# WilliamVenner/squad-mortar-helper

Measured on AMD Instinct MI355X. Metric: map frames/sec (1920x1080 full CV pipeline), whole job, higher is better.
Workload: dtype u8/f32

## Files before the change

squad-mortar-helper_amd/csrc/smh_kernels.h:

```cpp
#pragma once
#include <hip/hip_runtime.h>
#include <stdint.h>

#include "../../include/smh_vision_hip.h"
#include "../../include/smh_vision_hip_debug.h"

namespace smh {

struct Geom {
	uint32_t W, H;
	uint32_t rx, ry, rw, rh;
	uint32_t bx, by, bw, bh;
	uint32_t qx, qy, qw, qh;
	uint32_t m_ax, m_xoff, m_quads, m_block;
	uint32_t q_ax, q_xoff, q_quads, q_block;
	uint64_t frame_bytes;
	uint64_t ui_pitch, ui_stride;
	uint64_t mask_pitch, mask_stride;
	uint32_t bits_pitch_w; uint64_t bits_stride_w;
	uint64_t ocr_pitch, ocr_stride;
};

struct FrameAux {
	uint32_t open;
// ... 174 lines not shown
	uint8_t *img;
	uint8_t *cls;
	uint64_t img_stride, cls_stride;
	double mpx;
	double ring_m;
	float origin[2];
	uint32_t mm[4];
	uint32_t out_w, out_h;
	uint32_t origin_mode, line;
	uint32_t per_call, has_mpx, has_mm;
	uint32_t pal[10];
};
#define SMH_CLEAR_PROFILE (SMHV_CLEAR_MAX_SAMPLES + 1u)
struct ClearLinesRun {
	FiringRun fr;
	const smhv_frame_result *res;
	const smhv_line *lines;
	smhv_clearance_result *out;
	smhv_clearance *out_lines;
	float *profiles;
	double margin_m;
	uint32_t samples;
	uint32_t n_lines;
	uint32_t mm[4];
	uint32_t per_call, has_mm;
};
#define SMH_CLEAR_KC 32u
struct ClearMapRun {
	FiringRun fr;
	const FrameAux *aux;
	const smhv_frame_result *res;
	smhv_clearance_map_result *out;
	uint8_t *img;
	uint8_t *bytes;
	uint64_t img_stride, bytes_stride;
	double margin_m;
	float origin[2];
	uint32_t mm[4];
	uint32_t out_w, out_h;
	uint32_t samples;
	uint32_t origin_mode, line;
	uint32_t per_call, has_mm;
	uint32_t pal[4];
};
#define SMH_DBG_ITEMS (SMHV_TEXT_MAX_RUNS + 1u + 4u * SMHV_MAX_PROBES)
#define SMH_DBG_TEXT 200u
#define SMH_DBG_NONE 0u
#define SMH_DBG_TEXT_ITEM 1u
#define SMH_DBG_FILL 2u
#define SMH_DBG_FRAME 3u
struct DebugItem {
	const uint8_t *text;
	float ax, ay, bx, by;
	int32_t x0, y0, x1, y1;
	uint32_t color;
	uint32_t kind;
	uint32_t n_lines, pad;
	uint8_t off[8], len[8];
};
struct DebugRun {
	const uint8_t *ui;
	const FrameAux *aux;
	const smhv_frame_result *res;
	const smhv_text_run *runs;
	const smhv_probe_point *points;
	smhv_probe *probes;
	DebugItem *items;
	uint8_t *pool;
	uint8_t *img;
	uint64_t img_stride;
	uint32_t out_w, out_h;
	uint32_t n_runs, n_points;
	uint32_t flags;
	uint32_t scale;
	float sw, sh, tx, ty;
};
__host__ __device__ inline uint32_t tiled_rows(const Geom &g) { return (g.rh + 7u) >> 3; }
__host__ __device__ inline uint64_t tiled_stride_w(const Geom &g) { return (uint64_t)tiled_rows(g) * g.bits_pitch_w * 8u; }
__host__ __device__ inline uint32_t occ_pitch(const Geom &g) { return ((g.m_block >> 6) + 3u) & ~3u; }
__host__ __device__ inline uint64_t occ_stride(const Geom &g) { return (uint64_t)tiled_rows(g) * occ_pitch(g); }

#define SMH_RAY_OFF_BATCHES 168u

#define SMH_SECTOR_R 52
#define SMH_SECTOR_DIM (2 * SMH_SECTOR_R + 1)
#define SMH_SECTOR_ENTRIES (SMH_SECTOR_DIM * SMH_SECTOR_DIM)
#define SMH_CULL_CELLS (SMH_SECTOR_DIM * 4)
#define SMH_CULL_TAB_WORDS (SMH_CULL_CELLS + (SMH_SECTOR_ENTRIES + 3) / 4)

#define SVC_MAX_SLOTS 32u
struct SvcSlot {
	Buffers b;
	uint32_t n;
	uint32_t seq;
	uint32_t done;
	uint32_t pad;
	unsigned long long t_pub;
};
#define SVC_REMOTE_RING 12u
#define SVC_REMOTE_OPEN 0x80000000ull
struct SvcRemoteEntry {
	unsigned long long post;
	unsigned long long claim;
	uint32_t res_a[4];
	uint32_t res_b[4];
	unsigned long long pad[2];
};
struct SvcRemote {
	unsigned long long state;
	unsigned long long info;
	unsigned long long pad[6];
	SvcRemoteEntry ring[SVC_REMOTE_RING];
};
#define SVC_HELP_RING 256u
struct SvcCtl {
	int32_t avail;
	uint32_t closing;
	int32_t help_avail;
	uint32_t help_head, help_reserve;
	uint32_t stat_remote;
	uint32_t head;
	uint32_t reserve;
	uint32_t completed;
	uint32_t busy;
	uint32_t stat_items, stat_waves;
	unsigned long long stat_busy, stat_life;
	unsigned long long stat_phase[4];
	unsigned long long stat_help;
	uint32_t stat_requests, stat_attached;
	unsigned long long stat_t_wait, stat_t_sub, stat_t_last;
	uint32_t stat_h_polls, stat_h_empty, stat_h_lost, stat_h_idle_exit, stat_h_closed_exit, stat_h_pad;
	unsigned long long stat_h_cycles, stat_h_cast_cycles;
	unsigned long long help_ring[SVC_HELP_RING];
};
struct SvcHost {
	unsigned long long state;
	uint32_t launches;
	uint32_t pad0;
	uint32_t done_seq[SVC_MAX_SLOTS];
	uint32_t pad[12];
};
struct SvcParams {
	SvcCtl *ctl;
	unsigned long long *ring;
	SvcSlot *slots;
	SvcHost *host;
	const uint32_t *cull_tab;
	const float *ray_off;
	float max_gap;
	uint32_t tile_cap, list_cap;
	uint32_t part_words;
	uint32_t ring_log2;
	uint32_t epoch;
	uint32_t idle_short, idle_long;
	uint32_t flags;
	SvcRemote *remote;
	uint32_t *remote_store;
	uint32_t remote_store_words;
	uint32_t remote_after;
	uint32_t remote_tickets;
	uint32_t remote_last_div;
	uint32_t compact;
};
uint32_t svc_waves_for(const Geom &g, uint32_t tile_limit, uint32_t *part_words, uint32_t *tile_cap, uint32_t *list_cap, uint32_t *lds_bytes, uint32_t *compact = nullptr);
uint32_t svc_store_words_for(const Geom &g, uint32_t tile_cap, uint32_t compact);
hipError_t svc_probe_host_atomics(SvcHost *h, SvcHost *d_h, bool *ok);
hipError_t launch_svc_publish(SvcCtl *ctl, unsigned long long *ring, SvcSlot *slots, uint32_t slot, const Buffers &b, uint32_t n, uint32_t seq, uint32_t ring_log2, hipStream_t s);
hipError_t launch_lsd_service(const Geom &g, const SvcParams &p, uint32_t workgroups, uint32_t waves, uint32_t lds_bytes, hipStream_t s);

enum : uint32_t { MAP_UI = 1u, MAP_MASK = 2u, MAP_BYTES = 4u, MAP_PRIO = 0x100u, MAP_BAND_MAJOR = 0x200u };
enum : uint32_t { BRQ_OCR = 1u, BRQ_SCALES = 2u };
// ... 129 lines not shown
```

squad-mortar-helper_amd/csrc/smh_lsd.hip:

```cpp
#include <algorithm>
#include <atomic>
#include <cstdlib>
#include <cstring>

#include "smh_device.h"
#include "smh_proximity.h"
#include "smh_record.inc"

namespace smh {

struct RayDir { uint32_t dx, dy; };
__device__ RayDir g_ray_table[SMH_LSD_RAYS] = {
#include "ray_table.inc"
};

#ifndef LSD_BS
#define LSD_BS 1024
#endif
#define LSD_NW (LSD_BS / 64)
#ifndef LSD_C
#define LSD_C 8u
#endif
#ifndef LSD_C_RESET
#define LSD_C_RESET 2u
// ... 38 lines not shown
#define LSD_W2_PITCH 6u

enum { LSD_MODE_ROWS = 0, LSD_MODE_XWIN = 1, LSD_MODE_GLOBAL = 2, LSD_MODE_TILE = 3, LSD_MODE_WIN2 = 4, LSD_MODE_TILEC = 5 };

template <bool CACHED = false>
__device__ __forceinline__ uint32_t win_raw(const Win &m, int xi, int yi) {
	const uint32_t ry = min((uint32_t)(yi - m.y_lo), m.rows_hi);
	const int X = xi + m.xbias;
	const uint32_t rc = min((uint32_t)(X >> 5), m.cols_hi);
	uint32_t word;
	const uint32_t cr = ry - m.c_y0;
	if (CACHED && cr < m.c_rows) word = *(const LdsWord *)((const LdsByte *)m.c_p + __umul24(cr, m.c_pitch4) + (rc << 2));
	else word = *(const uint32_t *)((const char *)m.p + __umul24(ry, m.pitch4) + (rc << 2));
	return word >> ((uint32_t)X & 31u);
}
__device__ __forceinline__ uint32_t tile_word(const Win &m, int wq, int yi) {
	const uint32_t t = m.t_idx[__mul24(yi >> 3, (int)m.t_pitch) + wq];
	return m.t_tiles[(t << 3) + ((uint32_t)yi & 7u)];
}
typedef uint32_t lds_u32x4 __attribute__((ext_vector_type(4)));
__device__ __forceinline__ uint32_t tilec_number(const Win &m, int wq, int ty) {
	const uint32_t col = (uint32_t)(wq + 2);
	const lds_u32x4 e = *(const __attribute__((address_space(3))) lds_u32x4 *)(m.tc_rows + (__mul24(ty, (int)m.tc_groups) + (int)(col >> 6)) * 4);
	const uint32_t c = col & 63u;
	const uint32_t lo_m = c >= 32u ? 0xFFFFFFFFu : ((1u << c) - 1u), hi_m = c > 32u ? ((1u << (c - 32u)) - 1u) : 0u;
	const uint32_t bit = ((c >= 32u ? e.y >> (c - 32u) : e.x >> c) & 1u);
	const uint32_t before = (uint32_t)__builtin_popcount(e.x & lo_m) + (uint32_t)__builtin_popcount(e.y & hi_m);
	return bit ? e.z + before + 1u : 0u;
}
__device__ __forceinline__ uint32_t tilec_word(const Win &m, int wq, int yi) {
	return m.t_tiles[(tilec_number(m, wq, yi >> 3) << 3) + ((uint32_t)yi & 7u)];
}
__device__ __forceinline__ uint32_t tilec_raw(const Win &m, float x, float y) {
	const int yi = (int)__builtin_amdgcn_fmed3f(y, -1.0f, m.hf);
	const int xi = (int)x;
	return tilec_word(m, xi >> 5, yi) >> ((uint32_t)xi & 31u);
}
__device__ __forceinline__ void tilec_raw8(const Win &m, float xs, float ys, float dx, float dy, float &xo, float &yo, float &x, float &y, uint32_t &Wm) {
	int yi[8], xi[8];
	uint32_t t[8];
#pragma unroll
	for (int j = 0; j < 8; ++j) {
		x = xo + xs; y = yo + ys;
		yi[j] = (int)__builtin_amdgcn_fmed3f(y, -1.0f, m.hf);
		xi[j] = (int)x;
		xo += dx; yo += dy;
	}
#pragma unroll
	for (int j = 0; j < 8; ++j) t[j] = tilec_number(m, xi[j] >> 5, yi[j] >> 3);
#pragma unroll
	for (int j = 0; j < 8; ++j) t[j] = m.t_tiles[(t[j] << 3) + ((uint32_t)yi[j] & 7u)];
#pragma unroll
	for (int j = 0; j < 8; ++j) Wm = __builtin_amdgcn_alignbit(t[j] >> ((uint32_t)xi[j] & 31u), Wm, 1);
}
__device__ __forceinline__ uint32_t tile_raw(const Win &m, float x, float y) {
	const int yi = (int)__builtin_amdgcn_fmed3f(y, -1.0f, m.hf);
	const int xi = (int)x;
	return tile_word(m, xi >> 5, yi) >> ((uint32_t)xi & 31u);
}
__device__ __forceinline__ void tile_raw8(const Win &m, float xs, float ys, float dx, float dy, float &xo, float &yo, float &x, float &y, uint32_t &Wm) {
	int yi[8], xi[8];
	uint32_t t[8];
#pragma unroll
	for (int j = 0; j < 8; ++j) {
		x = xo + xs; y = yo + ys;
		yi[j] = (int)__builtin_amdgcn_fmed3f(y, -1.0f, m.hf);
		xi[j] = (int)x;
		xo += dx; yo += dy;
	}
#pragma unroll
	for (int j = 0; j < 8; ++j) t[j] = m.t_idx[__mul24(yi[j] >> 3, (int)m.t_pitch) + (xi[j] >> 5)];
#pragma unroll
	for (int j = 0; j < 8; ++j) t[j] = m.t_tiles[(t[j] << 3) + ((uint32_t)yi[j] & 7u)];
#pragma unroll
	for (int j = 0; j < 8; ++j) Wm = __builtin_amdgcn_alignbit(t[j] >> ((uint32_t)xi[j] & 31u), Wm, 1);
}
__device__ __forceinline__ uint32_t win2_raw(const Win &m, float x, float y) {
	const int yi = (int)y, xi = (int)x;
	const uint32_t word = *(const LdsWord *)(m.w2 + __mul24(yi, (int)(4u * LSD_W2_PITCH)) + ((xi >> 3) & ~3));
	return word >> ((uint32_t)xi & 31u);
}
__device__ __forceinline__ uint32_t win2_word(const Win &m, int wq, int yi) { return *(const LdsWord *)(m.w2 + __mul24(yi, (int)(4u * LSD_W2_PITCH)) + (wq << 2)); }
__device__ __forceinline__ uint32_t win2_bit(const Win &m, int xi, int yi) { return (win2_word(m, xi >> 5, yi) >> ((uint32_t)xi & 31u)) & 1u; }

__device__ __forceinline__ uint32_t win_bit(const Win &m, int xi, int yi) {
	if (m.tiled) return ((m.compact ? tilec_word(m, xi >> 5, yi) : tile_word(m, xi >> 5, yi)) >> ((uint32_t)xi & 31u)) & 1u;
	return (m.c_rows ? win_raw<true>(m, xi, yi) : win_raw<false>(m, xi, yi)) & 1u;
}

__device__ __forceinline__ uint32_t win_word(const Win &m, int wq, int yi) {
	if (m.tiled) return ((uint32_t)yi < m.h && (uint32_t)(wq + 2) < m.t_pitch) ? (m.compact ? tilec_word(m, wq, yi) : tile_word(m, wq, yi)) : 0u;
	const uint32_t ry = (uint32_t)(yi - m.y_lo), rc = (uint32_t)wq;
	uint32_t v = 0;
	if (ry <= m.rows_hi && rc <= m.cols_hi) {
		const uint32_t cr = ry - m.c_y0;
		if (cr < m.c_rows) v = *(const LdsWord *)((const LdsByte *)m.c_p + __umul24(cr, m.c_pitch4) + (rc << 2));
		else v = *(const uint32_t *)((const char *)m.p + __umul24(ry, m.pitch4) + (rc << 2));
	}
	return v;
}

__device__ __forceinline__ uint32_t win_raw_rows(const Win &m, float x, float y) {
	const int yi = (int)__builtin_amdgcn_fmed3f(y, m.ylo_f, m.yhi_f);
	const int xi = (int)x;
	const char *row = m.rows0 + __mul24(yi, (int)m.pitch4);
	const uint32_t word = *(const uint32_t *)(row + ((xi >> 5) << 2));
	return word >> ((uint32_t)xi & 31u);
}

__device__ __forceinline__ bool in_image(const Win &m, float x, float y) { return x >= 0.0f && y >= 0.0f && x < m.wf && y < m.hf; }

__device__ void cast_ray_literal(const Win &m, float xs, float ys, float max_gap, float dx, float dy, float &xe, float &ye, uint32_t &steps) {
	float x = xs, y = ys, xo = 0.0f, yo = 0.0f, g0 = 0.0f, g1 = 0.0f, g2 = 0.0f;
	while (in_image(m, x, y)) {
		++steps;
		if (win_bit(m, (int)x, (int)y)) {
			g0 = 0.0f; g1 = 0.0f; g2 = 0.0f;
		} else if (g0 >= max_gap) {
			x = g1; y = g2;
			break;
		} else if (g0 == 0.0f) {
			g0 = 1.0f; g1 = x; g2 = y;
		} else {
			g0 += 1.0f;
		}
		xo += dx; yo += dy;
		x = xo + xs; y = yo + ys;
	}
	xe = xs; ye = ys;
	const uint32_t xi = f2u(x), yi = f2u(y);
	if (xi < m.w && yi < m.h && win_bit(m, (int)xi, (int)yi) == 0u) { xe = x - dx; ye = y - dy; }
}

struct RayState {
	float bxo, byo;
	uint32_t k0, g;
	float gxo, gyo;
	uint32_t gj, gk0;
	uint32_t nexit;
};
enum { RAY_CONTINUE = 0, RAY_ABORTED = 1, RAY_LEFT_IMAGE = 2 };

template <int MODE, int G = 8>
__device__ __forceinline__ int ray_batch(const Win &m, float xs, float ys, float dx, float dy, uint32_t T, RayState &s, uint32_t &steps) {
	static_assert((G == 8 || G == 16 || G == 32) && ((MODE != LSD_MODE_TILE && MODE != LSD_MODE_TILEC) || G == 8), "group size");
	float xo = s.bxo, yo = s.byo, x = 0.0f, y = 0.0f;
	uint32_t Wm = 0;
	uint32_t taken = 0;
#pragma unroll 1
	for (int jj = 0; jj < 32 / G; ++jj) {
		if constexpr (MODE == LSD_MODE_TILE) tile_raw8(m, xs, ys, dx, dy, xo, yo, x, y, Wm);
		else if constexpr (MODE == LSD_MODE_TILEC) tilec_raw8(m, xs, ys, dx, dy, xo, yo, x, y, Wm);
		else
#pragma unroll
		for (int j = 0; j < G; ++j) {
			x = xo + xs; y = yo + ys;
			if (MODE == LSD_MODE_ROWS) Wm = __builtin_amdgcn_alignbit(win_raw_rows(m, x, y), Wm, 1);
			else if (MODE == LSD_MODE_WIN2) Wm = __builtin_amdgcn_alignbit(win2_raw(m, x, y), Wm, 1);
			else if (MODE == LSD_MODE_TILE) Wm = __builtin_amdgcn_alignbit(tile_raw(m, x, y), Wm, 1);
			else Wm = __builtin_amdgcn_alignbit(win_raw<MODE == LSD_MODE_GLOBAL>(m, (int)x, (int)y), Wm, 1);
			xo += dx; yo += dy;
		}
		taken += (uint32_t)G;
		if (taken > T && taken < 32u && __all((Wm >> (31u - T)) == 0u)) break;
	}
	Wm >>= 32u - taken;
// ... 43 lines not shown
				if (gg + len > T) {
					steps += s.k0 + pos + (T - gg) + 1u;
					return RAY_ABORTED;
				}
				gg += len;
				if (end >= 32u) break;
				rem &= 0xFFFFFFFFu << end;
			}
		}
		if (n < 32u) { steps += s.k0 + n; s.nexit = n; return RAY_LEFT_IMAGE; }
		s.g = gg;
	}
	s.bxo = xo; s.byo = yo; s.k0 += 32u;
	return RAY_CONTINUE;
}

__device__ __forceinline__ void ray_endpoint(const Win &m, int status, const RayState &s, float xs, float ys, float dx, float dy, float &xe, float &ye) {
	if (status == RAY_ABORTED) {
		float gx = s.gxo, gy = s.gyo;
		for (uint32_t k = 0; k < s.gj; ++k) { gx += dx; gy += dy; }
		xe = (gx + xs) - dx; ye = (gy + ys) - dy;
	} else {
		float rx = s.bxo, ry = s.byo;
		for (uint32_t k = 0; k < s.nexit; ++k) { rx += dx; ry += dy; }
		const float px = rx + xs, py = ry + ys;
		xe = xs; ye = ys;
		const uint32_t xi = f2u(px), yi = f2u(py);
		if (xi < m.w && yi < m.h && win_bit(m, (int)xi, (int)yi) == 0u) { xe = px - dx; ye = py - dy; }
	}
}

__device__ __forceinline__ uint32_t white_at(const Win &m, float fx, float fy) {
	const uint32_t xi = min(f2u(fx), m.w - 1u), yi = min(f2u(fy), m.h - 1u);
	return win_bit(m, (int)xi, (int)yi);
}
__device__ void get_centre(const Win &m, float px, float py, float &ox, float &oy) {
	float left = px;
	while (left > 0.0f && fabsf(left - px) < SMH_LSD_CENTRE_REACH && white_at(m, left, py)) left -= 1.0f;
	float right = px;
	while (right < (float)(m.w - 1u) && fabsf(right - px) < SMH_LSD_CENTRE_REACH && white_at(m, right, py)) right += 1.0f;
	float up = py;
	while (up > 0.0f && fabsf(up - py) < SMH_LSD_CENTRE_REACH && white_at(m, px, up)) up -= 1.0f;
	float down = py;
	while (down < (float)(m.h - 1u) && fabsf(down - py) < SMH_LSD_CENTRE_REACH && white_at(m, px, down)) down += 1.0f;
	ox = (left + right) / 2.0f;
	oy = (up + down) / 2.0f;
}


#ifdef SMH_LSD_PROFILE
#define PROF_DECL unsigned long long prof_t[12] = {0, 0, 0, 0, 0, 0, 0, 0, 0, 0, 0, 0}, prof_last = __builtin_amdgcn_s_memtime();
#define PROF_MARK(i) do { const unsigned long long _n = __builtin_amdgcn_s_memtime(); prof_t[i] += _n - prof_last; prof_last = _n; } while (0)
#define PROF_STORE(res) do { if (threadIdx.x == 0) for (int _i = 0; _i < 12; ++_i) ((unsigned long long *)(res)->meters)[20 + _i] = prof_t[_i]; } while (0)
#define PROF_ARG , prof_t
#else
#define PROF_DECL
#define PROF_MARK(i)
#define PROF_STORE(res)
#define PROF_ARG
#endif

struct LsdShared {
	unsigned long long cand_best[LSD_C];
	unsigned long long unit_key[LSD_UNITS];
	float unit_end[LSD_UNITS][2];
	uint32_t unit_kmax[LSD_UNITS];
	float cand_pt[LSD_C][2];
	float cand_end[LSD_C][2];
	uint32_t cand_steps[LSD_C];
	uint32_t cand_kmax[LSD_C];
	uint32_t cand_key[LSD_C];
	uint32_t scan[LSD_NW];
	uint32_t qtail, segnext, unit_next;
	uint32_t cand_px[LSD_C][2];
	uint32_t cand_wkey[LSD_C];
	uint32_t cached;
	uint32_t post[LSD_LOOKAHEAD];
	uint32_t req_tail, posted_hi, posted_new, helpers_seen, head_seen;
	uint32_t h_n;
	unsigned long long pick;
	uint32_t nlive;
	unsigned short ulist[LSD_UNITS];
	unsigned long long live[LSD_C];
	float lines[SMH_LSD_MAX_LINES][4];
	float prox_a[SMH_LSD_MAX_LINES];
	double prox_d[SMH_LSD_MAX_LINES][2];
#ifdef SMH_LSD_PROFILE
	uint32_t exp_far, exp_units;
#endif
};

__device__ __forceinline__ ProxLine shared_prox_line(const LsdShared &sh, uint32_t l) {
	ProxLine L;
	L.x0 = sh.lines[l][0]; L.y0 = sh.lines[l][1]; L.x1 = sh.lines[l][2]; L.y1 = sh.lines[l][3];
	L.a = sh.prox_a[l]; L.dxl = sh.prox_d[l][0]; L.dyl = sh.prox_d[l][1];
	L.degenerate = L.dxl == 0.0 && L.dyl == 0.0;
	return L;
}

template <int MODE>
__device__ void ray_engine(const Win &m, LsdShared &sh, uint32_t *queue, uint32_t nc, float max_gap, bool always_exact, unsigned long long *prof_t = nullptr) {
	const uint32_t tid = threadIdx.x, lane = tid & 63u, wave = tid >> 6;
#ifdef SMH_LSD_PROFILE
	unsigned long long prof_last = __builtin_amdgcn_s_memtime();
#endif
	const bool fast_gap = max_gap > 0.0f && max_gap <= 60000.0f;
	const uint32_t T = fast_gap ? (uint32_t)ceilf(max_gap) : 0u;
	const uint32_t nunits = nc * LSD_GROUPS, nlive = sh.nlive;

	uint32_t pos = wave;
	uint32_t pn = 0;
	if (lane == 0) pn = atomicAdd(&sh.unit_next, 1u);
	pn = (uint32_t)__builtin_amdgcn_readfirstlane((int)pn);
	uint32_t u = pos < nlive ? sh.ulist[pos] : 0u;
	RayDir nd = g_ray_table[min((u % LSD_GROUPS) * 64u + lane, (uint32_t)SMH_LSD_RAYS - 1u)];
	for (; pos < nlive; ) {
		const uint32_t c = u / LSD_GROUPS, i = (u - c * LSD_GROUPS) * 64u + lane;
		const bool valid = i < SMH_LSD_RAYS;
		const float dx = __uint_as_float(nd.dx), dy = __uint_as_float(nd.dy);
		const uint32_t ucur = u;
		pos = pn;
		if (pos < nlive) {
			u = sh.ulist[pos];
			nd = g_ray_table[min((u % LSD_GROUPS) * 64u + lane, (uint32_t)SMH_LSD_RAYS - 1u)];
			if (lane == 0) pn = atomicAdd(&sh.unit_next, 1u);
			pn = (uint32_t)__builtin_amdgcn_readfirstlane((int)pn);
		}
		const float xs = sh.cand_pt[c][0], ys = sh.cand_pt[c][1];
		const bool fast = fast_gap && in_image(m, xs, ys);
		float xe = xs, ye = ys;
		uint32_t steps = 0;
		int status = RAY_ABORTED;
		bool exact = false;
		RayState s = {0.0f, 0.0f, 0u, 0u, 0.0f, 0.0f, 0u, 0u, 0u};
		if (valid) {
			if (fast) {
				status = RAY_CONTINUE;
#pragma unroll 1
				for (uint32_t bi = 0; bi < LSD_A_BATCHES && status == RAY_CONTINUE; ++bi) status = ray_batch<MODE>(m, xs, ys, dx, dy, T, s, steps);
			} else {
				cast_ray_literal(m, xs, ys, max_gap, dx, dy, xe, ye, steps);
				exact = true;
			}
		}
#ifdef SMH_LSD_PROFILE
		if (prof_t) { const unsigned long long _n = __builtin_amdgcn_s_memtime(); prof_t[0] += _n - prof_last; prof_last = _n; }
#endif
		const uint64_t sv = __ballot(status == RAY_CONTINUE);
		if (sv) {
			uint32_t base = 0;
			if (lane == 0) base = atomicAdd(&sh.qtail, (uint32_t)__popcll(sv));
			base = (uint32_t)__builtin_amdgcn_readfirstlane((int)base);
			const uint32_t slot = base + (uint32_t)__popcll(sv & ((1ull << lane) - 1ull));
			if (status == RAY_CONTINUE && slot >= LSD_QCAP) {
				while (status == RAY_CONTINUE) status = ray_batch<MODE>(m, xs, ys, dx, dy, T, s, steps);
				ray_endpoint(m, status, s, xs, ys, dx, dy, xe, ye);
				exact = true;
			} else if (status == RAY_CONTINUE) {
				queue[2u * slot] = (c << 16) | i;
				queue[2u * slot + 1u] = s.g | (s.gj << 16) | ((s.gk0 >> 5) << 24);
			}
		}
		const bool fin = valid && status != RAY_CONTINUE;
		if (fin && !exact && (status == RAY_LEFT_IMAGE || (!always_exact && s.gk0 + s.gj > SMH_LSD_REJECT_K))) { ray_endpoint(m, status, s, xs, ys, dx, dy, xe, ye); exact = true; }
		if (__any(fin && exact)) {
			unsigned long long key = 0;
// ... 172 lines not shown
	uint32_t wy0, wrows, wwords;
	int xorg;
	uint32_t c_pitch, c_cap_rows;
};

template <int MODE, bool WAVE = false>
__device__ __forceinline__ void frame_setup(const Geom &g, const Buffers &b, uint32_t f, const FrameAux &aux, uint32_t *smem, FrameView &v) {
	static_assert(!WAVE || MODE == LSD_MODE_GLOBAL, "only the global-memory view is built without the workgroup");
	const uint32_t tid = threadIdx.x;
	const uint32_t *gbits = b.bits + (size_t)f * g.bits_stride_w;
	Win &m = v.m;
	v.gbits = gbits;
	m.w = g.rw; m.h = g.rh; m.wf = (float)g.rw; m.hf = (float)g.rh;
	m.rows0 = nullptr; m.ylo_f = 0.0f; m.yhi_f = 0.0f;
	m.c_p = (const LdsWord *)smem; m.c_y0 = 0u; m.c_rows = 0u; m.c_pitch4 = 0u;
	m.t_idx = nullptr; m.t_tiles = nullptr; m.t_pitch = 0u; m.tiled = false; m.w2 = nullptr;
	m.tc_rows = nullptr; m.tc_groups = 0u; m.compact = false;
	v.c_pitch = g.bits_pitch_w | 1u; v.c_cap_rows = min(g.rh, LSD_WIN_WORDS_CAP / v.c_pitch);
	if (MODE == LSD_MODE_ROWS) {
		const uint32_t wy0 = aux.y_min, wrows = aux.y_max - aux.y_min + 1u;
		v.wy0 = wy0; v.wrows = wrows; v.wwords = LSD_ROWS_PITCH(g.bits_pitch_w); v.xorg = 0;
		const uint32_t pitch = v.wwords, gp = g.bits_pitch_w;
		const uint32_t total = (wrows + 2u) * pitch + 4u;
		for (uint32_t idx = tid; idx < total; idx += blockDim.x) {
			uint32_t val = 0;
			if (idx >= 2u + pitch && idx < 2u + (wrows + 1u) * pitch) {
				const uint32_t k = idx - 2u - pitch, r = k / pitch, c = k - r * pitch;
				if (c < gp) {
					const uint32_t *src = gbits + (size_t)(wy0 + r) * gp + c;
					const uint32_t lo = src[0], hi = (c + 1u < gp) ? src[1] : 0u;
					val = __builtin_amdgcn_alignbit(hi, lo, g.m_xoff);
				}
			}
			smem[idx] = val;
		}
		m.p = smem + 2; m.pitch4 = pitch * 4u;
		m.y_lo = (int)wy0 - 1; m.rows_hi = wrows + 1u;
		m.xbias = 0; m.cols_hi = pitch - 1u;
		m.rows0 = (const char *)(smem + 2) - (ptrdiff_t)((int)wy0 - 1) * (ptrdiff_t)(pitch * 4u);
		m.ylo_f = (float)((int)wy0 - 1); m.yhi_f = (float)(wy0 + wrows);
	} else if (MODE == LSD_MODE_XWIN) {
		const uint32_t ww0 = aux.w_min, wy0 = aux.y_min, wrows = aux.y_max - aux.y_min + 1u, wwords = aux.w_max - aux.w_min + 1u;
		v.wy0 = wy0; v.wrows = wrows; v.wwords = wwords;
		v.xorg = (int)(ww0 * 32u) - (int)g.m_xoff;
		const uint32_t pitch = (wwords + 2u) | 1u;
		m.p = smem; m.pitch4 = pitch * 4u;
		m.y_lo = (int)wy0 - 1; m.rows_hi = wrows + 1u;
		m.xbias = (int)g.m_xoff - 32 * ((int)ww0 - 1); m.cols_hi = wwords + 1u;
		const uint32_t total = (wrows + 2u) * pitch;
		for (uint32_t idx = tid; idx < total; idx += blockDim.x) {
			const uint32_t r = idx / pitch, c = idx - r * pitch;
			uint32_t val = 0;
			if (r >= 1u && r <= wrows && c >= 1u && c <= wwords) val = gbits[(size_t)(wy0 + r - 1u) * g.bits_pitch_w + ww0 + c - 1u];
			smem[idx] = val;
		}
	} else {
		v.wy0 = 0; v.wrows = g.rh; v.wwords = g.bits_pitch_w; v.xorg = -(int)g.m_xoff;
		m.p = gbits; m.pitch4 = g.bits_pitch_w * 4u;
		m.y_lo = 0; m.rows_hi = g.rh - 1u;
		m.xbias = (int)g.m_xoff; m.cols_hi = g.bits_pitch_w - 1u;
	}
	if (!WAVE) __syncthreads();
}

template <int MODE>
__device__ __forceinline__ void cache_cover(const Geom &g, FrameView &v, uint32_t *smem, int lo, int hi) {
	if (MODE != LSD_MODE_GLOBAL) return;
	Win &m = v.m;
	lo = max(lo, 0); hi = min(hi, (int)g.rh - 1);
	if (m.c_rows && lo >= (int)m.c_y0 && hi < (int)(m.c_y0 + m.c_rows)) return;
	__syncthreads();
	const uint32_t y0 = (uint32_t)min(lo, (int)(g.rh - v.c_cap_rows));
	for (uint32_t idx = threadIdx.x; idx < v.c_cap_rows * v.c_pitch; idx += LSD_BS) {
		const uint32_t r = idx / v.c_pitch, c = idx - r * v.c_pitch;
		smem[idx] = c < g.bits_pitch_w ? v.gbits[(size_t)(y0 + r) * g.bits_pitch_w + c] : 0u;
	}
	m.c_y0 = y0; m.c_rows = v.c_cap_rows; m.c_pitch4 = v.c_pitch * 4u;
	__syncthreads();
}

__device__ __forceinline__ void group_reset(LsdShared &sh, uint32_t nc, bool cull) {
	const uint32_t tid = threadIdx.x;
	if (tid < nc * LSD_GROUPS) { sh.unit_key[tid] = 0ull; sh.unit_kmax[tid] = 0u; }
	if (tid < LSD_C) { sh.cand_best[tid] = 0ull; sh.cand_steps[tid] = 0u; sh.cand_kmax[tid] = 0u; sh.live[tid] = cull ? 0ull : ~0ull; }
	if (tid == 0) { sh.qtail = 0u; sh.unit_next = LSD_NW; sh.nlive = 0u; sh.cached = 0u;
#ifdef SMH_LSD_PROFILE
		sh.exp_far = 0u; sh.exp_units = 0u;
#endif
	}
}

template <int MODE>
__device__ __forceinline__ void cast_group(const Win &m, LsdShared &sh, uint32_t *queue, const uint32_t *cull_tab, uint32_t nc, bool cull, float max_gap,
                                           unsigned long long *prof_t = nullptr) {
	const uint32_t tid = threadIdx.x;
#ifdef SMH_LSD_PROFILE
	unsigned long long prof_last = __builtin_amdgcn_s_memtime();
#endif
	if (tid < nc * 32u) {
		const uint32_t c = tid >> 5, l = tid & 31u, dir = l >> 3, k = l & 7u;
		const float cx = (float)sh.cand_px[c][0], cy = (float)sh.cand_px[c][1];
		const float fk = (float)k;
		bool cond = k < 5u;
		if (dir == 0u) cond = cond && (cx - fk > 0.0f) && white_at(m, cx - fk, cy);
		else if (dir == 1u) cond = cond && (cx + fk < (float)(m.w - 1u)) && white_at(m, cx + fk, cy);
		else if (dir == 2u) cond = cond && (cy - fk > 0.0f) && white_at(m, cx, cy - fk);
		else cond = cond && (cy + fk < (float)(m.h - 1u)) && white_at(m, cx, cy + fk);
		const uint32_t bits = (uint32_t)(__ballot(cond) >> (tid & 32u));
		if (l == 0u) {
			const float nl = (float)__builtin_ctz(~(bits & 0xFFu)), nr = (float)__builtin_ctz(~((bits >> 8) & 0xFFu));
			const float nu = (float)__builtin_ctz(~((bits >> 16) & 0xFFu)), nd = (float)__builtin_ctz(~((bits >> 24) & 0xFFu));
			sh.cand_pt[c][0] = ((cx - nl) + (cx + nr)) / 2.0f;
			sh.cand_pt[c][1] = ((cy - nu) + (cy + nd)) / 2.0f;
		}
	}
	__syncthreads();
#ifdef SMH_LSD_PROFILE
	if (prof_t) { const unsigned long long _n = __builtin_amdgcn_s_memtime(); prof_t[10] += _n - prof_last; prof_last = _n; }
#endif
	const uint32_t cached = sh.cached;
	if (cull) {
		for (uint32_t id = tid; id < nc * SMH_CULL_CELLS; id += LSD_BS) {
			const uint32_t c = id / SMH_CULL_CELLS, cell = id - c * SMH_CULL_CELLS;
			if ((cached >> c) & 1u) continue;
			const int fx = (int)floorf(sh.cand_pt[c][0]), fy = (int)floorf(sh.cand_pt[c][1]);
			const int yi = fy + (int)(cell >> 2) - SMH_SECTOR_R;
			if ((uint32_t)yi >= m.h) continue;
			const int b0 = fx - SMH_SECTOR_R + (int)((cell & 3u) << 5) + m.xbias;
			const uint32_t lo = win_word(m, b0 >> 5, yi), hi = win_word(m, (b0 >> 5) + 1, yi);
			uint32_t hit = __builtin_amdgcn_alignbit(hi, lo, (uint32_t)b0 & 31u) & cull_tab[cell];
			if (hit) {
				const uint8_t *codes = (const uint8_t *)(cull_tab + SMH_CULL_CELLS) + (cell >> 2) * SMH_SECTOR_DIM + ((cell & 3u) << 5);
				unsigned long long acc = 0ull;
				while (hit) {
					const uint32_t code = codes[__builtin_ctz(hit)];
					hit &= hit - 1u;
					acc |= code == 0xFFu ? ~0ull : ((2ull << (code >> 6)) - 1ull) << (code & 63u);
				}
				atomicOr(&sh.live[c], (acc | (acc >> LSD_GROUPS)) & ((1ull << LSD_GROUPS) - 1ull));
			}
		}
		__syncthreads();
	}
	if (tid < nc * LSD_GROUPS) {
		const uint32_t c = tid / LSD_GROUPS;
		if (!((cached >> c) & 1u) && ((sh.live[c] >> (tid - c * LSD_GROUPS)) & 1ull)) sh.ulist[atomicAdd(&sh.nlive, 1u)] = (unsigned short)tid;
	}
	__syncthreads();
#ifdef SMH_LSD_PROFILE
	if (prof_t) { const unsigned long long _n = __builtin_amdgcn_s_memtime(); prof_t[11] += _n - prof_last; prof_last = _n; }
#endif
	if (sh.nlive != 0u) ray_engine<MODE>(m, sh, queue, nc, max_gap, false PROF_ARG);
}

template <int MODE>
__device__ void lsd_frame(const Geom &g, const Buffers &b, uint32_t f, float max_gap, int mode, float spx, float spy, const FrameAux &aux,
                          uint32_t *smem, LsdShared &sh, uint32_t *cull_tab, LsdCoop *co) {
	const uint32_t tid = threadIdx.x, lane = tid & 63u, wave = tid >> 6;
	smhv_frame_result *res = &b.results[f];
	PROF_DECL
	FrameView v;
	frame_setup<MODE>(g, b, f, aux, smem, v);
	Win &m = v.m;
	uint32_t *list = smem + LSD_WIN_WORDS_CAP, *queue = list + LSD_LIST_CAP;
	const uint32_t wy0 = v.wy0, wrows = v.wrows, wwords = v.wwords;
	const int xorg = v.xorg;
	const uint32_t WT = wrows * wwords;
	auto dom_word = [&](uint32_t wi) -> uint32_t {
		const uint32_t r = wi / wwords, c = wi - r * wwords;
		if (MODE == LSD_MODE_ROWS) return m.p[(r + 1u) * wwords + c];
		if (MODE == LSD_MODE_XWIN) return m.p[(r + 1u) * (m.pitch4 >> 2) + c + 1u];
		return m.p[wi];
	};

	if (mode == 1) {
		if (tid < LSD_GROUPS) { sh.unit_key[tid] = 0ull; sh.unit_kmax[tid] = 0u; sh.ulist[tid] = (unsigned short)tid; }
		cache_cover<MODE>(g, v, smem, (int)spy - (int)(v.c_cap_rows / 2u), (int)spy - (int)(v.c_cap_rows / 2u) + (int)v.c_cap_rows - 1);
		if (tid == 0) { sh.live[0] = ~0ull; sh.cand_best[0] = 0ull; sh.cand_steps[0] = 0u; sh.cand_kmax[0] = 0u; sh.qtail = 0u; sh.unit_next = LSD_NW; sh.nlive = LSD_GROUPS; sh.cand_pt[0][0] = spx; sh.cand_pt[0][1] = spy; }
		__syncthreads();
		ray_engine<MODE>(m, sh, queue, 1u, max_gap, true PROF_ARG);
		if (tid == 0) {
			res->lines[0].x0 = spx; res->lines[0].y0 = spy; res->lines[0].x1 = sh.cand_end[0][0]; res->lines[0].y1 = sh.cand_end[0][1];
			res->length_px[0] = (double)__uint_as_float((uint32_t)(sh.cand_best[0] >> 32));
			res->n_lines = 1; res->rounds = 1; res->ray_steps = sh.cand_steps[0]; res->status = SMHV_FRAME_OK;
		}
		return;
	}

	const bool cull = b.cull_tab != nullptr && max_gap > 0.0f && max_gap <= 49.0f;
	const uint32_t *ring = co ? b.co.req + (size_t)f * SMH_LSD_REQ_CAP : nullptr;
	const LsdCacheEntry *ctab = co ? b.co.cache + (size_t)f * SMH_LSD_CACHE_SLOTS : nullptr;
	if (tid == 0) { sh.req_tail = 0u; sh.posted_hi = 0u; sh.posted_new = 0u; sh.helpers_seen = 0u; sh.head_seen = 0u; if (co) st_relaxed(&co->mode1, (uint32_t)MODE + 1u); }
	if (tid < LSD_LOOKAHEAD) sh.post[tid] = 0u;
	uint32_t rounds = 0, n_lines = 0;
	unsigned long long steps = 0ull;
	uint32_t seg_start = 0, cmax = 1u;
	bool done = false;
	PROF_MARK(8);
	while (!done) {
		const uint32_t range = WT - seg_start;
		const uint32_t per = (range + LSD_BS - 1u) / LSD_BS;
		const uint32_t my0 = min(seg_start + tid * per, WT), my1 = min(my0 + per, WT);
		uint32_t cnt = 0;
		for (uint32_t wi = my0; wi < my1; ++wi) cnt += dom_word(wi) != 0u ? 1u : 0u;
		uint32_t incl = cnt;
		for (int o = 1; o < 64; o <<= 1) { const uint32_t t = __shfl_up(incl, o); if (lane >= (uint32_t)o) incl += t; }
		if (lane == 63) sh.scan[wave] = incl;
		if (tid == 0) sh.segnext = WT;
		__syncthreads();
		uint32_t wprefix = 0, total = 0;
#pragma unroll
		for (int k = 0; k < LSD_NW; ++k) { const uint32_t s = sh.scan[k]; if ((uint32_t)k < wave) wprefix += s; total += s; }
		uint32_t o = wprefix + incl - cnt;
		for (uint32_t wi = my0; wi < my1; ++wi)
			if (dom_word(wi) != 0u) {
				if (o < LSD_LIST_CAP) list[o] = wi;
				else if (o == LSD_LIST_CAP) sh.segnext = wi;
				++o;
			}
		__syncthreads();
		const uint32_t Tn = min(total, LSD_LIST_CAP);
		const uint32_t segnext = sh.segnext;
		PROF_MARK(9);

		for (uint32_t cbase = 0; cbase < Tn && !done; cbase += LSD_BS) {
			const uint32_t e = cbase + tid;
			uint32_t surv = 0, wkey0 = 0;
			float py = 0.0f, px0 = 0.0f;
			if (e < Tn) {
				const uint32_t wi = list[e];
				surv = dom_word(wi);
				const uint32_t r = wi / wwords, c = wi - r * wwords;
				py = (float)(wy0 + r);
				px0 = (float)(xorg + (int)(c * 32u));
				wkey0 = (wi << 5) + 1u;
				for (uint32_t l = 0; l < n_lines && surv; ++l) surv = prox_filter_word(surv, px0, py, shared_prox_line(sh, l));
			}
			while (true) {
				if (co && tid == 0) {
					sh.helpers_seen = ld_relaxed(&co->helpers); sh.head_seen = ld_relaxed(&co->req_head);
					sh.posted_hi = max(sh.posted_hi, sh.posted_new);
				}
				const uint32_t pc = __popc(surv);
				uint32_t pin = pc;
				for (int o2 = 1; o2 < 64; o2 <<= 1) { const uint32_t t = __shfl_up(pin, o2); if (lane >= (uint32_t)o2) pin += t; }
				if (lane == 63) sh.scan[wave] = pin;
				__syncthreads();
				uint32_t wp = 0, tot = 0;
#pragma unroll
				for (int k = 0; k < LSD_NW; ++k) { const uint32_t s = sh.scan[k]; if ((uint32_t)k < wave) wp += s; tot += s; }
				if (tot == 0u) break;
				const bool helped = co != nullptr && sh.helpers_seen != 0u;
				const uint32_t posted_hi = sh.posted_hi;
				uint32_t nc = min(tot, cmax);
				uint32_t rank = wp + pin - pc;
				while (surv && rank < cmax) {
					const uint32_t bit = __builtin_ctz(surv);
					surv &= surv - 1u;
					sh.cand_key[rank] = (tid << 5) | bit;
					sh.cand_wkey[rank] = wkey0 + bit;
					sh.cand_px[rank][0] = (uint32_t)((int)px0 + (int)bit); sh.cand_px[rank][1] = (uint32_t)py;
					++rank;
				}
				if (helped) {
					uint32_t s2 = surv, r2 = rank;
					while (s2 && r2 < cmax + LSD_LOOKAHEAD) {
						const uint32_t bit = __builtin_ctz(s2);
						s2 &= s2 - 1u;
						if (r2 >= cmax && wkey0 + bit > posted_hi) {
							sh.post[r2 - cmax] = 0x80000000u | pix_pack((uint32_t)((int)px0 + (int)bit), (uint32_t)py);
							atomicMax(&sh.posted_new, wkey0 + bit);
						}
// ... 14 lines not shown
					nc = nce;
					cache_cover<MODE>(g, v, smem, lo, (int)sh.cand_px[nc - 1u][1] + LSD_CACHE_MARGIN);
				}
				if (helped) {
					if (wave == 0) {
						const uint32_t pv = lane < LSD_LOOKAHEAD ? sh.post[lane] : 0u;
						if (lane < LSD_LOOKAHEAD) sh.post[lane] = 0u;
						const unsigned long long valid = __ballot((pv >> 31) != 0u);
						const uint32_t tail = sh.req_tail, used = tail - min(sh.head_seen, tail);
						const uint32_t room = SMH_LSD_REQ_CAP - min(used, SMH_LSD_REQ_CAP);
						const uint32_t pos = (uint32_t)__popcll(valid & ((1ull << lane) - 1ull));
						const uint32_t np = min((uint32_t)__popcll(valid), room);
						if ((pv >> 31) && pos < np) {
							const uint32_t idx = tail + pos;
							st_relaxed(const_cast<uint32_t *>(ring) + idx % SMH_LSD_REQ_CAP, (((idx / SMH_LSD_REQ_CAP) & 0xFFu) << 24) | (pv & 0xFFFFFFu));
						}
						if (lane == 0 && np) { st_release(&co->req_tail, tail + np); sh.req_tail = tail + np; }
						if (lane == 0) __hip_atomic_fetch_add(&co->stat_groups, 1u, __ATOMIC_RELAXED, __HIP_MEMORY_SCOPE_AGENT);
					} else if (tid >= 64u && tid < 64u + nc) {
						const uint32_t c = tid - 64u;
						unsigned long long best; float ex, ey; uint32_t st;
						if (cache_lookup(ctab, b.co.epoch, pix_pack(sh.cand_px[c][0], sh.cand_px[c][1]), best, ex, ey, st)) {
							sh.cand_best[c] = best; sh.cand_end[c][0] = ex; sh.cand_end[c][1] = ey; sh.cand_steps[c] = st;
							atomicOr(&sh.cached, 1u << c);
							__hip_atomic_fetch_add(&co->stat_hits, 1u, __ATOMIC_RELAXED, __HIP_MEMORY_SCOPE_AGENT);
						}
					}
					__syncthreads();
				}
				PROF_MARK(10);
				cast_group<MODE>(m, sh, queue, cull_tab, nc, cull, max_gap PROF_ARG);
#ifdef SMH_LSD_PROFILE
				prof_last = __builtin_amdgcn_s_memtime();
#endif

				const uint32_t first_new = n_lines;
				for (uint32_t c = 0; c < nc; ++c) {
					const float cx = (float)sh.cand_px[c][0], cy = (float)sh.cand_px[c][1];
					bool skip = false;
					for (uint32_t l = first_new; l < n_lines; ++l)
						skip = skip || near_line(cx, cy, sh.lines[l][0], sh.lines[l][1], sh.lines[l][2], sh.lines[l][3]);
					if (skip) continue;
					++rounds;
					steps += sh.cand_steps[c];
					const float len = __uint_as_float((uint32_t)(sh.cand_best[c] >> 32));
					if (len > SMH_LSD_ACCEPT_LEN_SQ) {
						float ex, ey;
						get_centre(m, sh.cand_end[c][0], sh.cand_end[c][1], ex, ey);
						sh.lines[n_lines][0] = sh.cand_pt[c][0]; sh.lines[n_lines][1] = sh.cand_pt[c][1];
						sh.lines[n_lines][2] = ex; sh.lines[n_lines][3] = ey;
						const ProxLine pl = prox_line(sh.cand_pt[c][0], sh.cand_pt[c][1], ex, ey);
						sh.prox_a[n_lines] = pl.a; sh.prox_d[n_lines][0] = pl.dxl; sh.prox_d[n_lines][1] = pl.dyl;
						++n_lines;
						if (n_lines == SMH_LSD_MAX_LINES) { done = true; break; }
					}
				}
				if (done) break;
				if (helped && n_lines != first_new && tid == 0) {
					__hip_atomic_fetch_max(&co->req_head, sh.req_tail, __ATOMIC_RELAXED, __HIP_MEMORY_SCOPE_AGENT);
					sh.posted_hi = sh.cand_wkey[nc - 1u]; sh.posted_new = 0u;
				}
				cmax = (n_lines != first_new) ? LSD_C_RESET : min(cmax * 2u, LSD_C);
				PROF_MARK(5);
				for (uint32_t l = first_new; l < n_lines && surv; ++l) surv = prox_filter_word(surv, px0, py, shared_prox_line(sh, l));
			}
			__syncthreads();
		}
		if (segnext >= WT) break;
		seg_start = segnext;
		__syncthreads();
	}
	__syncthreads();
	if (tid < n_lines) {
		res->lines[tid].x0 = sh.lines[tid][0]; res->lines[tid].y0 = sh.lines[tid][1];
		res->lines[tid].x1 = sh.lines[tid][2]; res->lines[tid].y1 = sh.lines[tid][3];
	}
	if (tid == 0) { res->n_lines = n_lines; res->rounds = rounds; res->ray_steps = steps; res->status = SMHV_FRAME_OK; }
	PROF_STORE(res);
}

template <int MODE>
__device__ void lsd_help(const Geom &g, const Buffers &b, uint32_t n_frames, float max_gap, uint32_t *smem, LsdShared &sh, uint32_t *cull_tab, bool have_cull_tab) {
	const uint32_t tid = threadIdx.x;
	const bool cull = b.cull_tab != nullptr && max_gap > 0.0f && max_gap <= 49.0f;
	if (cull && !have_cull_tab) for (uint32_t i = tid; i < SMH_CULL_TAB_WORDS; i += LSD_BS) cull_tab[i] = b.cull_tab[i];
	uint32_t *queue = smem + LSD_WIN_WORDS_CAP + LSD_LIST_CAP;
	uint32_t idle = 0;
	while (true) {
		unsigned long long key = 0ull;
		for (uint32_t f = tid; f < n_frames; f += LSD_BS) {
			const LsdCoop *c = &b.co.coop[f];
			const uint32_t rem = ld_relaxed(&c->remaining), hl = ld_relaxed(&c->helpers), dn = ld_relaxed(&c->done);
			if (!dn && hl < LSD_MAX_HELPERS && rem >= LSD_HELP_MIN_REMAINING && ld_relaxed(&c->mode1) == (uint32_t)MODE + 1u) {
				const unsigned long long k = ((unsigned long long)(rem / (hl + 1u)) << 32) | f;
				key = k > key ? k : key;
			}
		}
		if (tid == 0) sh.pick = 0ull;
		__syncthreads();
		key = wave_max64(key);
		if ((tid & 63u) == 0 && key) atomicMax(&sh.pick, key);
		__syncthreads();
		const unsigned long long pick = sh.pick;
		if (pick == 0ull) {
			if (tid == 0) sh.h_n = ld_relaxed(&b.co.ctl->finished[MODE]);
			__syncthreads();
			const uint32_t fin = sh.h_n;
			__syncthreads();
			if (fin >= n_frames || ++idle > LSD_HELPER_IDLE_POLLS) return;
			__builtin_amdgcn_s_sleep(127);
			continue;
		}
		const uint32_t f = (uint32_t)pick;
		LsdCoop *co = &b.co.coop[f];
		if (tid == 0) {
			const uint32_t prev = __hip_atomic_fetch_add(&co->helpers, 1u, __ATOMIC_RELAXED, __HIP_MEMORY_SCOPE_AGENT);
			sh.h_n = prev < LSD_MAX_HELPERS ? 1u : 0u;
			if (prev >= LSD_MAX_HELPERS) __hip_atomic_fetch_sub(&co->helpers, 1u, __ATOMIC_RELAXED, __HIP_MEMORY_SCOPE_AGENT);
		}
		__syncthreads();
		if (sh.h_n == 0u) { __syncthreads(); continue; }
		__syncthreads();
		const FrameAux aux = b.aux[f];
		FrameView v;
		frame_setup<MODE>(g, b, f, aux, smem, v);
		const uint32_t *ring = b.co.req + (size_t)f * SMH_LSD_REQ_CAP;
		LsdCacheEntry *ctab = b.co.cache + (size_t)f * SMH_LSD_CACHE_SLOTS;
		uint32_t misses = 0;
		while (true) {
			if (tid == 0) {
				uint32_t px[LSD_C];
				uint32_t n = 0;
				if (ld_relaxed(&co->done)) n = 0xFFFFFFFFu;
				else {
					const uint32_t got = ring_claim(co, ring, px);
					for (uint32_t i = 0; i < got; ++i) {
						const uint32_t x = px[i] & 0xFFFu, y = px[i] >> 12;
						unsigned long long best; float ex, ey; uint32_t st;
						if (x < v.m.w && y < v.m.h && !cache_lookup(ctab, b.co.epoch, px[i], best, ex, ey, st)) { sh.cand_px[n][0] = x; sh.cand_px[n][1] = y; ++n; }
					}
				}
				sh.h_n = n;
			}
			__syncthreads();
			const uint32_t nc = sh.h_n;
			if (nc == 0xFFFFFFFFu) break;
			if (nc == 0u) {
				__syncthreads();
				if (++misses > LSD_HELPER_IDLE_POLLS) break;
				__builtin_amdgcn_s_sleep(127);
				continue;
			}
			misses = 0; idle = 0;
			group_reset(sh, nc, cull);
			__syncthreads();
			if (MODE == LSD_MODE_GLOBAL) {
				int lo = (int)sh.cand_px[0][1], hi = lo;
				for (uint32_t c = 1; c < nc; ++c) { lo = min(lo, (int)sh.cand_px[c][1]); hi = max(hi, (int)sh.cand_px[c][1]); }
				cache_cover<MODE>(g, v, smem, lo - LSD_CACHE_MARGIN, min(hi + LSD_CACHE_MARGIN, lo - LSD_CACHE_MARGIN + (int)v.c_cap_rows - 1));
			}
			cast_group<MODE>(v.m, sh, queue, cull_tab, nc, cull, max_gap);
			if (tid == 0) __hip_atomic_fetch_add(&co->stat_casts, nc, __ATOMIC_RELAXED, __HIP_MEMORY_SCOPE_AGENT);
			if (tid < nc) cache_insert(ctab, b.co.epoch, pix_pack(sh.cand_px[tid][0], sh.cand_px[tid][1]), sh.cand_best[tid], sh.cand_end[tid][0], sh.cand_end[tid][1], sh.cand_steps[tid]);
			__syncthreads();
		}
		if (tid == 0) __hip_atomic_fetch_sub(&co->helpers, 1u, __ATOMIC_RELAXED, __HIP_MEMORY_SCOPE_AGENT);
		__syncthreads();
	}
}

__device__ __forceinline__ int lsd_mode_for(const Geom &g, const FrameAux &aux, uint32_t cap = LSD_WIN_WORDS_CAP) {
	int lmode = LSD_MODE_GLOBAL;
	if (aux.n_mask_px != 0) {
		const uint32_t wrows = aux.y_max - aux.y_min + 1u, wwords = aux.w_max - aux.w_min + 1u;
		if ((wrows + 2u) * LSD_ROWS_PITCH(g.bits_pitch_w) + 4u <= cap) lmode = LSD_MODE_ROWS;
		else if ((wrows + 2u) * ((wwords + 2u) | 1u) <= cap) lmode = LSD_MODE_XWIN;
	}
	return lmode;
}

template <int MODE, bool COOP>
__global__ void __launch_bounds__(LSD_BS) __attribute__((amdgpu_waves_per_eu(5, 5))) k_lsd(Geom g, Buffers b, float max_gap, int mode, float spx, float spy, uint32_t n_frames) {
	extern __shared__ __attribute__((aligned(16))) uint32_t smem[];
	__shared__ LsdShared sh;
	__shared__ uint32_t cull_tab[SMH_CULL_TAB_WORDS];
	const uint32_t f = blockIdx.x;
	const bool coop = COOP && mode == 0 && b.co.ctl != nullptr;
	bool have_tab = false;
	if (f < n_frames) {
		if (coop && threadIdx.x == 0) __hip_atomic_fetch_add(&b.co.ctl->started[MODE], 1u, __ATOMIC_RELAXED, __HIP_MEMORY_SCOPE_AGENT);
		const FrameAux aux = b.aux[f];
		bool mine = true;
		if (mode == 0) {
			if (!aux.open || aux.n_mask_px == 0) {
				if (MODE == LSD_MODE_ROWS && threadIdx.x == 0) { b.results[f].n_lines = 0; b.results[f].rounds = 0; b.results[f].ray_steps = 0; b.results[f].status = SMHV_FRAME_OK; }
				mine = false;
			}
		}
		bool record = mode == 0 && (b.rec_stages & SMH_REC_ON) != 0u && !mine && MODE == LSD_MODE_ROWS;
		if (mine && lsd_mode_for(g, aux) != MODE) mine = false;
		if (mine) {
			const bool cull = mode == 0 && b.cull_tab != nullptr && max_gap > 0.0f && max_gap <= 49.0f;
			if (cull) { for (uint32_t i = threadIdx.x; i < SMH_CULL_TAB_WORDS; i += LSD_BS) cull_tab[i] = b.cull_tab[i]; have_tab = true; }
			lsd_frame<MODE>(g, b, f, max_gap, mode, spx, spy, aux, smem, sh, cull_tab, (COOP && coop) ? &b.co.coop[f] : nullptr);
			record = mode == 0 && (b.rec_stages & SMH_REC_ON) != 0u;
		}
		if (record) {
			struct Head { Geom g; Buffers b; };
			const Head *ka = (const Head *)__builtin_amdgcn_kernarg_segment_ptr();
			__syncthreads();
			frame_record_tail(&ka->g, &ka->b, f);
		}
		if (!COOP || !coop) return;
		__syncthreads();
		if (threadIdx.x == 0) {
			if (mine) { st_relaxed(&b.co.coop[f].remaining, 0u); st_release(&b.co.coop[f].done, 1u); }
			__hip_atomic_fetch_add(&b.co.ctl->finished[MODE], 1u, __ATOMIC_RELAXED, __HIP_MEMORY_SCOPE_AGENT);
			sh.h_n = (mine && ld_relaxed(&b.co.ctl->started[MODE]) >= n_frames) ? 1u : 0u;
		}
		__syncthreads();
		if (sh.h_n == 0u) return;
		__syncthreads();
	} else if (!coop) {
		return;
	}
	if (COOP) lsd_help<MODE>(g, b, n_frames, max_gap, smem, sh, cull_tab, have_tab);
}

#include "smh_lsd_wave.inc"
#include "smh_lsd_seq.inc"
#include "smh_service.inc"

__global__ void k_build_sector_table(unsigned long long *tab, uint32_t T) {
	const uint32_t i = blockIdx.x * blockDim.x + threadIdx.x;
	if (i >= SMH_SECTOR_ENTRIES) return;
	const int oy = (int)(i / SMH_SECTOR_DIM) - SMH_SECTOR_R, ox = (int)(i % SMH_SECTOR_DIM) - SMH_SECTOR_R;
	const double rho = 0.7072 + 0.7072 + 0.05;
	const double kmin = T >= 50u ? 0.0 : (double)(50u - T), kmax = 50.0;
	const double r0 = sqrt((double)(ox * ox + oy * oy));
	unsigned long long m = 0ull;
	if (r0 >= kmin - rho && r0 <= kmax + rho) {
		if (r0 <= rho) {
			m = ~0ull;
		} else {
			const double PI = 3.14159265358979323846;
			double phi = atan2((double)oy, (double)ox) * 180.0 / PI;
			if (phi < 0.0) phi += 360.0;
			const double delta = asin(rho / r0 > 1.0 ? 1.0 : rho / r0) * 180.0 / PI + 0.2;
			for (int u = 0; u < LSD_GROUPS_HOST; ++u) {
				const double a0 = 6.4 * u, a1 = 6.4 * u + 6.3;
				bool hit = false;
				for (int wrap = -1; wrap <= 1 && !hit; ++wrap) {
					const double lo = phi - delta + 360.0 * wrap, hi = phi + delta + 360.0 * wrap;
					hit = !(hi < a0 || lo > a1);
				}
				if (hit) m |= 1ull << u;
			}
		}
	}
	tab[i] = m;
}

size_t lsd_lds_bytes() { return LSD_DYN_LDS_BYTES; }

static std::atomic<bool> &lsd_classic_flag() {
	static std::atomic<bool> flag{false};
	return flag;
}
void lsd_set_classic(bool on) { lsd_classic_flag().store(on, std::memory_order_relaxed); }
static std::atomic<uint32_t> g_tile_cap_override{0};
void lsd_set_tile_cap(uint32_t cap) { g_tile_cap_override.store(cap, std::memory_order_relaxed); }
static std::atomic<uint32_t> g_bs_override{0};
void lsd_set_threads(uint32_t threads) { g_bs_override.store(threads, std::memory_order_relaxed); }
static std::atomic<uint32_t> g_spin_limit{W_SPIN_LIMIT_DEFAULT};
void lsd_set_spin_limit(uint32_t polls) { g_spin_limit.store(polls ? polls : W_SPIN_LIMIT_DEFAULT, std::memory_order_relaxed); }

bool lsd_rows_only(const Geom &g) { return (g.rh + 2u) * LSD_ROWS_PITCH(g.bits_pitch_w) + 4u <= LSD_WIN_WORDS_CAP; }

static uint32_t lsd_tile_static_lds() {
	static const uint32_t v = [] { hipFuncAttributes a; return hipFuncGetAttributes(&a, (const void *)k_lsd_tile) == hipSuccess ? (uint32_t)a.sharedSizeBytes : 17408u; }();
	return v;
}
static uint32_t lsd_tile_cap_of(const Geom &g, uint32_t tile_limit) {
	const uint32_t cap_o = g_tile_cap_override.load(std::memory_order_relaxed);
	uint32_t cap = tile_cap_for(g);
	if (tile_limit) cap = std::min(cap, tile_limit);
	if (cap_o) cap = std::min(cap_o, tile_cap_for(g));
	return cap;
}
uint32_t lsd_tile_lds_bytes(const Geom &g, uint32_t tile_limit) {
	return lsd_tile_static_lds() + (tile_mask_words(g.rw, g.rh, lsd_tile_cap_of(g, tile_limit)) + 2u * tile_list_cap_for(g) + W_NWIN * W_WIN_STRIDE) * 4u;
}

hipError_t launch_lsd(const Geom &g, const Buffers &b, uint32_t n, float max_gap, int mode, float px, float py, hipStream_t s, const LsdFork *fk, uint32_t tile_bs, bool prefer_classic,
                      uint32_t tile_limit, bool *record_fused) {
	if (record_fused) *record_fused = false;
	const unsigned lds_full = LSD_DYN_LDS_BYTES;
	static std::atomic<uint64_t> attr_devices{0};
	int dev = 0;
	hipError_t e0 = hipGetDevice(&dev);
	if (e0 != hipSuccess) return e0;
	if (dev >= 64 || !((attr_devices.load(std::memory_order_acquire) >> dev) & 1ull)) {
		hipError_t e = hipSuccess;
		const void *fns[] = {(const void *)k_lsd<LSD_MODE_ROWS, false>, (const void *)k_lsd<LSD_MODE_XWIN, false>, (const void *)k_lsd<LSD_MODE_GLOBAL, false>,
		                     (const void *)k_lsd<LSD_MODE_ROWS, true>, (const void *)k_lsd<LSD_MODE_XWIN, true>, (const void *)k_lsd<LSD_MODE_GLOBAL, true>};
		for (const void *fn : fns) if (e == hipSuccess) e = hipFuncSetAttribute(fn, hipFuncAttributeMaxDynamicSharedMemorySize, (int)lds_full);
		if (e == hipSuccess) e = hipFuncSetAttribute((const void *)k_lsd_tile, hipFuncAttributeMaxDynamicSharedMemorySize, (int)LSD_TILE_DYN_LDS_MAX);
		if (e != hipSuccess) return e;
		if (dev < 64) attr_devices.fetch_or(1ull << dev, std::memory_order_release);
	}
	const bool rows_only = mode == 0 && lsd_rows_only(g);
	const bool coop = mode == 0 && b.co.ctl != nullptr;
	if (mode == 0 && !coop && !prefer_classic && !lsd_classic_flag().load(std::memory_order_relaxed)) {
		const uint32_t bs_o = g_bs_override.load(std::memory_order_relaxed);
		const uint32_t bs = std::max<uint32_t>(128u, bs_o ? bs_o : (tile_bs ? std::min<uint32_t>(tile_bs, LSD_TILE_BS) : 512u));
		const uint32_t cap = lsd_tile_cap_of(g, tile_limit);
		const unsigned t_lds = std::min<unsigned>((tile_mask_words(g.rw, g.rh, cap) + 2u * tile_list_cap_for(g) + W_NWIN * W_WIN_STRIDE) * 4u, LSD_TILE_DYN_LDS_MAX);
		if (record_fused) *record_fused = (b.rec_stages & SMH_REC_ON) != 0u;
		hipLaunchKernelGGL(k_lsd_tile, dim3(n), dim3(bs), t_lds, s, g, b, max_gap, cap, g_spin_limit.load(std::memory_order_relaxed), tile_list_cap_for(g), n);
		return hipGetLastError();
	}
	if (coop) {
		hipError_t e = hipMemsetAsync(b.co.ctl, 0, lsd_coop_ctl_bytes(n), s);
		if (e != hipSuccess) return e;
	}
	uint32_t extra = 0;
	if (coop && rows_only) {
		static std::atomic<int> n_cus{0};
		int cus = n_cus.load(std::memory_order_relaxed);
		if (cus == 0) {
			if (hipDeviceGetAttribute(&cus, hipDeviceAttributeMultiprocessorCount, dev) != hipSuccess || cus <= 0) cus = 256;
			n_cus.store(cus, std::memory_order_relaxed);
		}
		if (n < (uint32_t)cus) extra = std::min((uint32_t)cus - n, 4u * n);
	}
	hipStream_t s1 = s, s2 = s;
	if (!rows_only && fk) {
		hipError_t e = hipEventRecord(fk->fork, s);
		if (e == hipSuccess) e = hipStreamWaitEvent(fk->s1, fk->fork, 0);
		if (e == hipSuccess) e = hipStreamWaitEvent(fk->s2, fk->fork, 0);
		if (e != hipSuccess) return e;
		s1 = fk->s1; s2 = fk->s2;
	}
// ... 29 lines not shown
		const uint32_t part = (SVC_WS_WORDS + (c ? tilec_mask_words(g.rw, g.rh, cap) : tile_mask_words(g.rw, g.rh, cap)) + 2u * lc + SVC_WIN_STRIDE(c) + 3u) & ~3u;
		uint32_t w = SVC_MAX_WAVES;
		while (w > 0u && lsd_service_static_lds() + w * part * 4u + beside > lds_cu) --w;
		if (w > best_w) { best_w = w; best_part = part; best_lc = lc; best_c = c; }
	}
	if (part_words) *part_words = best_part;
	if (tile_cap) *tile_cap = cap;
	if (list_cap) *list_cap = best_lc;
	if (lds_bytes) *lds_bytes = best_w * best_part * 4u;
	if (compact) *compact = best_c;
	return best_w;
}

uint32_t svc_store_words_for(const Geom &g, uint32_t tile_cap, uint32_t compact) { return ((compact ? tilec_mask_words(g.rw, g.rh, tile_cap) : tile_mask_words(g.rw, g.rh, tile_cap)) + 7u) & ~3u; }

hipError_t svc_probe_host_atomics(SvcHost *h, SvcHost *d_h, bool *ok) {
	*ok = false;
	uint32_t *d_ok = nullptr;
	hipError_t e = hipMalloc((void **)&d_ok, sizeof(uint32_t));
	if (e != hipSuccess) return e;
	const unsigned long long expect = 0x0123456789ABCDEFull, desired = 0xFEDCBA9876543210ull;
	unsigned long long *w = (unsigned long long *)&h->pad[0];
	__atomic_store_n(w, expect, __ATOMIC_RELEASE);
	__atomic_store_n(&h->pad[2], 0u, __ATOMIC_RELEASE);
	e = hipMemset(d_ok, 0, sizeof(uint32_t));
	uint32_t dev_ok = 0;
	if (e == hipSuccess) { hipLaunchKernelGGL(k_svc_probe, dim3(1), dim3(1), 0, nullptr, d_h, expect, desired, d_ok); e = hipGetLastError(); }
	if (e == hipSuccess) e = hipMemcpy(&dev_ok, d_ok, sizeof dev_ok, hipMemcpyDeviceToHost);
	(void)hipFree(d_ok);
	if (e != hipSuccess) return e;
	*ok = dev_ok == 1u && __atomic_load_n(w, __ATOMIC_ACQUIRE) == desired && __atomic_load_n(&h->pad[2], __ATOMIC_ACQUIRE) == 0x600Du;
	__atomic_store_n(w, 0ull, __ATOMIC_RELEASE);
	__atomic_store_n(&h->pad[2], 0u, __ATOMIC_RELEASE);
	return hipSuccess;
}

hipError_t launch_svc_publish(SvcCtl *ctl, unsigned long long *ring, SvcSlot *slots, uint32_t slot, const Buffers &b, uint32_t n, uint32_t seq, uint32_t ring_log2, hipStream_t s) {
	hipLaunchKernelGGL(k_svc_publish, dim3(1), dim3(256), 0, s, ctl, ring, slots, slot, b, n, seq, ring_log2);
	return hipGetLastError();
}

hipError_t launch_lsd_service(const Geom &g, const SvcParams &p, uint32_t workgroups, uint32_t waves, uint32_t lds_bytes, hipStream_t s) {
	static std::atomic<uint64_t> attr_devices{0};
	int dev = 0;
	hipError_t e = hipGetDevice(&dev);
	if (e != hipSuccess) return e;
	if (dev >= 64 || !((attr_devices.load(std::memory_order_acquire) >> dev) & 1ull)) {
		e = hipFuncSetAttribute((const void *)k_lsd_service, hipFuncAttributeMaxDynamicSharedMemorySize, 160 * 1024 - (int)lsd_service_static_lds());
		if (e == hipSuccess) e = hipFuncSetAttribute((const void *)k_lsd_service_c, hipFuncAttributeMaxDynamicSharedMemorySize, 160 * 1024 - (int)lsd_service_static_lds());
		if (e != hipSuccess) return e;
		if (dev < 64) attr_devices.fetch_or(1ull << dev, std::memory_order_release);
	}
	if (p.compact) hipLaunchKernelGGL(k_lsd_service_c, dim3(workgroups), dim3(64u * waves), lds_bytes, s, g, p);
	else hipLaunchKernelGGL(k_lsd_service, dim3(workgroups), dim3(64u * waves), lds_bytes, s, g, p);
	return hipGetLastError();
}

size_t lsd_coop_ctl_bytes(uint32_t n) { return sizeof(LsdCtl) + sizeof(LsdCoop) * (size_t)n; }

hipError_t set_ray_table(const float *dx, const float *dy) {
	static RayDir host[SMH_LSD_RAYS];
	for (int i = 0; i < SMH_LSD_RAYS; ++i) { memcpy(&host[i].dx, &dx[i], 4); memcpy(&host[i].dy, &dy[i], 4); }
	return hipMemcpyToSymbol(HIP_SYMBOL(g_ray_table), host, sizeof host, 0, hipMemcpyHostToDevice);
}

__global__ void k_build_ray_offsets(float *off) {
	const uint32_t i = blockIdx.x * blockDim.x + threadIdx.x;
	if (i >= SMH_LSD_RAYS) return;
	const float dx = __uint_as_float(g_ray_table[i].dx), dy = __uint_as_float(g_ray_table[i].dy);
	float xo = 0.0f, yo = 0.0f;
	float2 *o = (float2 *)off + (size_t)i * (SMH_RAY_OFF_BATCHES + 1u);
	for (uint32_t j = 0; j <= SMH_RAY_OFF_BATCHES; ++j) {
		o[j] = make_float2(xo, yo);
		for (int k = 0; k < 32; ++k) { xo += dx; yo += dy; }
	}
}

hipError_t launch_build_ray_offsets(float *d_off, hipStream_t s) {
	hipLaunchKernelGGL(k_build_ray_offsets, dim3((SMH_LSD_RAYS + 63) / 64), dim3(64), 0, s, d_off);
	return hipGetLastError();
}

hipError_t launch_build_sector_table(unsigned long long *d_tab, uint32_t T, hipStream_t s) {
	static_assert(LSD_GROUPS == LSD_GROUPS_HOST && LSD_GROUPS <= 64, "sector masks are 64-bit");
	hipLaunchKernelGGL(k_build_sector_table, dim3((SMH_SECTOR_ENTRIES + 255) / 256), dim3(256), 0, s, d_tab, T);
	return hipGetLastError();
}

}
```

squad-mortar-helper_amd/csrc/smh_lsd_seq.inc:

```

template <int MODE>
__device__ __forceinline__ uint32_t seq_build_list(const Win &m, WShared &ws, uint32_t *list, uint32_t *survw, uint32_t list_cap, uint32_t wy0, uint32_t wrows, uint32_t wwords, uint32_t wi_min,
                                                   uint32_t WT, uint32_t *wi_next) {
	const uint32_t lane = threadIdx.x & 63u;
	uint32_t o = 0, next = WT;
	auto append = [&](uint32_t w, uint32_t wi) {
		const unsigned long long nz = __ballot(w != 0u);
		if (!nz) return;
		const uint32_t pos = o + (uint32_t)__popcll(nz & ((1ull << lane) - 1ull));
		if (w != 0u && pos < list_cap) { list[pos] = wi; survw[pos] = w; ws.stag[pos] = 0; }
		const uint32_t cnt = (uint32_t)__popcll(nz);
		if (o + cnt > list_cap) {
			unsigned long long rest = nz;
			for (uint32_t k = o; k < list_cap; ++k) rest &= rest - 1ull;
			next = (uint32_t)__builtin_amdgcn_readlane((int)wi, (int)__builtin_ctzll(rest));
			o = list_cap;
		} else o += cnt;
	};
	if constexpr (MODE == LSD_MODE_TILE || MODE == LSD_MODE_TILEC) {
		auto tile_at = [&](uint32_t ty, uint32_t c) -> uint32_t {
			if constexpr (MODE == LSD_MODE_TILEC) return tilec_number(m, (int)c, (int)ty);
			else return (uint32_t)m.t_idx[__mul24((int)ty, (int)m.t_pitch) + (int)c];
		};
		const bool two = wwords <= 32u;
// ... 116 lines not shown
	uint32_t ok = 0;
	if ((threadIdx.x & 63u) == 0u && tickets) {
		if (__hip_atomic_fetch_add(&ctl->help_avail, (int32_t)tickets, __ATOMIC_RELAXED, __HIP_MEMORY_SCOPE_AGENT) + (int32_t)tickets <= (int32_t)(SVC_HELP_RING / 2u)) {
			const uint32_t base = __hip_atomic_fetch_add(&ctl->help_reserve, tickets, __ATOMIC_RELAXED, __HIP_MEMORY_SCOPE_AGENT);
			for (uint32_t t = 0; t < tickets; ++t) {
				const uint32_t tk = base + t;
				g_st64(&ctl->help_ring[tk & (SVC_HELP_RING - 1u)], ((unsigned long long)(tk / SVC_HELP_RING + 1u) << 32) | ((gen & 0xFFFFu) << 16) | (ws.rem_owner & 0xFFFFu));
			}
			ok = 1u;
		} else __hip_atomic_fetch_sub(&ctl->help_avail, (int32_t)tickets, __ATOMIC_RELAXED, __HIP_MEMORY_SCOPE_AGENT);
	}
	return uniform_u32(ok) != 0u;
}
__device__ __forceinline__ SvcCtl *rem_ctl_of(const WShared &ws) {
	return (SvcCtl *)(uintptr_t)(((unsigned long long)uniform_u32((uint32_t)(ws.rem_ctl >> 32)) << 32) | uniform_u32((uint32_t)ws.rem_ctl));
}
template <bool COMPACT>
__device__ __attribute__((noinline)) bool remote_open(uint32_t ws_off, uint32_t store_off, uint32_t idx_words) {
	WShared &ws = *(WShared *)(LdsWord *)(uintptr_t)uniform_u32(ws_off);
	const uint32_t lane = threadIdx.x & 63u;
	SvcRemote *r = rem_of(ws);
	SvcCtl *ctl = rem_ctl_of(ws);
	uint32_t *dump = (uint32_t *)(uintptr_t)(((unsigned long long)uniform_u32((uint32_t)(ws.rem_store >> 32)) << 32) | uniform_u32((uint32_t)ws.rem_store));
	const uint32_t tickets = uniform_u32(ws.rem_tickets), tile_cap = uniform_u32(ws.rem_cap), ntiles = min(uniform_u32(ws.ntiles), tile_cap);
	const unsigned long long st = g_ld64(&r->state);
	const uint32_t st_lo = uniform_u32((uint32_t)st), st_hi = uniform_u32((uint32_t)(st >> 32));
	if (st_lo != 0u) return false;
	if ((int32_t)uniform_u32((uint32_t)__hip_atomic_load(&ctl->help_avail, __ATOMIC_RELAXED, __HIP_MEMORY_SCOPE_AGENT)) > (int32_t)(SVC_HELP_RING / 4u)) return false;
	const uint4 *src = (const uint4 *)(LdsWord *)(uintptr_t)uniform_u32(store_off);
	uint4 *dst = (uint4 *)dump;
	for (uint32_t i = lane; i < (ntiles + 1u) * 2u; i += 64u) dst[i] = src[i];
	const uint32_t q0 = (tile_cap + 1u) * 2u, nq = (idx_words + 3u) / 4u;
	for (uint32_t i = lane; i < nq; i += 64u) dst[q0 + i] = src[q0 + i];
	if (lane < SVC_REMOTE_RING) {
		const rem_u32x4 z = {0u, 0u, 0u, 0u};
		g_st64(&r->ring[lane].post, 0ull); g_st64(&r->ring[lane].claim, 0ull); g_st128(r->ring[lane].res_a, z); g_st128(r->ring[lane].res_b, z);
	}
	if (lane == 0) g_st64(&r->info, (unsigned long long)ntiles);
	asm volatile("s_waitcnt vmcnt(0)" ::: "memory");
	__builtin_amdgcn_fence(__ATOMIC_RELEASE, "agent");
	asm volatile("s_waitcnt vmcnt(0)" ::: "memory");
	uint32_t gen = st_hi + 1u;
	if ((gen & 0xFFFFu) == 0u) ++gen;
	if (lane == 0) {
		g_st64(&r->state, ((unsigned long long)gen << 32) | SVC_REMOTE_OPEN);
		__hip_atomic_fetch_add(&ctl->stat_requests, 1u, __ATOMIC_RELAXED, __HIP_MEMORY_SCOPE_AGENT);
		ws.rem_open = 1u; ws.rem_gen = gen; ws.rem_k = 0u; ws.rem_nr = 0u;
	}
	wave_lds_sync();
	(void)remote_issue_tickets(ws, ctl, gen, tickets);
	return true;
}

__device__ __forceinline__ void tile_win(Win &m, uint32_t rw, uint32_t rh, uint32_t *smem, uint32_t tile_cap) {
	const uint32_t TWP = tile_idx_pitch(rw);
	m.w = rw; m.h = rh; m.wf = (float)rw; m.hf = (float)rh;
	m.p = smem; m.pitch4 = 0u; m.y_lo = 0; m.xbias = 0; m.rows_hi = 0u; m.cols_hi = 0u;
	m.rows0 = nullptr; m.ylo_f = 0.0f; m.yhi_f = 0.0f;
	m.c_p = (const LdsWord *)smem; m.c_y0 = 0u; m.c_rows = 0u; m.c_pitch4 = 0u;
	m.t_idx = (const LdsU16 *)(smem + (tile_cap + 1u) * 8u) + TWP + 2u; m.t_tiles = (const LdsWord *)smem; m.t_pitch = TWP; m.tiled = true;
	m.tc_rows = nullptr; m.tc_groups = 0u; m.compact = false;
	m.w2 = nullptr;
}

__device__ __forceinline__ void tilec_win(Win &m, uint32_t rw, uint32_t rh, uint32_t *smem, uint32_t tile_cap) {
	tile_win(m, rw, rh, smem, tile_cap);
	const uint32_t G = tilec_groups(rw);
	m.t_idx = nullptr;
	m.tc_rows = (const LdsWord *)(smem + (tile_cap + 1u) * 8u + G * 4u); m.tc_groups = G; m.compact = true;
}

#ifndef SVC_WIN_EXTRA
#define SVC_WIN_EXTRA 24u
#endif
#ifdef SMH_NO_WINDOW_REUSE
#define SVC_WIN_REUSE(compact) false
#else
#define SVC_WIN_REUSE(compact) (!(compact))
#endif
#define SVC_WIN_ROWS(compact) (SVC_WIN_REUSE(compact) ? W_WIN_ROWS + SVC_WIN_EXTRA : W_WIN_ROWS)
#define SVC_WIN_STRIDE(compact) (SVC_WIN_ROWS(compact) * LSD_W2_PITCH + 2u)

template <int MODE, bool REUSE = false>
__device__ __forceinline__ void seq_cast_candidate(const Win &m, uint32_t *wwin, WinTag *tag, const uint32_t *cull_tab, bool cull, const RayDir *dirs, const float *ray_off, float max_gap,
                                                   uint32_t px, uint32_t py, float &xs, float &ys, unsigned long long &wkey, float &ex0, float &ey0, uint32_t &steps_sum
#ifdef SMH_LSD_WDEBUG
                                                   , unsigned long long *sprof, unsigned long long &slast, unsigned long long *uprof, uint32_t &n_units
#endif
                                                   ) {
	const uint32_t lane = opaque_lane();
	unsigned long long live;
#ifdef SMH_LSD_WDEBUG
	cand_setup<MODE == LSD_MODE_TILEC, (REUSE ? W_WIN_ROWS + SVC_WIN_EXTRA : W_WIN_ROWS), REUSE>(m, wwin, cull_tab, cull, px, py, xs, ys, live, tag, uprof);
	{ const unsigned long long _n = __builtin_amdgcn_s_memtime(); sprof[2] += _n - slast; slast = _n; }
#else
	cand_setup<MODE == LSD_MODE_TILEC, (REUSE ? W_WIN_ROWS + SVC_WIN_EXTRA : W_WIN_ROWS), REUSE>(m, wwin, cull_tab, cull, px, py, xs, ys, live, tag);
#endif
	unsigned long long bkey = 0ull;
	float bxe = xs, bye = ys;
	uint32_t st = 0;
	auto unit_dirs_lds = [&](uint32_t u) -> RayDir { return dirs[min(u * 64u + lane, (uint32_t)SMH_LSD_RAYS - 1u)]; };
	RayDir dn = unit_dirs_lds(live ? (uint32_t)__builtin_ctzll(live) : 0u);
	for (unsigned long long todo = live; todo; todo &= todo - 1ull) {
		const uint32_t u = (uint32_t)__builtin_ctzll(todo);
		const RayDir d = dn;
		const unsigned long long rest = todo & (todo - 1ull);
		if (rest) dn = unit_dirs_lds((uint32_t)__builtin_ctzll(rest));
		unsigned long long key;
		float xe, ye;
#ifdef SMH_LSD_WDEBUG
		unit_rays<MODE, (MODE == LSD_MODE_TILEC ? SEQ_RAY_GROUP_C : SEQ_RAY_GROUP), REUSE>(m, wwin, ray_off, px, py, xs, ys, u, d, max_gap, key, xe, ye, st, uprof, tag);
		++n_units;
#else
		unit_rays<MODE, (MODE == LSD_MODE_TILEC ? SEQ_RAY_GROUP_C : SEQ_RAY_GROUP), REUSE>(m, wwin, ray_off, px, py, xs, ys, u, d, max_gap, key, xe, ye, st, tag);
#endif
		if (key > bkey) { bkey = key; bxe = xe; bye = ye; }
	}
	steps_sum = wave_sum32_dpp(st);
	wkey = 0ull; ex0 = xs; ey0 = ys;
	if (__any(bkey != 0ull)) {
		const uint32_t hi = (uint32_t)(bkey >> 32), lo = (uint32_t)bkey;
		const uint32_t mhi = wave_max32_dpp(hi);
		const uint32_t mlo = wave_max32_dpp(hi == mhi ? lo : 0u);
		wkey = ((unsigned long long)mhi << 32) | mlo;
		if (wkey != 0ull) {
			const uint32_t src = (uint32_t)__builtin_ctzll(__ballot(bkey == wkey));
			ex0 = bcast_f(bxe, src); ey0 = bcast_f(bye, src);
		}
	}
#ifdef SMH_LSD_WDEBUG
	{ const unsigned long long _n = __builtin_amdgcn_s_memtime(); sprof[3] += _n - slast; slast = _n; }
#endif
}

__device__ __forceinline__ bool desk_take(WShared &ws, uint32_t px, uint32_t py, float &xs, float &ys, unsigned long long &wkey, float &ex0, float &ey0, uint32_t &steps_sum) {
	const uint32_t lane = opaque_lane();
	bool match = false;
	if (lane < SEQ_DESK_ENTRIES) {
		const uint32_t st = W_LD_ACQ(&ws.rob[lane].state);
		match = st != (uint32_t)H_FREE && st != (uint32_t)H_RZOMBIE && ws.rob[lane].px == px && ws.rob[lane].py == py;
	}
	const unsigned long long hit = __ballot(match);
	if (!hit) return false;
	const uint32_t e = (uint32_t)__builtin_ctzll(hit);
	WSlot &sl = ws.rob[e];
	if (e >= SEQ_HELP_SLOTS) {
		if (uniform_u32(sl.state) == (uint32_t)H_RPOSTED) remote_harvest(ws);
		WDBG(0, 1u);
		if (uniform_u32(sl.state) == (uint32_t)H_RPOSTED) {
			const uint32_t k = uniform_u32(sl.lines_seen);
			uint32_t old = 0;
			if (lane == 0) old = (uint32_t)__hip_atomic_fetch_max(&rem_of(ws)->ring[e - SEQ_HELP_SLOTS].claim, (unsigned long long)k, __ATOMIC_RELAXED, __HIP_MEMORY_SCOPE_AGENT);
			if (uniform_u32(old) < k) {
				if (lane == 0) sl.state = H_FREE;
				wave_lds_sync();
				WDBG(1, 1u);
				return false;
			}
			WDBG(2, 1u);
#ifdef SMH_LSD_WDEBUG
			const unsigned long long t_w = __builtin_amdgcn_s_memtime();
#endif
			while (uniform_u32(sl.state) != (uint32_t)H_DONE) { __builtin_amdgcn_s_sleep(16); remote_harvest(ws); }
#ifdef SMH_LSD_WDEBUG
			if (lane == 0) ws.prof[0] += __builtin_amdgcn_s_memtime() - t_w;
#endif
		}
// ... 107 lines not shown
	for (uint32_t k = 1; k < np; ++k) {
		const uint32_t qx = (uint32_t)__builtin_amdgcn_readlane((int)mpx, (int)k), qy = (uint32_t)__builtin_amdgcn_readlane((int)mpy, (int)k);
		const bool live = lane < SEQ_DESK_ENTRIES && st != (uint32_t)H_FREE && st != (uint32_t)H_RZOMBIE;
		if (__ballot(live && spx == qx && spy == qy) != 0ull) continue;
		const unsigned long long free_l = __ballot(lane < SEQ_HELP_SLOTS && st == (uint32_t)H_FREE);
		const unsigned long long free_r = __ballot(lane >= SEQ_HELP_SLOTS && lane < SEQ_DESK_ENTRIES && st == (uint32_t)H_FREE);
		const uint32_t busy_l = SEQ_HELP_SLOTS - (uint32_t)__popcll(free_l);
		const uint32_t busy_r = (uint32_t)__popcll(__ballot(lane >= SEQ_HELP_SLOTS && live));
		if (busy_l < cap_local && free_l) {
			const uint32_t slot = (uint32_t)__builtin_ctzll(free_l);
			if (lane == slot) {
				ws.rob[slot].px = qx; ws.rob[slot].py = qy; ws.rob[slot].lines_seen = post_seq;
				W_ST_REL(&ws.rob[slot].state, (uint32_t)H_POSTED);
				st = H_POSTED; spx = qx; spy = qy;
			}
			++post_seq;
		} else if (busy_r < cap_remote && free_r) desk_post_remote(ws, (uint32_t)__builtin_ctzll(free_r), qx, qy, st, spx, spy);
		else break;
	}
}

__device__ __forceinline__ void desk_post_more(WShared &ws, const uint32_t *list, uint32_t *survw, uint32_t wy0, uint32_t wwords, int xorg, uint32_t cap_local, uint32_t cap_remote, uint32_t &post_seq,
                                               uint32_t &cur_e, int &cur_bit, uint32_t &ahead) {
	const uint32_t lane = opaque_lane();
	uint32_t st = H_DONE;
	if (lane < SEQ_DESK_ENTRIES) st = W_LD_ACQ(&ws.rob[lane].state);
	unsigned long long free_l = __ballot(lane < SEQ_HELP_SLOTS && st == (uint32_t)H_FREE);
	unsigned long long free_r = __ballot(lane >= SEQ_HELP_SLOTS && lane < SEQ_DESK_ENTRIES && st == (uint32_t)H_FREE);
	uint32_t busy_l = SEQ_HELP_SLOTS - (uint32_t)__popcll(free_l);
	uint32_t busy_r = (uint32_t)__popcll(__ballot(lane >= SEQ_HELP_SLOTS && lane < SEQ_DESK_ENTRIES && (st == (uint32_t)H_RPOSTED || st == (uint32_t)H_DONE)));
	if (cap_remote && busy_r < cap_remote && !free_r && __ballot(lane >= SEQ_HELP_SLOTS && lane < SEQ_DESK_ENTRIES && st == (uint32_t)H_RZOMBIE)) {
		remote_harvest(ws);
		if (lane < SEQ_DESK_ENTRIES) st = W_LD_ACQ(&ws.rob[lane].state);
		free_r = __ballot(lane >= SEQ_HELP_SLOTS && lane < SEQ_DESK_ENTRIES && st == (uint32_t)H_FREE);
	}
	bool room_l = busy_l < cap_local && free_l, room_r = busy_r < cap_remote && free_r;
	if (!room_l && !room_r) return;
	const uint32_t n_lines = W_LD(&ws.n_lines), end = ws.disp_end, first = W_LD(&ws.disp_e);
	while ((room_l || room_r) && cur_e < end) {
		const uint32_t e0 = cur_e & ~63u;
		float fpx0, fpy;
		uint32_t w = disp_entry(ws, list, survw, e0 + lane, first, end, n_lines, wy0, wwords, xorg, fpx0, fpy);
		if (e0 + lane < cur_e) w = 0u;
		else if (e0 + lane == cur_e && cur_bit >= 0) w = cur_bit >= 31 ? 0u : (w & ~((2u << (uint32_t)cur_bit) - 1u));
		const unsigned long long any = __ballot(w != 0u);
		if (!any) { cur_e = e0 + 64u; cur_bit = -1; continue; }
		const uint32_t src = (uint32_t)__builtin_ctzll(any);
		const uint32_t ww = (uint32_t)__builtin_amdgcn_readlane((int)w, (int)src);
		const uint32_t bit = (uint32_t)__builtin_ctz(ww);
		const uint32_t ppx = (uint32_t)((int)bcast_f(fpx0, src) + (int)bit), ppy = (uint32_t)bcast_f(fpy, src);
		cur_e = e0 + src; cur_bit = (int)bit;
		if (ahead++ == 0u) continue;
		if (room_l) {
			const uint32_t slot = (uint32_t)__builtin_ctzll(free_l);
			free_l &= free_l - 1ull;
			if (lane == slot) {
				ws.rob[slot].px = ppx; ws.rob[slot].py = ppy; ws.rob[slot].lines_seen = post_seq;
				W_ST_REL(&ws.rob[slot].state, (uint32_t)H_POSTED);
			}
			++post_seq; ++busy_l;
		} else {
			uint32_t d0 = 0, d1 = 0, d2 = 0;
			desk_post_remote(ws, (uint32_t)__builtin_ctzll(free_r), ppx, ppy, d0, d1, d2);
			free_r &= free_r - 1ull;
			++busy_r;
		}
		room_l = busy_l < cap_local && free_l; room_r = busy_r < cap_remote && free_r;
	}
}

template <int MODE, bool WAVE = false, bool TEAM = false, bool REUSE = false>
__device__ void lsd_frame_seq(const Geom &g, const Buffers &b, uint32_t f, float max_gap, const FrameAux &aux, uint32_t *smem, WShared &ws, const uint32_t *cull_tab, const RayDir *dirs,
                              uint32_t win_cap, uint32_t list_cap, const FrameView *tile_view = nullptr) {
	static_assert(!TEAM || (WAVE && (MODE == LSD_MODE_TILE || MODE == LSD_MODE_TILEC)), "helpers read the owner's tile store in LDS");
	const uint32_t lane = threadIdx.x & 63u;
	FrameView v;
	if constexpr (MODE == LSD_MODE_TILE || MODE == LSD_MODE_TILEC) v = *tile_view;
	else frame_setup<MODE, WAVE>(g, b, f, aux, smem, v);
	const Win &m = v.m;
	uint32_t *list = smem + win_cap, *survw = list + list_cap, *wwin = survw + list_cap;
	const uint32_t wy0 = v.wy0, wrows = v.wrows, wwords = v.wwords;
	const int xorg = v.xorg;
	const uint32_t WT = wrows * wwords;
	const bool cull = b.cull_tab != nullptr && max_gap > 0.0f && max_gap <= 49.0f;
	if (lane == 0) { ws.n_lines = 0u; ws.rounds = 0u; ws.steps = 0ull; }
	if (TEAM && lane < SEQ_DESK_ENTRIES) ws.rob[lane].state = H_FREE;
	if (TEAM && lane == 0) { ws.rem_open = 0u; ws.rem_nr = 0u; if (REUSE) ws.frame_no += 1u; }
#ifdef SMH_LSD_WDEBUG
	if (lane < 8u) ws.dbg[lane] = 0u;
	if (lane < 10u) ws.rdbg[lane] = 0ull;
	if (lane == 0) ws.prof[0] = 0ull;
#endif
	const bool remote_ok = TEAM && ws.rem_r != 0ull;
	bool rem_open = false;
	uint32_t rem_nr = 0, rem_asked = 0;
	uint32_t rounds = 0, n_lines = 0, post_seq = 0;
	uint32_t seg_start = 0, cur_e = 0, ahead = 0;
	int cur_bit = -1;
	bool done = false, want = false, desk_valid = false;
	WinTag wtag = {0, 0, false};
#ifdef SMH_LSD_WDEBUG
	unsigned long long sprof[8] = {0, 0, 0, 0, 0, 0, 0, 0}, slast = __builtin_amdgcn_s_memtime(), uprof[12] = {0, 0, 0, 0, 0, 0, 0, 0, 0, 0, 0, 0};
	uint32_t n_units = 0, n_taken = 0;
#define SPROF(i) do { const unsigned long long _n = __builtin_amdgcn_s_memtime(); sprof[i] += _n - slast; slast = _n; } while (0)
#else
#define SPROF(i)
#endif
	while (!done) {
		uint32_t segnext;
		const uint32_t n_list = seq_build_list<MODE>(m, ws, list, survw, list_cap, wy0, wrows, wwords, seg_start, WT, &segnext);
		if (lane == 0) { ws.disp_e = 0u; ws.disp_end = n_list; }
		desk_valid = false;
		__builtin_amdgcn_fence(__ATOMIC_RELEASE, "workgroup");
		__builtin_amdgcn_wave_barrier();
		__builtin_amdgcn_fence(__ATOMIC_ACQUIRE, "workgroup");
		SPROF(0);
		while (true) {
			uint32_t px = 0, py = 0;
			if (!wave_dispatch(ws, list, survw, wy0, wwords, xorg, px, py)) break;
			__builtin_amdgcn_fence(__ATOMIC_RELEASE, "workgroup");
			__builtin_amdgcn_wave_barrier();
			SPROF(1);
			float xs = 0.0f, ys = 0.0f, ex0 = 0.0f, ey0 = 0.0f;
			unsigned long long wkey = 0ull;
			uint32_t st_sum = 0u;
			++rounds;
			if (ahead) --ahead;
			bool have = false;
#ifdef SMH_LSD_WDEBUG
			const unsigned long long t_tk = __builtin_amdgcn_s_memtime();
#endif
			if (TEAM && want) have = desk_take(ws, px, py, xs, ys, wkey, ex0, ey0, st_sum);
#ifdef SMH_LSD_WDEBUG
			if (rem_open) RDBG(7, __builtin_amdgcn_s_memtime() - t_tk);
#endif
#ifdef SMH_LSD_WDEBUG
			if (have) ++n_taken;
			if (!have) seq_cast_candidate<MODE, REUSE>(m, wwin, &wtag, cull_tab, cull, dirs, b.ray_off, max_gap, px, py, xs, ys, wkey, ex0, ey0, st_sum, sprof, slast, uprof, n_units);
#else
			if (!have) seq_cast_candidate<MODE, REUSE>(m, wwin, &wtag, cull_tab, cull, dirs, b.ray_off, max_gap, px, py, xs, ys, wkey, ex0, ey0, st_sum);
#endif
			if (lane == 0) ws.steps += st_sum;
			if (wkey != 0ull && __uint_as_float((uint32_t)(wkey >> 32)) > SMH_LSD_ACCEPT_LEN_SQ) {
				float ex, ey;
				get_centre(m, ex0, ey0, ex, ey);
				if (lane == 0) {
					ws.lines[n_lines][0] = xs; ws.lines[n_lines][1] = ys; ws.lines[n_lines][2] = ex; ws.lines[n_lines][3] = ey;
					const ProxLine pl = prox_line(xs, ys, ex, ey);
					ws.prox_a[n_lines] = pl.a; ws.prox_d[n_lines][0] = pl.dxl; ws.prox_d[n_lines][1] = pl.dyl;
					W_ST_REL(&ws.n_lines, n_lines + 1u);
				}
				++n_lines;
				desk_valid = false;
				__builtin_amdgcn_fence(__ATOMIC_RELEASE, "workgroup");
				__builtin_amdgcn_wave_barrier();
				__builtin_amdgcn_fence(__ATOMIC_ACQUIRE, "workgroup");
				if (n_lines == SMH_LSD_MAX_LINES) { done = true; break; }
			}
			if (TEAM) {
				if (!want && rounds >= SEQ_HELP_AFTER) {
					want = true;
					if (lane == 0) W_ST_REL(&ws.want_set, 1u);
				}
				if (want) {
					if (remote_ok && (rounds & (rem_open ? 7u : 1u)) == 0u) {
						if (rem_open) {
							rem_nr = remote_helpers(ws);
// ... 77 lines not shown
```

squad-mortar-helper_amd/csrc/smh_lsd_wave.inc:

```

#ifndef W_WAVES_PER_EU
#define W_WAVES_PER_EU 4
#endif
#ifndef W_A_BATCHES
#define W_A_BATCHES LSD_A_BATCHES
#endif
#ifndef W_NWIN
#define W_NWIN 4u
#endif
#define W_ROB 16u
#define W_LIST_CAP_MAX 1024u
#define W_WIN_R 67
#define W_WIN_ROWS (2 * W_WIN_R + 1)
#include "smh_window_place.h"
static_assert(W_WIN_R == SMH_WIN_R && LSD_W2_PITCH == SMH_WIN_WORDS, "smh_window_place.h speaks of this window");
#define W_WIN_STRIDE (W_WIN_ROWS * LSD_W2_PITCH + 2u)
#ifndef W_SPEC_MAX
#define W_SPEC_MAX 8u
#endif
static_assert(W_SPEC_MAX + SMH_FARM_RING <= W_ROB && W_NWIN <= W_SPEC_MAX && W_NWIN + SMH_FARM_RING <= W_ROB && (W_ROB & (W_ROB - 1u)) == 0u && W_NWIN <= 32u, "reorder buffer: every local (one window each) and remote (one ring entry each) candidate in flight has a slot");
static_assert(2 * W_WIN_R + 1 + 31 <= 32 * LSD_W2_PITCH, "a window row holds the neighbourhood from a word boundary on");
static_assert(W_WIN_R >= 32 * (int)W_A_BATCHES + 3 && W_WIN_R >= SMH_SECTOR_R + 3, "the window covers the first batches and the culling annulus");
#ifndef W_SPEC_MIN
#define W_SPEC_MIN 2u
// ... 3 lines not shown
#endif
#define W_SPIN_LIMIT_DEFAULT 4000000u

struct WSlot {
	uint32_t px, py;
	uint32_t lines_seen;
	uint32_t state;
	float ptx, pty;
	unsigned long long todo;
	unsigned long long live;
	unsigned long long best;
	float ex, ey;
	uint32_t block;
	uint32_t pending;
	uint32_t steps;
	uint32_t win;
	unsigned long long tag;
#ifdef SMH_LSD_WDEBUG
	unsigned long long t_disp, t_setup, t_done;
#endif
};
enum { W_FREE = 0, W_SETUP = 1, W_CASTING = 2, W_DONE = 3, W_REMOTE = 4 };

struct WShared {
	WSlot rob[W_ROB];
	uint32_t lock;
	uint32_t head, tail;
	uint32_t spec;
	uint32_t disp_e, disp_end;
	uint32_t n_lines, rounds, frame_done;
	unsigned long long steps;
	float lines[SMH_LSD_MAX_LINES][4];
	float prox_a[SMH_LSD_MAX_LINES];
	double prox_d[SMH_LSD_MAX_LINES][2];
	unsigned char stag[W_LIST_CAP_MAX];
	uint32_t scan[LSD_NW];
	uint32_t segnext;
	uint32_t ntiles;
	uint32_t stuck;
	uint32_t win_free;
	uint32_t farm_on, farm_posted, farm_retired, frame_no;
	uint32_t late, want_set, want_tick, pick;
	unsigned long long t0, late_cycles;
	unsigned long long rem_r, rem_store, rem_ctl;
	uint32_t rem_after, rem_tickets, rem_owner, rem_cap;
	uint32_t rem_open, rem_gen, rem_k, rem_nr;
	unsigned long long rem_done;
	uint32_t rem_n, rem_last_div;
	uint32_t rem_flags, rem_pad;
#ifdef SMH_LSD_WDEBUG
	uint32_t dbg[8];
	unsigned long long rdbg[10];
	uint32_t why[4];
	unsigned long long prof[12];
	unsigned long long lat[8];
#endif
};
#ifdef SMH_LSD_WDEBUG
#define WDBG(i, v) do { if ((threadIdx.x & 63u) == 0) atomicAdd(&ws.dbg[i], (v)); } while (0)
#define WPROF(i) do { const unsigned long long _n = __builtin_amdgcn_s_memtime(); wprof[i] += _n - wlast; wlast = _n; } while (0)
#else
#define WDBG(i, v)
#define WPROF(i)
#endif

#define W_LD(p) __hip_atomic_load((p), __ATOMIC_RELAXED, __HIP_MEMORY_SCOPE_WORKGROUP)
#define W_LD_ACQ(p) __hip_atomic_load((p), __ATOMIC_ACQUIRE, __HIP_MEMORY_SCOPE_WORKGROUP)
#define W_ST(p, v) __hip_atomic_store((p), (v), __ATOMIC_RELAXED, __HIP_MEMORY_SCOPE_WORKGROUP)
#define W_ST_REL(p, v) __hip_atomic_store((p), (v), __ATOMIC_RELEASE, __HIP_MEMORY_SCOPE_WORKGROUP)

__device__ __forceinline__ float bcast_f(float v, uint32_t src) { return __uint_as_float((uint32_t)__builtin_amdgcn_readlane((int)__float_as_uint(v), (int)src)); }
__device__ __forceinline__ uint32_t uniform_u32(uint32_t v) { return (uint32_t)__builtin_amdgcn_readfirstlane((int)v); }

__device__ __forceinline__ const LdsByte *window_base(const uint32_t *wwin, uint32_t px, uint32_t py) {
	const int x0 = ((int)px - W_WIN_R) & ~31, y0 = (int)py - W_WIN_R;
	return (const LdsByte *)(const LdsWord *)wwin - (__mul24(y0, (int)(4u * LSD_W2_PITCH)) + ((x0 >> 5) << 2));
}
__device__ __forceinline__ const LdsByte *window_base_at(const uint32_t *wwin, int x0w, int y0) {
	return (const LdsByte *)(const LdsWord *)wwin - (__mul24(y0, (int)(4u * LSD_W2_PITCH)) + (x0w << 2));
}
struct WinTag { int x0w, y0; bool valid; };
__device__ __forceinline__ uint32_t opaque_lane() { uint32_t l = threadIdx.x & 63u; asm volatile("" : "+v"(l)); return l; }
template <bool COMPACT = false, uint32_t ROWS = W_WIN_ROWS, bool TAGGED = false>
__device__ __forceinline__ void cand_setup(const Win &m, uint32_t *wwin, const uint32_t *cull_tab, bool cull, uint32_t px, uint32_t py, float &xs, float &ys, unsigned long long &live,
                                           WinTag *tag = nullptr
#ifdef SMH_LSD_WDEBUG
                                           , unsigned long long *cprof = nullptr
#endif
                                           ) {
	static_assert(ROWS >= W_WIN_ROWS, "a fill covers its own candidate's needed rows");
	const uint32_t lane = opaque_lane();
#ifdef SMH_LSD_WDEBUG
	const unsigned long long c_t0 = __builtin_amdgcn_s_memtime();
#endif
	[[maybe_unused]] bool fill = true;
	if constexpr (TAGGED) {
		const int upx = (int)uniform_u32(px), upy = (int)uniform_u32(py);
		if (tag->valid && smh_window_holds(tag->x0w, tag->y0, (int)ROWS, upx, upy)) fill = false;
		else { smh_window_fresh(upx, upy, &tag->x0w, &tag->y0); tag->valid = true; }
	}
	if (!TAGGED || fill) {
		const int wq0 = TAGGED ? tag->x0w : (((int)px - W_WIN_R) & ~31) >> 5, y0 = TAGGED ? tag->y0 : (int)py - W_WIN_R;
		constexpr uint32_t NIT = (ROWS * LSD_W2_PITCH + 63u) / 64u;
		if (m.tiled) {
#pragma unroll
			for (uint32_t k = 0; k < NIT; ++k) {
				const uint32_t i = lane + 64u * k;
				if (i < ROWS * LSD_W2_PITCH) wwin[i] = 0u;
			}
			const int ty0 = y0 >> 3, ty1 = (y0 + (int)ROWS - 1) >> 3;
			const uint32_t nslots = (uint32_t)(ty1 - ty0 + 1) * LSD_W2_PITCH;
			static_assert(((ROWS + 6u) / 8u + 1u) * LSD_W2_PITCH <= 128u, "two tile slots per lane cover the window (ROWS rows from any row of a tile on touch at most (ROWS + 6) / 8 + 1 tile rows)");
			uint32_t tv[2];
#pragma unroll
			for (uint32_t rnd = 0; rnd < 2u; ++rnd) {
				const uint32_t sidx = lane + 64u * rnd, tr = sidx / LSD_W2_PITCH, tc = sidx - tr * LSD_W2_PITCH;
				const int ty = ty0 + (int)tr, wq = wq0 + (int)tc;
				const bool ok = sidx < nslots && ty >= 0 && (uint32_t)(ty << 3) < m.h && (uint32_t)(wq + 2) < m.t_pitch;
				if constexpr (COMPACT) tv[rnd] = ok ? tilec_number(m, wq, ty) : 0u;
				else tv[rnd] = ok ? (uint32_t)m.t_idx[__mul24(ty, (int)m.t_pitch) + wq] : 0u;
			}
			const uint32_t grp = lane >> 3, row = lane & 7u;
#pragma unroll
			for (uint32_t rnd = 0; rnd < 2u; ++rnd) {
				unsigned long long todo = __ballot(tv[rnd] != 0u);
				while (todo) {
					uint32_t src = 64u;
#pragma unroll
					for (uint32_t k = 0; k < 8u; ++k) {
						const uint32_t p = todo ? (uint32_t)__builtin_ctzll(todo) : 64u;
						todo &= todo - 1ull;
						if (grp == k) src = p;
					}
					const uint32_t tt = (uint32_t)__shfl((int)tv[rnd], (int)(src & 63u));
					const uint32_t sidx = src + 64u * rnd, tr = sidx / LSD_W2_PITCH, tc = sidx - tr * LSD_W2_PITCH;
					const int rr = ((ty0 + (int)tr) << 3) + (int)row - y0;
					if (src < 64u && rr >= 0 && rr < (int)ROWS) wwin[(uint32_t)rr * LSD_W2_PITCH + tc] = (uint32_t)m.t_tiles[(tt << 3) + row];
				}
			}
		} else {
#pragma unroll 1
			for (uint32_t i = lane; i < ROWS * LSD_W2_PITCH; i += 64u) {
				const uint32_t r = i / LSD_W2_PITCH, c = i - r * LSD_W2_PITCH;
				const int b0 = ((wq0 + (int)c) << 5) + m.xbias;
				wwin[i] = __builtin_amdgcn_alignbit(win_word(m, (b0 >> 5) + 1, y0 + (int)r), win_word(m, b0 >> 5, y0 + (int)r), (uint32_t)b0 & 31u);
			}
		}
		if (lane < 2u) wwin[ROWS * LSD_W2_PITCH + lane] = 0u;
		__builtin_amdgcn_fence(__ATOMIC_RELEASE, "workgroup");
		__builtin_amdgcn_wave_barrier();
	}
#ifdef SMH_LSD_WDEBUG
	if (cprof) { cprof[0] += __builtin_amdgcn_s_memtime() - c_t0; if (fill) cprof[2] += 1ull; }
#endif
	Win mw = m;
	mw.w2 = TAGGED ? window_base_at(wwin, tag->x0w, tag->y0) : window_base(wwin, px, py);
	{
		const uint32_t l = lane & 31u, dir = l >> 3, k = l & 7u;
		const float cx = (float)px, cy = (float)py, fk = (float)k;
		bool cond = k < 5u;
		if (dir == 0u) cond = cond && (cx - fk > 0.0f);
		else if (dir == 1u) cond = cond && (cx + fk < (float)(m.w - 1u));
		else if (dir == 2u) cond = cond && (cy - fk > 0.0f);
		else cond = cond && (cy + fk < (float)(m.h - 1u));
		if (cond) {
			const int k_ = (int)k;
			const int xi = (int)px + (dir == 0u ? -k_ : (dir == 1u ? k_ : 0)), yi = (int)py + (dir == 2u ? -k_ : (dir == 3u ? k_ : 0));
			cond = win2_bit(mw, xi, yi) != 0u;
		}
		const uint32_t bits = (uint32_t)__ballot(cond);
		const float nl = (float)__builtin_ctz(~(bits & 0xFFu)), nr = (float)__builtin_ctz(~((bits >> 8) & 0xFFu));
		const float nu = (float)__builtin_ctz(~((bits >> 16) & 0xFFu)), nd = (float)__builtin_ctz(~((bits >> 24) & 0xFFu));
		xs = ((cx - nl) + (cx + nr)) / 2.0f;
		ys = ((cy - nu) + (cy + nd)) / 2.0f;
	}
	live = (1ull << LSD_GROUPS) - 1ull;
#ifdef SMH_LSD_WDEBUG
	const unsigned long long c_t1 = __builtin_amdgcn_s_memtime();
	struct CullTimer { unsigned long long *p, t; __device__ ~CullTimer() { if (p) p[1] += __builtin_amdgcn_s_memtime() - t; } } c_timer{cprof, c_t1};
#endif
	if (cull) {
		unsigned long long acc = 0ull;
		const int fx = (int)floorf(xs), fy = (int)floorf(ys);
		constexpr int ROUNDS = (SMH_CULL_CELLS + 63) / 64;
		uint32_t hits[ROUNDS];
#pragma unroll
		for (int it = 0; it < ROUNDS; ++it) {
			const uint32_t cell = lane + 64u * (uint32_t)it;
			const int yi = fy + (int)(cell >> 2) - SMH_SECTOR_R;
			uint32_t hit = 0;
			if (cell < SMH_CULL_CELLS) {
				const int b0 = fx - SMH_SECTOR_R + (int)((cell & 3u) << 5);
				const uint32_t lo = win2_word(mw, b0 >> 5, yi), hi = win2_word(mw, (b0 >> 5) + 1, yi);
				hit = __builtin_amdgcn_alignbit(hi, lo, (uint32_t)b0 & 31u) & cull_tab[cell];
			}
			hits[it] = hit;
		}
#pragma unroll
		for (int it = 0; it < ROUNDS; ++it) {
			uint32_t hit = hits[it];
			if (hit) {
				const uint32_t cell = lane + 64u * (uint32_t)it;
				const uint8_t *codes = (const uint8_t *)(cull_tab + SMH_CULL_CELLS) + (cell >> 2) * SMH_SECTOR_DIM + ((cell & 3u) << 5);
				while (hit) {
					const uint32_t code = codes[__builtin_ctz(hit)];
					hit &= hit - 1u;
					acc |= code == 0xFFu ? ~0ull : ((2ull << (code >> 6)) - 1ull) << (code & 63u);
				}
			}
		}
		acc = wave_or64(acc);
		live = (acc | (acc >> LSD_GROUPS)) & ((1ull << LSD_GROUPS) - 1ull);
	}
}

__device__ __forceinline__ void slot_merge_best(WSlot &sl, unsigned long long key, float xe, float ye) {
	if (!__any(key != 0ull)) return;
	const uint32_t hi = (uint32_t)(key >> 32), lo = (uint32_t)key;
	const uint32_t mhi = wave_max32_dpp(hi);
	const uint32_t mlo = wave_max32_dpp(hi == mhi ? lo : 0u);
	const unsigned long long wkey = ((unsigned long long)mhi << 32) | mlo;
	if (wkey == 0ull) return;
	const uint32_t src = (uint32_t)__builtin_ctzll(__ballot(key == wkey));
	const float bx = bcast_f(xe, src), by = bcast_f(ye, src);
	if ((threadIdx.x & 63u) == 0u) {
		while (__hip_atomic_exchange(&sl.block, 1u, __ATOMIC_ACQUIRE, __HIP_MEMORY_SCOPE_WORKGROUP) != 0u) __builtin_amdgcn_s_sleep(1);
		if (wkey > sl.best) { sl.best = wkey; sl.ex = bx; sl.ey = by; }
		__hip_atomic_store(&sl.block, 0u, __ATOMIC_RELEASE, __HIP_MEMORY_SCOPE_WORKGROUP);
	}
}

template <int MODE>
__device__ __forceinline__ void sample32(const Win &m, float xs, float ys, float dx, float dy, float xo, float yo, uint32_t &Wm, uint32_t &n) {
	Wm = 0u; n = 0u;
	if (!in_image(m, xo + xs, yo + ys)) return;
	const float xo0 = xo, yo0 = yo;
	float x = 0.0f, y = 0.0f;
	uint32_t W = 0;
#pragma unroll 1
	for (int jj = 0; jj < 4; ++jj) {
		if constexpr (MODE == LSD_MODE_TILE) tile_raw8(m, xs, ys, dx, dy, xo, yo, x, y, W);
		else if constexpr (MODE == LSD_MODE_TILEC) tilec_raw8(m, xs, ys, dx, dy, xo, yo, x, y, W);
		else
#pragma unroll
		for (int j = 0; j < 8; ++j) {
			x = xo + xs; y = yo + ys;
			if (MODE == LSD_MODE_TILE) W = __builtin_amdgcn_alignbit(tile_raw(m, x, y), W, 1);
			else W = __builtin_amdgcn_alignbit(win_raw<false>(m, (int)x, (int)y), W, 1);
			xo += dx; yo += dy;
		}
	}
	Wm = W; n = 32u;
	if (!in_image(m, x, y)) {
		float rx = xo0, ry = yo0;
#pragma unroll 1
		for (n = 0; n < 32u; ++n) {
			if (!in_image(m, rx + xs, ry + ys)) break;
			rx += dx; ry += dy;
		}
	}
}

#define W_PAR_LANES 8u
#ifndef W_PAR_MAX_RAYS
#define W_PAR_MAX_RAYS 8u
#endif

template <int MODE>
__device__ __forceinline__ void long_rays_round(const Win &m, const float *ray_off, uint32_t u, float xs, float ys, float dx, float dy, uint32_t T,
                                                unsigned long long cont, RayState &s, int &status, uint32_t &steps) {
	const uint32_t lane = threadIdx.x & 63u;
	const uint32_t q = lane / W_PAR_LANES, t = lane % W_PAR_LANES;
	unsigned long long c = cont;
	for (uint32_t k = 0; k < q && c; ++k) c &= c - 1ull;
	const bool have = c != 0ull;
	const uint32_t src = have ? (uint32_t)__builtin_ctzll(c) : 0u;
	unsigned long long sel = 0ull;
	{
		unsigned long long cc = cont;
		for (uint32_t k = 0; k < 64u / W_PAR_LANES && cc; ++k) { sel |= cc & (~cc + 1ull); cc &= cc - 1ull; }
	}
	const float rdx = __shfl(dx, (int)src), rdy = __shfl(dy, (int)src);
	const uint32_t rk0 = __shfl(s.k0, (int)src);
	uint32_t g = __shfl(s.g, (int)src);
	uint32_t jg = __shfl(s.gk0, (int)src) >> 5, gj = __shfl(s.gj, (int)src);
	const uint32_t j0 = rk0 >> 5, i = u * 64u + src;
	uint32_t Wm = 0, n = 0;
	if (have) {
		const float2 o = ((const float2 *)ray_off)[(size_t)i * (SMH_RAY_OFF_BATCHES + 1u) + min(j0 + t, SMH_RAY_OFF_BATCHES)];
		sample32<MODE>(m, xs, ys, rdx, rdy, o.x, o.y, Wm, n);
	}
	uint32_t Wt[W_PAR_LANES], nt[W_PAR_LANES];
#pragma unroll
	for (uint32_t k = 0; k < W_PAR_LANES; ++k) { Wt[k] = __shfl(Wm, (int)(q * W_PAR_LANES + k)); nt[k] = __shfl(n, (int)(q * W_PAR_LANES + k)); }
	int st = RAY_CONTINUE;
// ... 650 lines not shown
				uint32_t m[8], sp[8];
				bool any_m, any_s;
				feeds(c, lo, hi, m, sp, any_m, any_s);
				const uint32_t ty = c >> 16, col = (c & 0xFFFFu) + 2u;
				if (any_m) atomicOr(rows0 + (ty * G + (col >> 6)) * 4u + ((col & 63u) >> 5), 1u << (col & 31u));
				if (any_s) atomicOr(rows0 + (ty * G + ((col - 1u) >> 6)) * 4u + (((col - 1u) & 63u) >> 5), 1u << ((col - 1u) & 31u));
			}
		}
	}
	team_barrier<true>();
	uint32_t count = 0;
	for (uint32_t r0 = 0; r0 < nty; r0 += 64u) {
		const uint32_t r = r0 + lane;
		uint32_t *row = rows0 + (ty0 + min(r, nty - 1u)) * G * 4u;
		uint32_t cnt = 0;
		if (r < nty) for (uint32_t h = 0; h < G; ++h) cnt += (uint32_t)__builtin_popcount(row[h * 4u]) + (uint32_t)__builtin_popcount(row[h * 4u + 1u]);
		uint32_t total;
		uint32_t base = count + wave_excl_prefix32(cnt, lane, &total);
		if (r < nty) for (uint32_t h = 0; h < G; ++h) { row[h * 4u + 2u] = base; base += (uint32_t)__builtin_popcount(row[h * 4u]) + (uint32_t)__builtin_popcount(row[h * 4u + 1u]); }
		count += total;
	}
	if (lane == 0) *ntiles = count;
	Win &m = v.m;
	v.gbits = b.bits + (size_t)f * g.bits_stride_w;
	m.w = g.rw; m.h = g.rh; m.wf = (float)g.rw; m.hf = (float)g.rh;
	m.p = smem; m.pitch4 = 0u; m.y_lo = 0; m.xbias = 0; m.rows_hi = 0u; m.cols_hi = 0u;
	m.rows0 = nullptr; m.ylo_f = 0.0f; m.yhi_f = 0.0f;
	m.c_p = (const LdsWord *)smem; m.c_y0 = 0u; m.c_rows = 0u; m.c_pitch4 = 0u;
	m.t_idx = nullptr; m.t_tiles = (const LdsWord *)tiles; m.t_pitch = TWP; m.tiled = true;
	m.tc_rows = (const LdsWord *)rows0; m.tc_groups = G; m.compact = true;
	m.w2 = nullptr;
	v.wy0 = aux.y_min; v.wrows = aux.y_max - aux.y_min + 1u; v.wwords = TW; v.xorg = 0;
	v.c_pitch = 0u; v.c_cap_rows = 0u;
	if (count > tile_cap) { team_barrier<true>(); return 1u; }
	for (uint32_t i = 8u + lane; i < (count + 1u) * 8u; i += 64u) tiles[i] = 0u;
	team_barrier<true>();
	for (uint32_t e0 = 0; e0 < n_g; e0 += 128u) {
#pragma unroll
		for (uint32_t h = 0; h < 2u; ++h) {
			const uint32_t e = e0 + h * 64u + lane;
			if (e < n_g) {
				const uint32_t c = tmp[e];
				const uint4 *src = (const uint4 *)(tg + ((size_t)(c >> 16) * gp + (c & 0xFFFFu)) * 8u);
				const uint4 lo = src[0], hi = src[1];
				uint32_t mm[8], sp[8];
				bool any_m, any_s;
				feeds(c, lo, hi, mm, sp, any_m, any_s);
				const int ty = (int)(c >> 16), wx = (int)(c & 0xFFFFu);
				if (any_m) {
					uint32_t *t = tiles + tilec_number(m, wx, ty) * 8u;
#pragma unroll
					for (uint32_t r = 0; r < 8u; ++r) if (mm[r]) atomicOr(t + r, mm[r]);
				}
				if (any_s) {
					uint32_t *t = tiles + tilec_number(m, wx - 1, ty) * 8u;
#pragma unroll
					for (uint32_t r = 0; r < 8u; ++r) if (sp[r]) atomicOr(t + r, sp[r]);
				}
			}
		}
	}
	team_barrier<true>();
	return 0u;
}

template <int MODE>
__device__ void lsd_frame_wave(const Geom &g, const Buffers &b, uint32_t f, float max_gap, const FrameAux &aux, uint32_t *smem, WShared &ws, const uint32_t *cull_tab, uint32_t win_cap,
                               uint32_t spin_limit, uint32_t list_cap, const FrameView *tile_view = nullptr, FarmFrame *farm = nullptr) {
	const uint32_t tid = threadIdx.x, lane = tid & 63u, wave = tid >> 6, bs = blockDim.x, nw = bs >> 6;
	smhv_frame_result *res = &b.results[f];
	FrameView v;
	if (MODE == LSD_MODE_TILE) v = *tile_view;
	else frame_setup<MODE>(g, b, f, aux, smem, v);
	const Win &m = v.m;
	uint32_t *list = smem + win_cap, *survw = list + list_cap, *wwins = survw + list_cap;
	const uint32_t wy0 = v.wy0, wrows = v.wrows, wwords = v.wwords;
	const int xorg = v.xorg;
	const uint32_t WT = wrows * wwords;
	auto dom_word = [&](uint32_t wi) -> uint32_t {
		const uint32_t r = wi / wwords, c = wi - r * wwords;
		if (MODE == LSD_MODE_TILE) return tile_word(m, (int)c, (int)(wy0 + r));
		return m.p[wi];
	};
	const bool cull = b.cull_tab != nullptr && max_gap > 0.0f && max_gap <= 49.0f;
	const uint32_t epoch = b.co.epoch;
	if (tid == 0) { ws.stuck = 0u; ws.lock = 0u; ws.head = 0u; ws.tail = 0u; ws.spec = 1u; ws.n_lines = 0u; ws.rounds = 0u; ws.frame_done = 0u; ws.steps = 0ull;
	                ws.win_free = (1u << W_NWIN) - 1u; ws.farm_on = 0u; ws.farm_posted = 0u; ws.farm_retired = 0u;
	                ws.late = (farm && (b.lsd_flags & SMH_LSD_LATE_HELP)) ? 1u : 0u; ws.want_set = 0u; ws.want_tick = 0u; ws.t0 = __builtin_amdgcn_s_memtime(); ws.late_cycles = (unsigned long long)b.lsd_late_kc << 10; }
	if (tid < W_ROB) { ws.rob[tid].state = W_FREE; ws.rob[tid].todo = 0ull; }
#ifdef SMH_LSD_WDEBUG
	if (tid < 8) ws.dbg[tid] = 0u;
	if (tid < 4) ws.why[tid] = 0u;
	if (tid < 12) ws.prof[tid] = 0ull;
	if (tid < 8) ws.lat[tid] = 0ull;
#endif
	uint32_t seg_start = 0;
	while (true) {
		const uint32_t range = WT - seg_start;
		const uint32_t per = (range + bs - 1u) / bs;
		const uint32_t my0 = min(seg_start + tid * per, WT), my1 = min(my0 + per, WT);
		uint32_t cnt = 0;
		for (uint32_t wi = my0; wi < my1; ++wi) cnt += dom_word(wi) != 0u ? 1u : 0u;
		uint32_t incl = cnt;
		for (int o = 1; o < 64; o <<= 1) { const uint32_t t = __shfl_up(incl, o); if (lane >= (uint32_t)o) incl += t; }
		if (lane == 63) ws.scan[wave] = incl;
		if (tid == 0) ws.segnext = WT;
		__syncthreads();
		uint32_t wprefix = 0, total = 0;
#pragma unroll
		for (int k = 0; k < LSD_NW; ++k) { const uint32_t s = (uint32_t)k < nw ? ws.scan[k] : 0u; if ((uint32_t)k < wave) wprefix += s; total += s; }
		uint32_t o = wprefix + incl - cnt;
		for (uint32_t wi = my0; wi < my1; ++wi) {
			const uint32_t w = dom_word(wi);
			if (w != 0u) {
				if (o < list_cap) { list[o] = wi; survw[o] = w; ws.stag[o] = 0; }
				else if (o == list_cap) ws.segnext = wi;
				++o;
			}
		}
		if (tid == 0) { ws.disp_e = 0u; ws.disp_end = min(total, list_cap); }
		__syncthreads();
		const uint32_t segnext = ws.segnext;

		uint32_t spins = 0;
#ifdef SMH_LSD_WDEBUG
		unsigned long long wprof[12] = {0, 0, 0, 0, 0, 0, 0, 0, 0, 0, 0, 0}, wlast = __builtin_amdgcn_s_memtime();
		const unsigned long long wstart = wlast;
#endif
		bool finished_one = false;
		while (true) {
			uint32_t slot = 0, unit = 0;
			if (!finished_one && claim_unit(ws, slot, unit)) {
				WDBG(0, 1u);
				WPROF(0);
				WSlot &sl = ws.rob[slot];
				#ifdef SMH_LSD_WDEBUG
				const bool last = unit_cast<MODE>(m, wwins + sl.win * W_WIN_STRIDE, b.ray_off, sl, &ws.win_free, unit, max_gap, wprof);
#else
				const bool last = unit_cast<MODE>(m, wwins + sl.win * W_WIN_STRIDE, b.ray_off, sl, &ws.win_free, unit, max_gap);
#endif
				WPROF(1);
				if (last) { finished_one = true; WPROF(2); }
				spins = 0;
				continue;
			}
			WPROF(0);
			if (!finished_one) {
				const uint32_t h0 = W_LD(&ws.head), t0 = W_LD(&ws.tail);
				bool can_retire = false;
				if (h0 != t0) {
					const WSlot &hs = ws.rob[h0 % W_ROB];
					const uint32_t hst = W_LD(&hs.state);
					can_retire = hst == W_DONE || (hst == W_REMOTE && (g_ld64(&farm->ring[hs.win].done) >> 32) == hs.tag);
				}
				const bool can_dispatch = t0 - h0 < W_LD(&ws.spec) && W_LD(&ws.disp_e) < ws.disp_end &&
				                          (W_LD(&ws.win_free) != 0u || (farm && W_LD(&ws.farm_on) && W_LD(&ws.farm_posted) - W_LD(&ws.farm_retired) < SMH_FARM_RING));
				const bool maybe_over = h0 == t0 && W_LD(&ws.disp_e) >= ws.disp_end;
#ifdef SMH_LSD_WDEBUG
				if (lane == 0 && !can_retire && !can_dispatch) {
					atomicAdd(&ws.why[3], 1u);
					if (!(t0 - h0 < W_LD(&ws.spec))) atomicAdd(&ws.why[0], 1u);
					else if (W_LD(&ws.win_free) == 0u) atomicAdd(&ws.why[1], 1u);
					else if (!(W_LD(&ws.disp_e) < ws.disp_end)) atomicAdd(&ws.why[2], 1u);
				}
#endif
				if (!can_retire && !can_dispatch && !maybe_over && !W_LD(&ws.frame_done)) {
					if (++spins > spin_limit) { if (lane == 0) { W_ST(&ws.stuck, 1u); W_ST(&ws.frame_done, 1u); } break; }
// ... 73 lines not shown
#endif
			if (got) {
				WSlot &sl = ws.rob[slot];
				float xs, ys;
				unsigned long long live;
				cand_setup(m, wwins + uniform_u32(sl.win) * W_WIN_STRIDE, cull_tab, cull, px, py, xs, ys, live);
				WDBG(1, 1u);
#ifdef SMH_LSD_WDEBUG
				if (lane == 0) { sl.t_setup = __builtin_amdgcn_s_memtime(); sl.t_done = sl.t_setup; }
#endif
				if (lane == 0) {
					sl.ptx = xs; sl.pty = ys; sl.live = live; sl.best = 0ull; sl.ex = xs; sl.ey = ys; sl.block = 0u;
					sl.steps = 0u; sl.pending = (uint32_t)__popcll(live);
					if (live) {
						W_ST(&sl.state, (uint32_t)W_CASTING);
						__hip_atomic_store(&sl.todo, live, __ATOMIC_RELEASE, __HIP_MEMORY_SCOPE_WORKGROUP);
					} else {
						__hip_atomic_fetch_or(&ws.win_free, 1u << sl.win, __ATOMIC_RELEASE, __HIP_MEMORY_SCOPE_WORKGROUP);
						W_ST_REL(&sl.state, (uint32_t)W_DONE);
					}
				}
				finished_one = live == 0ull;
				spins = 0;
				WPROF(5);
				continue;
			}
			if (fdone || (exhausted && drained)) break;
			WDBG(4, 1u);
			if (++spins > spin_limit) {
				if (lane == 0) { W_ST(&ws.stuck, 1u); W_ST(&ws.frame_done, 1u); }
				break;
			}
			__builtin_amdgcn_s_sleep(4);
			WPROF(6);
		}
#ifdef SMH_LSD_WDEBUG
		wprof[7] = __builtin_amdgcn_s_memtime() - wstart;
		if (lane == 0) for (int k = 0; k < 12; ++k) atomicAdd(&ws.prof[k], wprof[k]);
#endif
		__syncthreads();
#ifdef SMH_LSD_WDEBUG
		if (tid < ws.disp_end && survw[tid] != 0u) atomicAdd(&ws.dbg[1], 1u);
		__syncthreads();
#endif
		if (ws.frame_done || segnext >= WT) break;
		seg_start = segnext;
		__syncthreads();
	}
	if (farm && tid == 0) g_st64(&farm->owner_done, (unsigned long long)epoch);
	const uint32_t n_lines = ws.n_lines;
	if (tid < n_lines) {
		res->lines[tid].x0 = ws.lines[tid][0]; res->lines[tid].y0 = ws.lines[tid][1];
		res->lines[tid].x1 = ws.lines[tid][2]; res->lines[tid].y1 = ws.lines[tid][3];
	}
	if (tid == 0) { res->n_lines = n_lines; res->rounds = ws.rounds; res->ray_steps = ws.steps; res->status = SMHV_FRAME_OK; }
	if (ws.stuck && tid == 0) {
		res->n_lines = 0; res->rounds = 0xFFFFFFFFu; res->status = SMHV_FRAME_LSD_STUCK;
		BatchError *er = b.err;
		if (er && __hip_atomic_fetch_add(&er->count, 1u, __ATOMIC_RELAXED, __HIP_MEMORY_SCOPE_SYSTEM) == 0u) {
			er->frame = f; er->status = SMHV_FRAME_LSD_STUCK;
			er->info[0] = ws.head; er->info[1] = ws.tail; er->info[2] = ws.disp_e; er->info[3] = ws.disp_end;
			er->info[4] = ws.n_lines; er->info[5] = ws.rounds; er->info[6] = ws.spec; er->info[7] = ws.rob[ws.head % W_ROB].state;
			__threadfence_system();
		}
	}
#ifdef SMH_LSD_WDEBUG
	if (tid < 4) res->meters[28 + tid] = (double)ws.dbg[tid];
	if (tid < 8) res->meters[20 + tid] = (double)ws.prof[tid];
	if (tid < 4) res->angle[16 + tid] = (float)ws.prof[8 + tid];
	if (tid < 4) res->length_px[28 + tid] = (double)ws.lat[tid];
	if (tid < 4) res->length_px[22 + tid] = (double)ws.lat[4 + tid];
	if (tid < 4) res->angle[20 + tid] = (float)ws.why[tid];
	if (tid == 0) { res->length_px[27] = (double)ws.farm_retired; res->length_px[26] = (double)ws.farm_on; }
#endif
}


template <int MODE>
__device__ void lsd_frame_help(const Buffers &b, float max_gap, uint32_t *smem, WShared &ws, const uint32_t *cull_tab, uint32_t win_cap, uint32_t spin_limit, uint32_t list_cap,
                               const FrameView &v, FarmFrame *farm) {
	const uint32_t tid = threadIdx.x, lane = tid & 63u;
	const Win &m = v.m;
	uint32_t *wwins = smem + win_cap + 2u * list_cap;
	const bool cull = b.cull_tab != nullptr && max_gap > 0.0f && max_gap <= 49.0f;
	const uint32_t epoch = b.co.epoch;
	if (tid == 0) { ws.lock = 0u; ws.head = 0u; ws.tail = 0u; ws.win_free = (1u << W_NWIN) - 1u; ws.farm_posted = 0u; ws.frame_done = 0u; }
	if (tid < W_ROB) { ws.rob[tid].state = W_FREE; ws.rob[tid].todo = 0ull; }
	__syncthreads();
	if (tid == 0) g_st64(&farm->attached, (unsigned long long)epoch);
	uint32_t spins = 0;
	bool finished_one = false;
	while (true) {
		uint32_t slot = 0, unit = 0;
		if (!finished_one && claim_unit(ws, slot, unit)) {
			WSlot &sl = ws.rob[slot];
#ifdef SMH_LSD_WDEBUG
			unsigned long long wprof[12];
			const bool last = unit_cast<MODE>(m, wwins + sl.win * W_WIN_STRIDE, b.ray_off, sl, &ws.win_free, unit, max_gap, wprof);
#else
			const bool last = unit_cast<MODE>(m, wwins + sl.win * W_WIN_STRIDE, b.ray_off, sl, &ws.win_free, unit, max_gap);
#endif
			if (last) finished_one = true;
			spins = 0;
			continue;
		}
		const uint32_t k_next = W_LD(&ws.farm_posted);
		if (!finished_one) {
			const uint32_t h0 = W_LD(&ws.head), t0 = W_LD(&ws.tail);
			const bool can_retire = h0 != t0 && W_LD(&ws.rob[h0 % W_ROB].state) == W_DONE;
			const unsigned long long pw = g_ld64(&farm->ring[k_next % SMH_FARM_RING].post);
			const bool can_fetch = W_LD(&ws.win_free) != 0u && (pw >> 24) == (farm_post_word(epoch, k_next, 0u, 0u) >> 24);
			if (!can_retire && !can_fetch) {
				if (h0 == t0 && g_ld64(&farm->owner_done) == (unsigned long long)epoch) break;
				if (++spins > spin_limit) break;
				__builtin_amdgcn_s_sleep(16);
				continue;
			}
		}
		finished_one = false;
		uint32_t got_lock = 0;
		if (lane == 0) got_lock = __hip_atomic_exchange(&ws.lock, 1u, __ATOMIC_ACQUIRE, __HIP_MEMORY_SCOPE_WORKGROUP) == 0u ? 1u : 0u;
		if (uniform_u32(got_lock) == 0u) { __builtin_amdgcn_s_sleep(8); continue; }
		__builtin_amdgcn_fence(__ATOMIC_ACQUIRE, "workgroup");
		uint32_t head = W_LD(&ws.head);
		const uint32_t tail = W_LD(&ws.tail);
		while (head != tail) {
			WSlot &sl = ws.rob[head % W_ROB];
			if (W_LD_ACQ(&sl.state) != W_DONE) break;
			if (lane == 0) {
				FarmEntry *e = &farm->ring[(uint32_t)(sl.tag >> 32)];
				g_st64(&e->best, sl.best);
				g_st64(&e->end, ((unsigned long long)__float_as_uint(sl.ey) << 32) | __float_as_uint(sl.ex));
				g_st64(&e->start, ((unsigned long long)__float_as_uint(sl.pty) << 32) | __float_as_uint(sl.ptx));
				asm volatile("s_waitcnt vmcnt(0)" ::: "memory");
				g_st64(&e->done, ((unsigned long long)(uint32_t)sl.tag << 32) | sl.steps);
				W_ST(&sl.state, (uint32_t)W_FREE);
			}
			++head;
		}
		if (lane == 0) W_ST(&ws.head, head);
		bool got = false;
		uint32_t px = 0, py = 0;
		const uint32_t k = W_LD(&ws.farm_posted), wfree = W_LD(&ws.win_free);
		if (wfree != 0u) {
			const unsigned long long pw = g_ld64(&farm->ring[k % SMH_FARM_RING].post);
			if ((pw >> 24) == (farm_post_word(epoch, k, 0u, 0u) >> 24)) {
				got = true;
				px = (uint32_t)pw & 0xFFFu; py = (uint32_t)(pw >> 12) & 0xFFFu;
				slot = tail % W_ROB;
				if (lane == 0) {
					WSlot &sl = ws.rob[slot];
					const uint32_t w = (uint32_t)__builtin_ctz(wfree);
					__hip_atomic_fetch_and(&ws.win_free, ~(1u << w), __ATOMIC_RELAXED, __HIP_MEMORY_SCOPE_WORKGROUP);
					sl.px = px; sl.py = py; sl.win = w;
					sl.tag = ((unsigned long long)(k % SMH_FARM_RING) << 32) | farm_done_tag(epoch, k);
					W_ST(&ws.farm_posted, k + 1u);
					W_ST(&sl.state, (uint32_t)W_SETUP);
					W_ST_REL(&ws.tail, tail + 1u);
				}
			}
		}
		__builtin_amdgcn_fence(__ATOMIC_RELEASE, "workgroup");
		if (lane == 0) __hip_atomic_store(&ws.lock, 0u, __ATOMIC_RELEASE, __HIP_MEMORY_SCOPE_WORKGROUP);
		if (got) {
			WSlot &sl = ws.rob[slot];
			float xs, ys;
			unsigned long long live;
			cand_setup(m, wwins + uniform_u32(sl.win) * W_WIN_STRIDE, cull_tab, cull, px, py, xs, ys, live);
			if (lane == 0) {
				sl.ptx = xs; sl.pty = ys; sl.live = live; sl.best = 0ull; sl.ex = xs; sl.ey = ys; sl.block = 0u;
				sl.steps = 0u; sl.pending = (uint32_t)__popcll(live);
				if (live) {
					W_ST(&sl.state, (uint32_t)W_CASTING);
					__hip_atomic_store(&sl.todo, live, __ATOMIC_RELEASE, __HIP_MEMORY_SCOPE_WORKGROUP);
				} else {
					__hip_atomic_fetch_or(&ws.win_free, 1u << sl.win, __ATOMIC_RELEASE, __HIP_MEMORY_SCOPE_WORKGROUP);
					W_ST_REL(&sl.state, (uint32_t)W_DONE);
				}
			}
			finished_one = live == 0ull;
			spins = 0;
		}
	}
}

__device__ __forceinline__ uint32_t late_pick(const Buffers &b, uint32_t n_frames, uint32_t self, WShared &ws) {
	const uint32_t epoch = b.co.epoch;
	const unsigned long long tag = (unsigned long long)(epoch & 0xFFFFu) << 48;
	for (uint32_t attempt = 0; attempt < 3u; ++attempt) {
		if (threadIdx.x == 0) ws.pick = 0u;
		__syncthreads();
		uint32_t key = 0u;
		for (uint32_t f = threadIdx.x; f < n_frames; f += blockDim.x) {
			if (f == self) continue;
			const unsigned long long w = g_ld64(&b.farm[f].want);
			if ((w & 0xFFFF000000000000ull) != tag) continue;
			const uint32_t left = (uint32_t)min(w & 0xFFFFFFFFull, 0xFFFFEull);
			if (left < LATE_MIN_LEFT) continue;
			if (g_ld64(&b.farm[f].claimed) == (unsigned long long)epoch || g_ld64(&b.farm[f].owner_done) == (unsigned long long)epoch) continue;
			key = max(key, ((left + 1u) << 12) | (f & 0xFFFu));
		}
		key = wave_max32_dpp(key);
		if ((threadIdx.x & 63u) == 0u && key) atomicMax(&ws.pick, key);
		__syncthreads();
		const uint32_t best = ws.pick;
		__syncthreads();
		if (!best) return 0xFFFFFFFFu;
		const uint32_t f = best & 0xFFFu;
		if (threadIdx.x == 0) {
			unsigned long long expect = g_ld64(&b.farm[f].claimed);
			bool won = false;
			if (expect != (unsigned long long)epoch)
				won = __hip_atomic_compare_exchange_strong(&b.farm[f].claimed, &expect, (unsigned long long)epoch, __ATOMIC_RELAXED, __ATOMIC_RELAXED, __HIP_MEMORY_SCOPE_AGENT);
			ws.pick = won ? 1u : 0u;
		}
		__syncthreads();
		const bool won = ws.pick != 0u;
		__syncthreads();
		if (won) return f;
	}
	return 0xFFFFFFFFu;
}

struct TileKernelArgs { Geom g; Buffers b; float max_gap; uint32_t tile_cap; uint32_t spin_limit; uint32_t list_cap; uint32_t n_frames; };
__device__ __attribute__((noinline)) void lsd_frame_global(const TileKernelArgs *ka, uint32_t f, uint32_t *smem, WShared *wsp, const uint32_t *cull_tab) {
	const Geom g = ka->g;
	const Buffers b = ka->b;
	const FrameAux aux = b.aux[f];
	lsd_frame_wave<LSD_MODE_GLOBAL>(g, b, f, ka->max_gap, aux, smem, *wsp, cull_tab, 0u, ka->spin_limit, ka->list_cap);
}

#define LSD_TILE_BS 1024
__global__ void __launch_bounds__(LSD_TILE_BS) __attribute__((amdgpu_waves_per_eu(W_WAVES_PER_EU, W_WAVES_PER_EU))) k_lsd_tile(Geom g, Buffers b, float max_gap, uint32_t tile_cap, uint32_t spin_limit, uint32_t list_cap, uint32_t n_frames) {
	extern __shared__ __attribute__((aligned(16))) uint32_t smem[];
	__shared__ WShared ws;
	__shared__ uint32_t cull_tab[SMH_CULL_TAB_WORDS];
#ifdef SMH_LSD_FAT
	asm volatile("; register footprint experiment" ::: SMH_LSD_FAT);
#endif
	const bool cull = b.cull_tab != nullptr && max_gap > 0.0f && max_gap <= 49.0f;
	const uint32_t f = blockIdx.x;
	const FrameAux aux = b.aux[f];
	const TileKernelArgs *ka = (const TileKernelArgs *)__builtin_amdgcn_kernarg_segment_ptr();
	const bool record = (b.rec_stages & SMH_REC_ON) != 0u;
	if (!aux.open || aux.n_mask_px == 0) {
		if (threadIdx.x == 0) { b.results[f].n_lines = 0; b.results[f].rounds = 0; b.results[f].ray_steps = 0; b.results[f].status = SMHV_FRAME_OK; }
		if (record) { __syncthreads(); frame_record_tail(&ka->g, &ka->b, f); }
		return;
	}
	if (cull) for (uint32_t i = threadIdx.x; i < SMH_CULL_TAB_WORDS; i += blockDim.x) cull_tab[i] = b.cull_tab[i];
	const bool late = b.farm && (b.lsd_flags & SMH_LSD_LATE_HELP) && n_frames <= 4096u;
	FarmFrame *farm = late ? &b.farm[f] : nullptr;
	FrameView v;
	if (frame_setup_tile(g, b, f, aux, smem, tile_cap, &ws.ntiles, v)) lsd_frame_wave<LSD_MODE_TILE>(g, b, f, max_gap, aux, smem, ws, cull_tab, tile_mask_words(g.rw, g.rh, tile_cap), spin_limit, list_cap, &v, farm);
	else lsd_frame_global(ka, f, smem, &ws, cull_tab);
	if (record) { __syncthreads(); frame_record_tail(&ka->g, &ka->b, f); }
	if (late) {
		__syncthreads();
		const uint32_t t = late_pick(b, n_frames, f, ws);
		if (t == 0xFFFFFFFFu) return;
		const FrameAux aux_t = b.aux[t];
		FrameView vt;
		if (!frame_setup_tile(g, b, t, aux_t, smem, tile_cap, &ws.ntiles, vt)) return;
		if (g_ld64(&b.farm[t].owner_done) == (unsigned long long)b.co.epoch) return;
		lsd_frame_help<LSD_MODE_TILE>(b, max_gap, smem, ws, cull_tab, tile_mask_words(g.rw, g.rh, tile_cap), spin_limit, list_cap, vt, &b.farm[t]);
	}
}
```

squad-mortar-helper_amd/csrc/smh_runtime.cpp:

```cpp
#include <hip/hip_runtime.h>

#include <atomic>
#include <condition_variable>
#include <deque>
#include <thread>
#include <cmath>
#include <cstdarg>
#include <cstdio>
#include <cstdlib>
#include <cstring>
#include <ctime>
#include <sched.h>
#include <pthread.h>
#include <cctype>
#include <mutex>
#include <vector>
#include <new>
#include <string>

#include "smh_consts.h"
#include "smh_kernels.h"

using namespace smh;

// ... 223 lines not shown
	uint8_t *d_ui_tight = nullptr;
	size_t d_ui_tight_cap = 0;
	uint8_t *d_fire = nullptr, *h_fire = nullptr;
	size_t fire_cap = 0;
	std::mutex fire_mu;
	uint32_t ui_turn = 0;
	bool ui_pending = false, minimap_cached = false;
	uint32_t W = 0, H = 0;
	bool have_frame = false;
	uint8_t *d_frame = nullptr;
	size_t d_frame_cap = 0;
	const uint8_t *frame_ptr = nullptr;
	smhv_batch *fb = nullptr;
	uint8_t *h_ocr = nullptr, *h_scales = nullptr;
	uint8_t *h_stage[3] = {nullptr, nullptr, nullptr};
	size_t h_stage_cap[3] = {0, 0, 0};
	smhv_frame_result *h_res = nullptr;
	FrameAux *h_aux = nullptr;
	uint32_t *h_bars = nullptr;
	bool cropped = false, map_open = false, isolated = false, mask_valid = false, scales_valid = false;
	static constexpr int SECTOR_CACHE = 8;
	uint32_t sector_T[SECTOR_CACHE] = {};
	uint32_t *sector_tab[SECTOR_CACHE] = {};
	int sector_n = 0;
	float *d_ray_off = nullptr;
	uint32_t *d_side = nullptr;
	std::atomic<uint64_t> tt_ns[SMHV_TRAIT_CALLS] = {}, tt_calls[SMHV_TRAIT_CALLS] = {};
	std::mutex mu;
	std::atomic<int> refs{1};
	std::atomic<bool> closed{false};
};

static std::mutex g_ctx_mu;
static std::vector<smhv_ctx *> g_ctx_open;

static void ctx_release(smhv_ctx *c) {
	if (c && c->refs.fetch_sub(1, std::memory_order_acq_rel) == 1) delete c;
}
#define CTX_OPEN(c)                                                                                          \
	do {                                                                                                     \
		if (!(c) || (c)->closed.load(std::memory_order_acquire)) return fail(SMHV_E_INVALID, "the context was shut down"); \
	} while (0)

static void logf(smhv_ctx *c, int lvl, const char *fmt, ...) {
	if (!c || !c->log) return;
	char buf[512];
	va_list ap;
	va_start(ap, fmt);
	vsnprintf(buf, sizeof buf, fmt, ap);
	va_end(ap);
	c->log(lvl, buf);
}

static uint8_t unit_code(unsigned long long m) {
	const uint32_t NU = 57;
	m &= (1ull << NU) - 1ull;
	uint32_t first = 0, cnt = NU, best_gap = 0;
	for (uint32_t st = 0; st < NU; ++st) {
		if (!((m >> st) & 1ull)) continue;
		uint32_t gap = 0;
		while (gap < NU - 1 && !((m >> ((st + 1 + gap) % NU)) & 1ull)) ++gap;
		if (gap > best_gap) { best_gap = gap; first = (st + 1 + gap) % NU; cnt = NU - gap; }
	}
	if (best_gap == 0 || cnt > 4) return 0xFF;
	return (uint8_t)(first | ((cnt - 1) << 6));
}

static int sector_table_for(smhv_ctx *c, uint32_t max_gap, hipStream_t s, Buffers *bf) {
	bf->cull_tab = nullptr;
	if (max_gap == 0 || max_gap > 49) return SMHV_OK;
	std::lock_guard<std::mutex> lk(c->mu);
	for (int i = 0; i < c->sector_n; ++i)
		if (c->sector_T[i] == max_gap) { bf->cull_tab = c->sector_tab[i]; return SMHV_OK; }
	if (c->sector_n == smhv_ctx::SECTOR_CACHE) return SMHV_OK;
	unsigned long long *d_dense = nullptr;
	HIPCHK(hipMalloc((void **)&d_dense, sizeof(unsigned long long) * SMH_SECTOR_ENTRIES));
	std::vector<unsigned long long> dense(SMH_SECTOR_ENTRIES);
	hipError_t e = launch_build_sector_table(d_dense, max_gap, s);
	if (e == hipSuccess) e = hipMemcpyAsync(dense.data(), d_dense, sizeof(unsigned long long) * SMH_SECTOR_ENTRIES, hipMemcpyDeviceToHost, s);
	if (e == hipSuccess) e = hipStreamSynchronize(s);
	(void)hipFree(d_dense);
	if (e != hipSuccess) return fail(SMHV_E_HIP, "sector table: %s", hipGetErrorString(e));
	std::vector<uint32_t> cells(SMH_CULL_TAB_WORDS, 0u);
	uint8_t *codes = (uint8_t *)&cells[SMH_CULL_CELLS];
	for (uint32_t row = 0; row < SMH_SECTOR_DIM; ++row)
		for (uint32_t col = 0; col < SMH_SECTOR_DIM; ++col) {
			const unsigned long long m = dense[row * SMH_SECTOR_DIM + col] & ((1ull << 57) - 1ull);
			if (!m) continue;
			cells[row * 4 + (col >> 5)] |= 1u << (col & 31u);
			codes[row * SMH_SECTOR_DIM + col] = unit_code(m);
		}
	uint32_t *d = nullptr;
	HIPCHK(hipMalloc((void **)&d, sizeof(uint32_t) * cells.size()));
	e = hipMemcpy(d, cells.data(), sizeof(uint32_t) * cells.size(), hipMemcpyHostToDevice);
	if (e != hipSuccess) { (void)hipFree(d); return fail(SMHV_E_HIP, "sector table: %s", hipGetErrorString(e)); }
	c->sector_T[c->sector_n] = max_gap; c->sector_tab[c->sector_n] = d; c->sector_n++;
	bf->cull_tab = d;
	return SMHV_OK;
}

static Buffers make_buffers(smhv_batch *b, const uint8_t *frames, uint32_t result_slot) {
	Buffers bf;
	bf.err = b->d_err;
	bf.farm = b->d_farm; bf.rec_stages = 0u; bf.rec_bars = nullptr; bf.lsd_flags = 0u; bf.lsd_late_kc = 0u;
	bf.cull_tab = nullptr;
	bf.ray_off = b->ctx->d_ray_off;
	bf.frames = frames;
	bf.ui = b->d_ui; bf.mask = b->d_mask; bf.ocr = b->d_ocr; bf.scales = b->d_scales;
	bf.bits = b->d_bits; bf.aux = b->d_aux;
	bf.tiled = b->d_tiled; bf.occ = b->d_occ;
	bf.results = b->d_results + result_slot;
	bf.anchors = b->d_anchors;
	bf.firing = nullptr;
	bf.co.ctl = nullptr;
	bf.co.coop = (LsdCoop *)(b->d_lsd_ctl + sizeof(LsdCtl));
	bf.co.req = b->d_lsd_req;
	bf.co.cache = b->d_lsd_cache;
	if (++b->lsd_epoch == 0) {
		(void)hipMemset(b->d_lsd_cache, 0, sizeof(LsdCacheEntry) * SMH_LSD_CACHE_SLOTS * (size_t)b->max_frames);
		b->lsd_epoch = 1;
	}
	bf.co.epoch = b->lsd_epoch;
	return bf;
}

extern "C" SMHV_API int smhv_init(int device, smhv_log_fn log, smhv_ctx **out) {
	if (!out) return fail(SMHV_E_INVALID, "null output");
	*out = nullptr;
	int count = 0;
	hipError_t e = hipGetDeviceCount(&count);
	if (e != hipSuccess || count <= 0) return fail(SMHV_E_NO_DEVICE, "no HIP device available (%s)", e == hipSuccess ? "count = 0" : hipGetErrorString(e));
	if (device < 0 || device >= count) return fail(SMHV_E_NO_DEVICE, "device %d out of range (%d devices)", device, count);
	HIPCHK(hipSetDevice(device));
	hipDeviceProp_t prop;
	HIPCHK(hipGetDeviceProperties(&prop, device));
	if (strncmp(prop.gcnArchName, "gfx950", 6) != 0)
		return fail(SMHV_E_NO_DEVICE, "device %d is %s; this library carries gfx950 (MI355X) code objects only", device, prop.gcnArchName);
	smhv_ctx *c = new (std::nothrow) smhv_ctx();
	if (!c) return fail(SMHV_E_INVALID, "out of host memory");
	c->device = device; c->log = log;
	hipError_t he = hipStreamCreateWithFlags(&c->s_main, hipStreamNonBlocking);
	if (he == hipSuccess) he = hipStreamCreateWithFlags(&c->s_markers, hipStreamNonBlocking);
	if (he == hipSuccess) he = hipStreamCreateWithFlags(&c->s_scales, hipStreamNonBlocking);
	if (he == hipSuccess) he = hipStreamCreateWithFlags(&c->s_ui, hipStreamNonBlocking);
	if (he == hipSuccess) he = hipEventCreateWithFlags(&c->ev_map, hipEventDisableTiming);
	for (int i = 0; i < 2 && he == hipSuccess; ++i) he = hipEventCreateWithFlags(&c->ev_ui[i], hipEventDisableTiming);
	for (int i = 0; i < 3 && he == hipSuccess; ++i) he = hipEventCreateWithFlags(&c->ev_ui_part[i], hipEventDisableTiming);
	if (he == hipSuccess) he = hipHostMalloc((void **)&c->h_res, sizeof(smhv_frame_result) * 4);
	if (he == hipSuccess) he = hipHostMalloc((void **)&c->h_aux, sizeof(FrameAux));
	if (he == hipSuccess) he = hipHostMalloc((void **)&c->h_bars, sizeof(uint32_t) * SMHV_MAX_SCALES * 4 + sizeof(smhv_anchors));
	if (he == hipSuccess) he = hipMalloc((void **)&c->d_ray_off, sizeof(float) * 2 * SMH_LSD_RAYS * (SMH_RAY_OFF_BATCHES + 1));
	if (he == hipSuccess) he = launch_build_ray_offsets(c->d_ray_off, c->s_main);
	if (he == hipSuccess) he = hipStreamSynchronize(c->s_main);
	if (he != hipSuccess) {
		smhv_shutdown(c);
		return fail(SMHV_E_HIP, "context setup failed: %s", hipGetErrorString(he));
	}
	logf(c, 3, "smh_vision_hip ready on device %d (%s, %d CUs)", device, prop.gcnArchName, prop.multiProcessorCount);
	{ std::lock_guard<std::mutex> lk(g_ctx_mu); g_ctx_open.push_back(c); }
	*out = c;
	return SMHV_OK;
}

extern "C" SMHV_API void smhv_shutdown(smhv_ctx *c) {
	if (!c || c->closed.exchange(true, std::memory_order_acq_rel)) return;
	{
		std::lock_guard<std::mutex> lk(g_ctx_mu);
		for (size_t i = 0; i < g_ctx_open.size(); ++i) if (g_ctx_open[i] == c) { g_ctx_open.erase(g_ctx_open.begin() + (long)i); break; }
	}
	(void)hipSetDevice(c->device);
	(void)hipDeviceSynchronize();
	if (c->fb) { smhv_batch_destroy(c->fb); c->fb = nullptr; }
// ... 2527 lines not shown
```

squad-mortar-helper_amd/csrc/smh_service.inc:

```
#pragma once

struct SvcKernelArgs { Geom g; SvcParams p; };
#ifdef __HIP_DEVICE_COMPILE__
typedef const __attribute__((address_space(4))) SvcSlot *SvcSlotPtr;
typedef const __attribute__((address_space(4))) SvcKernelArgs *SvcKernelArgsPtr;
#else
typedef const SvcSlot *SvcSlotPtr;
typedef const SvcKernelArgs *SvcKernelArgsPtr;
#endif
__device__ __forceinline__ SvcKernelArgsPtr svc_args(const void *ka) {
	const unsigned long long v = (unsigned long long)(uintptr_t)ka;
	const uint32_t lo = (uint32_t)__builtin_amdgcn_readfirstlane((int)(uint32_t)v), hi = (uint32_t)__builtin_amdgcn_readfirstlane((int)(uint32_t)(v >> 32));
	return (SvcKernelArgsPtr)(uintptr_t)(((unsigned long long)hi << 32) | lo);
}

#define SVC_WS_WORDS ((uint32_t)((sizeof(WShared) + 15u) / 16u * 4u))
#define SVC_POLL_SLEEP 64

__device__ __forceinline__ uint32_t svc_ld(const uint32_t *p) { return __hip_atomic_load(p, __ATOMIC_RELAXED, __HIP_MEMORY_SCOPE_AGENT); }

__device__ __forceinline__ uint32_t *lds_ptr(uint32_t byte_off) { return (uint32_t *)(LdsWord *)(uintptr_t)uniform_u32(byte_off); }
__device__ __forceinline__ uint32_t lds_off(const void *p) { return (uint32_t)(uintptr_t)(const LdsByte *)p; }

template <bool COMPACT>
__device__ __attribute__((noinline)) void svc_frame_global(const void *kargs, uint32_t slot, uint32_t f, uint32_t part_off, uint32_t cull_off, uint32_t dirs_off) {
	SvcKernelArgsPtr ka = svc_args(kargs);
	slot = uniform_u32(slot); f = uniform_u32(f);
	uint32_t *part = lds_ptr(part_off);
	const Geom g = ka->g;
	const Buffers b = ((SvcSlotPtr)(ka->p.slots + slot))->b;
	const FrameAux aux = b.aux[f];
	lsd_frame_seq<LSD_MODE_GLOBAL, true, false, SVC_WIN_REUSE(COMPACT)>(g, b, f, ka->p.max_gap, aux, part + SVC_WS_WORDS, *(WShared *)part, lds_ptr(cull_off), (const RayDir *)lds_ptr(dirs_off), 0u, ka->p.list_cap);
}

template <bool COMPACT>
__device__ __attribute__((noinline)) unsigned long long svc_frame(const void *kargs, uint32_t slot, uint32_t f, uint32_t part_off, uint32_t cull_off, uint32_t dirs_off) {
	SvcKernelArgsPtr ka = svc_args(kargs);
	slot = uniform_u32(slot); f = uniform_u32(f);
	uint32_t *part = lds_ptr(part_off);
	const Geom g = ka->g;
	const Buffers b = ((SvcSlotPtr)(ka->p.slots + slot))->b;
	const FrameAux aux = b.aux[f];
	WShared &ws = *(WShared *)part;
	uint32_t *smem = part + SVC_WS_WORDS;
	if (!aux.open || aux.n_mask_px == 0) {
		if ((threadIdx.x & 63u) == 0) { b.results[f].n_lines = 0; b.results[f].rounds = 0; b.results[f].ray_steps = 0; b.results[f].status = SMHV_FRAME_OK; }
	} else {
		const uint32_t tile_cap = ka->p.tile_cap;
		if ((threadIdx.x & 63u) == 0) {
			SvcSlot *sl = ka->p.slots + slot;
			ws.rem_done = (unsigned long long)(uintptr_t)&sl->done;
			ws.rem_n = __hip_atomic_load(&sl->n, __ATOMIC_RELAXED, __HIP_MEMORY_SCOPE_AGENT);
		}
		FrameView v;
		bool fits;
		if constexpr (COMPACT) {
			uint32_t rc = 2u;
			if (b.tiled && aux.tiles && !(ka->p.flags & 32u)) rc = frame_setup_tilec_occ(g, b, f, aux, smem, tile_cap, &ws.ntiles, v, smem + tilec_mask_words(g.rw, g.rh, tile_cap), 2u * ka->p.list_cap + SVC_WIN_STRIDE(true));
			fits = rc == 2u ? frame_setup_tilec(g, b, f, aux, smem, tile_cap, &ws.ntiles, v) : rc == 0u;
		} else {
			uint32_t rc = 2u;
			if (b.tiled && aux.tiles && !(ka->p.flags & 32u)) rc = frame_setup_tile_occ(g, b, f, aux, smem, tile_cap, &ws.ntiles, v, smem + tile_mask_words(g.rw, g.rh, tile_cap), 2u * ka->p.list_cap + SVC_WIN_STRIDE(false));
			fits = rc == 2u ? frame_setup_tile<true>(g, b, f, aux, smem, tile_cap, &ws.ntiles, v) : rc == 0u;
		}
		if (fits) {
			if constexpr (COMPACT) lsd_frame_seq<LSD_MODE_TILEC, true, true, SVC_WIN_REUSE(true)>(g, b, f, ka->p.max_gap, aux, smem, ws, lds_ptr(cull_off), (const RayDir *)lds_ptr(dirs_off), tilec_mask_words(g.rw, g.rh, tile_cap), ka->p.list_cap, &v);
			else lsd_frame_seq<LSD_MODE_TILE, true, true, SVC_WIN_REUSE(false)>(g, b, f, ka->p.max_gap, aux, smem, ws, lds_ptr(cull_off), (const RayDir *)lds_ptr(dirs_off), tile_mask_words(g.rw, g.rh, tile_cap), ka->p.list_cap, &v);
		} else svc_frame_global<COMPACT>(kargs, slot, f, part_off, cull_off, dirs_off);
	}
	const unsigned long long t_search_end = __builtin_amdgcn_s_memtime();
	if (b.rec_stages & SMH_REC_ON) frame_record_tail_wave(&((const SvcKernelArgs *)kargs)->g, &((const SvcSlot *)(ka->p.slots + slot))->b, f);
	return t_search_end;
}

#define SVC_HELP_IDLE_POLLS 160u
template <bool COMPACT>
__device__ __attribute__((noinline)) void svc_help(const void *kargs, uint32_t owner_off, uint32_t my_off, uint32_t cull_off, uint32_t dirs_off) {
	SvcKernelArgsPtr ka = svc_args(kargs);
	uint32_t *opart = lds_ptr(owner_off), *mpart = lds_ptr(my_off);
	WShared &wo = *(WShared *)opart;
	const uint32_t lane = threadIdx.x & 63u;
	uint32_t ok = 0;
	if (lane == 0 && W_LD_ACQ(&wo.want_set) && W_LD(&wo.late) < SEQ_MAX_HELPERS) {
		const uint32_t prev = __hip_atomic_fetch_add(&wo.late, 1u, __ATOMIC_ACQ_REL, __HIP_MEMORY_SCOPE_WORKGROUP);
		if (prev < SEQ_MAX_HELPERS && W_LD_ACQ(&wo.want_set)) ok = 1u;
		else __hip_atomic_fetch_sub(&wo.late, 1u, __ATOMIC_RELEASE, __HIP_MEMORY_SCOPE_WORKGROUP);
	}
	if (!uniform_u32(ok)) return;
	const uint32_t rw = ka->g.rw, rh = ka->g.rh, tile_cap = ka->p.tile_cap, list_cap = ka->p.list_cap;
	const float max_gap = ka->p.max_gap;
	const bool cull = ka->p.cull_tab != nullptr && max_gap > 0.0f && max_gap <= 49.0f;
	const float *ray_off = ka->p.ray_off;
	Win m;
	if constexpr (COMPACT) tilec_win(m, rw, rh, opart + SVC_WS_WORDS, tile_cap); else tile_win(m, rw, rh, opart + SVC_WS_WORDS, tile_cap);
	uint32_t *wwin = mpart + SVC_WS_WORDS + (COMPACT ? tilec_mask_words(rw, rh, tile_cap) : tile_mask_words(rw, rh, tile_cap)) + 2u * list_cap;
	const uint32_t *cull_tab = lds_ptr(cull_off);
	const RayDir *dirs = (const RayDir *)lds_ptr(dirs_off);
	uint32_t idle = 0;
	WinTag wtag = {0, 0, false};
	uint32_t wframe = 0u;
	while (uniform_u32(W_LD_ACQ(&wo.want_set))) {
		uint32_t key = 0u;
		if (lane < SEQ_HELP_SLOTS && W_LD_ACQ(&wo.rob[lane].state) == (uint32_t)H_POSTED) key = ~((wo.rob[lane].lines_seen << 2) | lane);
		key = wave_max32_dpp(key);
		if (!key) {
			if (++idle > SVC_HELP_IDLE_POLLS) break;
			__builtin_amdgcn_s_sleep(8);
			continue;
		}
		WSlot &sl = wo.rob[~key & 3u];
		uint32_t got = 0;
		if (lane == 0) { uint32_t expect = H_POSTED; got = __hip_atomic_compare_exchange_strong(&sl.state, &expect, (uint32_t)H_TAKEN, __ATOMIC_ACQ_REL, __ATOMIC_RELAXED, __HIP_MEMORY_SCOPE_WORKGROUP) ? 1u : 0u; }
		if (!uniform_u32(got)) continue;
		idle = 0;
		const uint32_t px = uniform_u32(sl.px), py = uniform_u32(sl.py);
		if (SVC_WIN_REUSE(COMPACT)) {
			const uint32_t oframe = uniform_u32(W_LD(&wo.frame_no));
			if (oframe != wframe) { wframe = oframe; wtag.valid = false; }
		}
		float xs, ys, ex0, ey0;
		unsigned long long wkey;
		uint32_t st_sum;
#ifdef SMH_LSD_WDEBUG
		unsigned long long sprof[8] = {0, 0, 0, 0, 0, 0, 0, 0}, slast = __builtin_amdgcn_s_memtime(), uprof[12] = {0, 0, 0, 0, 0, 0, 0, 0, 0, 0, 0, 0};
		uint32_t n_units = 0;
		seq_cast_candidate<COMPACT ? LSD_MODE_TILEC : LSD_MODE_TILE, SVC_WIN_REUSE(COMPACT)>(m, wwin, &wtag, cull_tab, cull, dirs, ray_off, max_gap, px, py, xs, ys, wkey, ex0, ey0, st_sum, sprof, slast, uprof, n_units);
#else
		seq_cast_candidate<COMPACT ? LSD_MODE_TILEC : LSD_MODE_TILE, SVC_WIN_REUSE(COMPACT)>(m, wwin, &wtag, cull_tab, cull, dirs, ray_off, max_gap, px, py, xs, ys, wkey, ex0, ey0, st_sum);
#endif
		if (lane == 0) {
			sl.ptx = xs; sl.pty = ys; sl.best = wkey; sl.ex = ex0; sl.ey = ey0; sl.steps = st_sum;
			W_ST_REL(&sl.state, (uint32_t)H_DONE);
		}
	}
	if (lane == 0) __hip_atomic_fetch_sub(&wo.late, 1u, __ATOMIC_RELEASE, __HIP_MEMORY_SCOPE_WORKGROUP);
}

#define SVC_REMOTE_IDLE_POLLS 12u
#define SVC_REMOTE_IDLE_POLLS_FREE 600u
#define SVC_REMOTE_MAX_HELPERS 12u
template <bool COMPACT>
__device__ __attribute__((noinline)) void svc_help_remote(const void *kargs, uint32_t ticket, uint32_t my_off, uint32_t cull_off, uint32_t dirs_off) {
	SvcKernelArgsPtr ka = svc_args(kargs);
	ticket = uniform_u32(ticket);
	const uint32_t owner = ticket & 0xFFFFu, gen16 = ticket >> 16;
	SvcRemote *r = ka->p.remote + owner;
	const uint32_t lane = threadIdx.x & 63u;
	uint32_t ok = 0, gen = 0;
	if (lane == 0) {
		unsigned long long st = g_ld64(&r->state);
		while ((st & SVC_REMOTE_OPEN) && ((uint32_t)(st >> 32) & 0xFFFFu) == gen16 && ((uint32_t)st & 0x7FFFFFFFu) < SVC_REMOTE_MAX_HELPERS) {
			if (__hip_atomic_compare_exchange_strong(&r->state, &st, st + 1ull, __ATOMIC_ACQ_REL, __ATOMIC_RELAXED, __HIP_MEMORY_SCOPE_AGENT)) { ok = 1u; gen = (uint32_t)(st >> 32); break; }
		}
	}
	if (!uniform_u32(ok)) return;
	gen = uniform_u32(gen);
	if (lane == 0) __hip_atomic_fetch_add(&ka->p.ctl->stat_attached, 1u, __ATOMIC_RELAXED, __HIP_MEMORY_SCOPE_AGENT);
	__builtin_amdgcn_fence(__ATOMIC_ACQUIRE, "agent");
	const uint32_t rw = ka->g.rw, rh = ka->g.rh, tile_cap = ka->p.tile_cap, list_cap = ka->p.list_cap;
	const uint32_t ntiles = min(uniform_u32((uint32_t)g_ld64(&r->info)), tile_cap);
	uint32_t *mpart = lds_ptr(my_off), *store = mpart + SVC_WS_WORDS;
	{
		const uint4 *src = (const uint4 *)(ka->p.remote_store + (size_t)owner * ka->p.remote_store_words);
		uint4 *dst = (uint4 *)store;
		for (uint32_t i = lane; i < (ntiles + 1u) * 2u; i += 64u) dst[i] = src[i];
		const uint32_t q0 = (tile_cap + 1u) * 2u, nq = ((COMPACT ? tilec_idx_words(rw, rh) : tile_idx_words(rw, rh)) + 3u) / 4u;
		for (uint32_t i = lane; i < nq; i += 64u) dst[q0 + i] = src[q0 + i];
	}
	wave_lds_sync();
	const float max_gap = ka->p.max_gap;
	const bool cull = ka->p.cull_tab != nullptr && max_gap > 0.0f && max_gap <= 49.0f;
	const float *ray_off = ka->p.ray_off;
	Win m;
	if constexpr (COMPACT) tilec_win(m, rw, rh, store, tile_cap); else tile_win(m, rw, rh, store, tile_cap);
	uint32_t *wwin = store + (COMPACT ? tilec_mask_words(rw, rh, tile_cap) : tile_mask_words(rw, rh, tile_cap)) + 2u * list_cap;
	const uint32_t *cull_tab = lds_ptr(cull_off);
	const RayDir *dirs = (const RayDir *)lds_ptr(dirs_off);
	WinTag wtag = {0, 0, false};
	uint32_t idle = 0, n_cast = 0, n_polls = 0, n_empty = 0, n_lost = 0, exit_idle = 0;
	unsigned long long t_cast = 0ull;
	const unsigned long long t_att = __builtin_amdgcn_s_memtime();
	while (true) {
		++n_polls;
		const unsigned long long st = g_ld64(&r->state);
		unsigned long long pw = 0ull, cw = 0ull;
		if (lane < SVC_REMOTE_RING) { pw = g_ld64(&r->ring[lane].post); cw = g_ld64(&r->ring[lane].claim); }
		if (!(uniform_u32((uint32_t)st) & (uint32_t)SVC_REMOTE_OPEN) || uniform_u32((uint32_t)(st >> 32)) != gen) break;
		const uint32_t pk = (uint32_t)(pw >> 32);
		const bool open_post = lane < SVC_REMOTE_RING && pk != 0u && (unsigned long long)pk > cw;
		const uint32_t key = wave_max32_dpp(open_post ? ~pk : 0u);
		if (!key) {
			const int32_t waiting = (int32_t)uniform_u32((uint32_t)__hip_atomic_load(&ka->p.ctl->avail, __ATOMIC_RELAXED, __HIP_MEMORY_SCOPE_AGENT));
			++n_empty;
			if (++idle > (waiting > 0 ? SVC_REMOTE_IDLE_POLLS : SVC_REMOTE_IDLE_POLLS_FREE)) { exit_idle = 1u; break; }
			if (idle < 4u) __builtin_amdgcn_s_sleep(24); else __builtin_amdgcn_s_sleep(72);
			continue;
		}
		const uint32_t k = ~key;
		const uint32_t e = (uint32_t)__builtin_ctzll(__ballot(open_post && pk == k));
		uint32_t mine = 0;
		if (lane == 0) mine = __hip_atomic_fetch_max(&r->ring[e].claim, (unsigned long long)k, __ATOMIC_RELAXED, __HIP_MEMORY_SCOPE_AGENT) < (unsigned long long)k ? 1u : 0u;
		if (!uniform_u32(mine)) { ++n_lost; continue; }
		idle = 0;
		const unsigned long long t_c0 = __builtin_amdgcn_s_memtime();
		const uint32_t pxy = (uint32_t)__builtin_amdgcn_readlane((int)(uint32_t)pw, (int)e);
		const uint32_t px = pxy & 0xFFFFu, py = pxy >> 16;
		float xs, ys, ex0, ey0;
		unsigned long long wkey;
		uint32_t st_sum;
#ifdef SMH_LSD_WDEBUG
		unsigned long long sprof[8] = {0, 0, 0, 0, 0, 0, 0, 0}, slast = __builtin_amdgcn_s_memtime(), uprof[12] = {0, 0, 0, 0, 0, 0, 0, 0, 0, 0, 0, 0};
		uint32_t n_units = 0;
		seq_cast_candidate<COMPACT ? LSD_MODE_TILEC : LSD_MODE_TILE, SVC_WIN_REUSE(COMPACT)>(m, wwin, &wtag, cull_tab, cull, dirs, ray_off, max_gap, px, py, xs, ys, wkey, ex0, ey0, st_sum, sprof, slast, uprof, n_units);
#else
		seq_cast_candidate<COMPACT ? LSD_MODE_TILEC : LSD_MODE_TILE, SVC_WIN_REUSE(COMPACT)>(m, wwin, &wtag, cull_tab, cull, dirs, ray_off, max_gap, px, py, xs, ys, wkey, ex0, ey0, st_sum);
#endif
		++n_cast;
		t_cast += __builtin_amdgcn_s_memtime() - t_c0;
		if (lane == 0) {
			SvcRemoteEntry *en = &r->ring[e];
			const rem_u32x4 a = {k, st_sum, (uint32_t)(wkey >> 32), (uint32_t)wkey};
			const rem_u32x4 b = {k, __float_as_uint(ex0), __float_as_uint(ey0), ((uint32_t)(ys * 2.0f) << 16) | ((uint32_t)(xs * 2.0f) & 0xFFFFu)};
			g_st128(en->res_a, a);
			g_st128(en->res_b, b);
		}
	}
	asm volatile("s_waitcnt vmcnt(0)" ::: "memory");
	if (lane == 0) {
		__hip_atomic_fetch_sub(&r->state, 1ull, __ATOMIC_RELEASE, __HIP_MEMORY_SCOPE_AGENT);
		SvcCtl *ctl = ka->p.ctl;
		__hip_atomic_fetch_add(&ctl->stat_remote, n_cast, __ATOMIC_RELAXED, __HIP_MEMORY_SCOPE_AGENT);
		__hip_atomic_fetch_add(&ctl->stat_h_polls, n_polls, __ATOMIC_RELAXED, __HIP_MEMORY_SCOPE_AGENT);
		__hip_atomic_fetch_add(&ctl->stat_h_empty, n_empty, __ATOMIC_RELAXED, __HIP_MEMORY_SCOPE_AGENT);
		__hip_atomic_fetch_add(&ctl->stat_h_lost, n_lost, __ATOMIC_RELAXED, __HIP_MEMORY_SCOPE_AGENT);
		__hip_atomic_fetch_add(exit_idle ? &ctl->stat_h_idle_exit : &ctl->stat_h_closed_exit, 1u, __ATOMIC_RELAXED, __HIP_MEMORY_SCOPE_AGENT);
		__hip_atomic_fetch_add(&ctl->stat_h_cycles, __builtin_amdgcn_s_memtime() - t_att, __ATOMIC_RELAXED, __HIP_MEMORY_SCOPE_AGENT);
		__hip_atomic_fetch_add(&ctl->stat_h_cast_cycles, t_cast, __ATOMIC_RELAXED, __HIP_MEMORY_SCOPE_AGENT);
	}
}

__device__ __forceinline__ uint32_t svc_sibling_in_need(uint32_t *smem, uint32_t part_words, uint32_t nw, uint32_t me) {
	for (uint32_t w = 0; w < nw; ++w) {
		if (w == me) continue;
		const WShared &wsib = *(const WShared *)(smem + w * part_words);
		if (uniform_u32(W_LD(&wsib.want_set)) && uniform_u32(W_LD(&wsib.late)) < SEQ_MAX_HELPERS) return lds_off(smem + w * part_words);
	}
	return 0xFFFFFFFFu;
}

__device__ __forceinline__ uint32_t svc_pop(const SvcParams &p, uint32_t *team_smem, uint32_t nw, uint32_t me, bool checker, uint32_t *help_ticket) {
	const uint32_t lane = threadIdx.x & 63u;
	SvcCtl *ctl = p.ctl;
	const unsigned long long t_idle0 = __builtin_amdgcn_s_memtime();
	uint32_t polls = 0;
// ... 196 lines not shown
```

Before: 632,700.

## Factor sector-cull rule into shared header with optional chained two-annulus culling

Moves the sector culling table rule into a shared host/device header and adds an optional second (middle) annulus, so a ray group stays live only if pixels are seen in both annuli when SMH_CULL_CHAIN is defined. The wave-level cull setup is restructured: all window words and masks are loaded first, then hit codes are decoded four at a time to batch LDS lookups. Without SMH_CULL_CHAIN the annulus count stays at one and the mode reduces to the old behaviour. The batched decode adds some register pressure and extra instructions for wasted slots.

```diff
diff --git a/squad-mortar-helper_amd/csrc/smh_cull_rule.h b/squad-mortar-helper_amd/csrc/smh_cull_rule.h
--- /dev/null
+++ b/squad-mortar-helper_amd/csrc/smh_cull_rule.h
@@ -0,0 +1,71 @@
+#pragma once
+#include <math.h>
+#include <stdint.h>
+#if defined(__HIPCC__) || defined(__CUDACC__)
+#define SMH_CR_FN __host__ __device__ inline
+#else
+#define SMH_CR_FN inline
+#endif
+
+#define SMH_CULL_ACCEPT_STEP 50
+#define SMH_CULL_UNITS 57
+#define SMH_CULL_RHO (0.7072 + 0.7072 + 0.05)
+#define SMH_CULL_DELTA_MARGIN 0.2
+#define SMH_CULL_IN_OUTER (1ull << 62)
+#define SMH_CULL_IN_MIDDLE (1ull << 63)
+#ifdef SMH_CULL_CHAIN
+#define SMH_CULL_ANNULI 2
+#else
+#define SMH_CULL_ANNULI 1
+#endif
+
+SMH_CR_FN bool smh_cull_window(uint32_t T, int a, int *lo, int *hi) {
+	const int t = (int)T, top = SMH_CULL_ACCEPT_STEP - a * (t + 1);
+	*hi = top;
+	*lo = top - t < 0 ? 0 : top - t;
+	if (a == 0) return true;
+#ifdef SMH_CULL_CHAIN
+	return a == 1 && top - t >= 1;
+#else
+	return false;
+#endif
+}
+SMH_CR_FN bool smh_cull_chained(uint32_t T) { int lo, hi; return smh_cull_window(T, 1, &lo, &hi); }
+
+SMH_CR_FN bool smh_cull_in_annulus(int lo, int hi, int ox, int oy) {
+	const double r0 = sqrt((double)(ox * ox + oy * oy));
+	return r0 >= (double)lo - SMH_CULL_RHO && r0 <= (double)hi + SMH_CULL_RHO;
+}
+
+SMH_CR_FN unsigned long long smh_cull_units(int ox, int oy) {
+	const double rho = SMH_CULL_RHO;
+	const double r0 = sqrt((double)(ox * ox + oy * oy));
+	if (r0 <= rho) return (1ull << SMH_CULL_UNITS) - 1ull;
+	const double PI = 3.14159265358979323846;
+	double phi = atan2((double)oy, (double)ox) * 180.0 / PI;
+	if (phi < 0.0) phi += 360.0;
+	const double delta = asin(rho / r0 > 1.0 ? 1.0 : rho / r0) * 180.0 / PI + SMH_CULL_DELTA_MARGIN;
+	unsigned long long m = 0ull;
+	for (int u = 0; u < SMH_CULL_UNITS; ++u) {
+		const double a0 = 6.4 * u, a1 = 6.4 * u + 6.3;
+		bool hit = false;
+		for (int wrap = -1; wrap <= 1 && !hit; ++wrap) {
+			const double lo = phi - delta + 360.0 * wrap, hi = phi + delta + 360.0 * wrap;
+			hit = !(hi < a0 || lo > a1);
+		}
+		if (hit) m |= 1ull << u;
+	}
+	return m;
+}
+
+SMH_CR_FN unsigned long long smh_cull_entry(uint32_t T, int ox, int oy) {
+	unsigned long long in = 0ull;
+	int lo, hi;
+	if (smh_cull_window(T, 0, &lo, &hi) && smh_cull_in_annulus(lo, hi, ox, oy)) in |= SMH_CULL_IN_OUTER;
+	if (smh_cull_window(T, 1, &lo, &hi) && smh_cull_in_annulus(lo, hi, ox, oy)) in |= SMH_CULL_IN_MIDDLE;
+	return in ? in | smh_cull_units(ox, oy) : 0ull;
+}
+
+SMH_CR_FN unsigned long long smh_cull_live(unsigned long long seen_outer, unsigned long long seen_middle, bool chained) {
+	return chained ? seen_outer & seen_middle : seen_outer;
+}
diff --git a/squad-mortar-helper_amd/csrc/smh_kernels.h b/squad-mortar-helper_amd/csrc/smh_kernels.h
--- a/squad-mortar-helper_amd/csrc/smh_kernels.h
+++ b/squad-mortar-helper_amd/csrc/smh_kernels.h
@@ -280,11 +280,14 @@
 
 #define SMH_RAY_OFF_BATCHES 168u
 
+#include "smh_cull_rule.h"
 #define SMH_SECTOR_R 52
 #define SMH_SECTOR_DIM (2 * SMH_SECTOR_R + 1)
 #define SMH_SECTOR_ENTRIES (SMH_SECTOR_DIM * SMH_SECTOR_DIM)
 #define SMH_CULL_CELLS (SMH_SECTOR_DIM * 4)
-#define SMH_CULL_TAB_WORDS (SMH_CULL_CELLS + (SMH_SECTOR_ENTRIES + 3) / 4)
+#define SMH_CULL_TAB_WORDS (SMH_CULL_ANNULI * SMH_CULL_CELLS + (SMH_SECTOR_ENTRIES + 3) / 4)
+#define SMH_CULL_CODES(tab) ((const uint8_t *)((tab) + SMH_CULL_ANNULI * SMH_CULL_CELLS))
+#define SMH_CULL_MID_CELL(tab, cell) (SMH_CULL_ANNULI == 2 ? (tab)[(SMH_CULL_ANNULI - 1) * SMH_CULL_CELLS + (cell)] : 0u)
 
 #define SVC_MAX_SLOTS 32u
 struct SvcSlot {
diff --git a/squad-mortar-helper_amd/csrc/smh_lsd.hip b/squad-mortar-helper_amd/csrc/smh_lsd.hip
--- a/squad-mortar-helper_amd/csrc/smh_lsd.hip
+++ b/squad-mortar-helper_amd/csrc/smh_lsd.hip
@@ -144,6 +144,21 @@
 }
 __device__ __forceinline__ uint32_t win2_word(const Win &m, int wq, int yi) { return *(const LdsWord *)(m.w2 + __mul24(yi, (int)(4u * LSD_W2_PITCH)) + (wq << 2)); }
 __device__ __forceinline__ uint32_t win2_bit(const Win &m, int xi, int yi) { return (win2_word(m, xi >> 5, yi) >> ((uint32_t)xi & 31u)) & 1u; }
+
+__device__ __forceinline__ uint32_t cull_mode_for(const uint32_t *tab, float max_gap) {
+	if (tab == nullptr || !(max_gap > 0.0f && max_gap <= 49.0f)) return 0u;
+	return smh_cull_chained((uint32_t)ceilf(max_gap)) ? 2u : 1u;
+}
+__device__ __forceinline__ unsigned long long cull_units_of(uint32_t hit, const uint8_t *codes) {
+	unsigned long long acc = 0ull;
+	while (hit) {
+		const uint32_t code = codes[__builtin_ctz(hit)];
+		hit &= hit - 1u;
+		acc |= code == 0xFFu ? ~0ull : ((2ull << (code >> 6)) - 1ull) << (code & 63u);
+	}
+	return acc;
+}
+__device__ __forceinline__ unsigned long long cull_fold(unsigned long long acc) { return (acc | (acc >> LSD_GROUPS)) & ((1ull << LSD_GROUPS) - 1ull); }
 
 __device__ __forceinline__ uint32_t win_bit(const Win &m, int xi, int yi) {
 	if (m.tiled) return ((m.compact ? tilec_word(m, xi >> 5, yi) : tile_word(m, xi >> 5, yi)) >> ((uint32_t)xi & 31u)) & 1u;
@@ -353,6 +368,7 @@
 	uint32_t nlive;
 	unsigned short ulist[LSD_UNITS];
 	unsigned long long live[LSD_C];
+	unsigned long long live_mid[LSD_C];
 	float lines[SMH_LSD_MAX_LINES][4];
 	float prox_a[SMH_LSD_MAX_LINES];
 	double prox_d[SMH_LSD_MAX_LINES][2];
@@ -691,7 +707,7 @@
 __device__ __forceinline__ void group_reset(LsdShared &sh, uint32_t nc, bool cull) {
 	const uint32_t tid = threadIdx.x;
 	if (tid < nc * LSD_GROUPS) { sh.unit_key[tid] = 0ull; sh.unit_kmax[tid] = 0u; }
-	if (tid < LSD_C) { sh.cand_best[tid] = 0ull; sh.cand_steps[tid] = 0u; sh.cand_kmax[tid] = 0u; sh.live[tid] = cull ? 0ull : ~0ull; }
+	if (tid < LSD_C) { sh.cand_best[tid] = 0ull; sh.cand_steps[tid] = 0u; sh.cand_kmax[tid] = 0u; sh.live[tid] = cull ? 0ull : ~0ull; sh.live_mid[tid] = 0ull; }
 	if (tid == 0) { sh.qtail = 0u; sh.unit_next = LSD_NW; sh.nlive = 0u; sh.cached = 0u;
 #ifdef SMH_LSD_PROFILE
 		sh.exp_far = 0u; sh.exp_units = 0u;
@@ -700,7 +716,7 @@
 }
 
 template <int MODE>
-__device__ __forceinline__ void cast_group(const Win &m, LsdShared &sh, uint32_t *queue, const uint32_t *cull_tab, uint32_t nc, bool cull, float max_gap,
+__device__ __forceinline__ void cast_group(const Win &m, LsdShared &sh, uint32_t *queue, const uint32_t *cull_tab, uint32_t nc, uint32_t cull, float max_gap,
                                            unsigned long long *prof_t = nullptr) {
 	const uint32_t tid = threadIdx.x;
 #ifdef SMH_LSD_PROFILE
@@ -732,24 +748,22 @@
 		for (uint32_t id = tid; id < nc * SMH_CULL_CELLS; id += LSD_BS) {
 			const uint32_t c = id / SMH_CULL_CELLS, cell = id - c * SMH_CULL_CELLS;
 			if ((cached >> c) & 1u) continue;
+			const uint32_t m_out = cull_tab[cell], m_mid = SMH_CULL_MID_CELL(cull_tab, cell);
 			const int fx = (int)floorf(sh.cand_pt[c][0]), fy = (int)floorf(sh.cand_pt[c][1]);
 			const int yi = fy + (int)(cell >> 2) - SMH_SECTOR_R;
 			if ((uint32_t)yi >= m.h) continue;
 			const int b0 = fx - SMH_SECTOR_R + (int)((cell & 3u) << 5) + m.xbias;
 			const uint32_t lo = win_word(m, b0 >> 5, yi), hi = win_word(m, (b0 >> 5) + 1, yi);
-			uint32_t hit = __builtin_amdgcn_alignbit(hi, lo, (uint32_t)b0 & 31u) & cull_tab[cell];
-			if (hit) {
-				const uint8_t *codes = (const uint8_t *)(cull_tab + SMH_CULL_CELLS) + (cell >> 2) * SMH_SECTOR_DIM + ((cell & 3u) << 5);
-				unsigned long long acc = 0ull;
-				while (hit) {
-					const uint32_t code = codes[__builtin_ctz(hit)];
-					hit &= hit - 1u;
-					acc |= code == 0xFFu ? ~0ull : ((2ull << (code >> 6)) - 1ull) << (code & 63u);
-				}
-				atomicOr(&sh.live[c], (acc | (acc >> LSD_GROUPS)) & ((1ull << LSD_GROUPS) - 1ull));
-			}
+			const uint32_t px32 = __builtin_amdgcn_alignbit(hi, lo, (uint32_t)b0 & 31u);
+			const uint8_t *codes = SMH_CULL_CODES(cull_tab) + (cell >> 2) * SMH_SECTOR_DIM + ((cell & 3u) << 5);
+			if (px32 & m_out) atomicOr(&sh.live[c], cull_fold(cull_units_of(px32 & m_out, codes)));
+			if (cull == 2u && (px32 & m_mid)) atomicOr(&sh.live_mid[c], cull_fold(cull_units_of(px32 & m_mid, codes)));
 		}
 		__syncthreads();
+		if (cull == 2u) {
+			if (tid < nc && !((cached >> tid) & 1u)) sh.live[tid] = smh_cull_live(sh.live[tid], sh.live_mid[tid], true);
+			__syncthreads();
+		}
 	}
 	if (tid < nc * LSD_GROUPS) {
 		const uint32_t c = tid / LSD_GROUPS;
@@ -796,7 +810,7 @@
 		return;
 	}
 
-	const bool cull = b.cull_tab != nullptr && max_gap > 0.0f && max_gap <= 49.0f;
+	const uint32_t cull = cull_mode_for(b.cull_tab, max_gap);
 	const uint32_t *ring = co ? b.co.req + (size_t)f * SMH_LSD_REQ_CAP : nullptr;
 	const LsdCacheEntry *ctab = co ? b.co.cache + (size_t)f * SMH_LSD_CACHE_SLOTS : nullptr;
 	if (tid == 0) { sh.req_tail = 0u; sh.posted_hi = 0u; sh.posted_new = 0u; sh.helpers_seen = 0u; sh.head_seen = 0u; if (co) st_relaxed(&co->mode1, (uint32_t)MODE + 1u); }
@@ -977,7 +991,7 @@
 template <int MODE>
 __device__ void lsd_help(const Geom &g, const Buffers &b, uint32_t n_frames, float max_gap, uint32_t *smem, LsdShared &sh, uint32_t *cull_tab, bool have_cull_tab) {
 	const uint32_t tid = threadIdx.x;
-	const bool cull = b.cull_tab != nullptr && max_gap > 0.0f && max_gap <= 49.0f;
+	const uint32_t cull = cull_mode_for(b.cull_tab, max_gap);
 	if (cull && !have_cull_tab) for (uint32_t i = tid; i < SMH_CULL_TAB_WORDS; i += LSD_BS) cull_tab[i] = b.cull_tab[i];
 	uint32_t *queue = smem + LSD_WIN_WORDS_CAP + LSD_LIST_CAP;
 	uint32_t idle = 0;
@@ -1095,7 +1109,7 @@
 		bool record = mode == 0 && (b.rec_stages & SMH_REC_ON) != 0u && !mine && MODE == LSD_MODE_ROWS;
 		if (mine && lsd_mode_for(g, aux) != MODE) mine = false;
 		if (mine) {
-			const bool cull = mode == 0 && b.cull_tab != nullptr && max_gap > 0.0f && max_gap <= 49.0f;
+			const uint32_t cull = mode == 0 ? cull_mode_for(b.cull_tab, max_gap) : 0u;
 			if (cull) { for (uint32_t i = threadIdx.x; i < SMH_CULL_TAB_WORDS; i += LSD_BS) cull_tab[i] = b.cull_tab[i]; have_tab = true; }
 			lsd_frame<MODE>(g, b, f, max_gap, mode, spx, spy, aux, smem, sh, cull_tab, (COOP && coop) ? &b.co.coop[f] : nullptr);
 			record = mode == 0 && (b.rec_stages & SMH_REC_ON) != 0u;
@@ -1130,30 +1144,7 @@
 	const uint32_t i = blockIdx.x * blockDim.x + threadIdx.x;
 	if (i >= SMH_SECTOR_ENTRIES) return;
 	const int oy = (int)(i / SMH_SECTOR_DIM) - SMH_SECTOR_R, ox = (int)(i % SMH_SECTOR_DIM) - SMH_SECTOR_R;
-	const double rho = 0.7072 + 0.7072 + 0.05;
-	const double kmin = T >= 50u ? 0.0 : (double)(50u - T), kmax = 50.0;
-	const double r0 = sqrt((double)(ox * ox + oy * oy));
-	unsigned long long m = 0ull;
-	if (r0 >= kmin - rho && r0 <= kmax + rho) {
-		if (r0 <= rho) {
-			m = ~0ull;
-		} else {
-			const double PI = 3.14159265358979323846;
-			double phi = atan2((double)oy, (double)ox) * 180.0 / PI;
-			if (phi < 0.0) phi += 360.0;
-			const double delta = asin(rho / r0 > 1.0 ? 1.0 : rho / r0) * 180.0 / PI + 0.2;
-			for (int u = 0; u < LSD_GROUPS_HOST; ++u) {
-				const double a0 = 6.4 * u, a1 = 6.4 * u + 6.3;
-				bool hit = false;
-				for (int wrap = -1; wrap <= 1 && !hit; ++wrap) {
-					const double lo = phi - delta + 360.0 * wrap, hi = phi + delta + 360.0 * wrap;
-					hit = !(hi < a0 || lo > a1);
-				}
-				if (hit) m |= 1ull << u;
-			}
-		}
-	}
-	tab[i] = m;
+	tab[i] = smh_cull_entry(T, ox, oy);
 }
 
 size_t lsd_lds_bytes() { return LSD_DYN_LDS_BYTES; }
@@ -1349,7 +1340,7 @@
 }
 
 hipError_t launch_build_sector_table(unsigned long long *d_tab, uint32_t T, hipStream_t s) {
-	static_assert(LSD_GROUPS == LSD_GROUPS_HOST && LSD_GROUPS <= 64, "sector masks are 64-bit");
+	static_assert(LSD_GROUPS == LSD_GROUPS_HOST && LSD_GROUPS == SMH_CULL_UNITS && LSD_GROUPS <= 62, "sector masks are 64-bit, and smh_cull_rule.h keeps two flags above the units");
 	hipLaunchKernelGGL(k_build_sector_table, dim3((SMH_SECTOR_ENTRIES + 255) / 256), dim3(256), 0, s, d_tab, T);
 	return hipGetLastError();
 }
diff --git a/squad-mortar-helper_amd/csrc/smh_lsd_seq.inc b/squad-mortar-helper_amd/csrc/smh_lsd_seq.inc
--- a/squad-mortar-helper_amd/csrc/smh_lsd_seq.inc
+++ b/squad-mortar-helper_amd/csrc/smh_lsd_seq.inc
@@ -222,7 +222,7 @@
 #define SVC_WIN_STRIDE(compact) (SVC_WIN_ROWS(compact) * LSD_W2_PITCH + 2u)
 
 template <int MODE, bool REUSE = false>
-__device__ __forceinline__ void seq_cast_candidate(const Win &m, uint32_t *wwin, WinTag *tag, const uint32_t *cull_tab, bool cull, const RayDir *dirs, const float *ray_off, float max_gap,
+__device__ __forceinline__ void seq_cast_candidate(const Win &m, uint32_t *wwin, WinTag *tag, const uint32_t *cull_tab, uint32_t cull, const RayDir *dirs, const float *ray_off, float max_gap,
                                                    uint32_t px, uint32_t py, float &xs, float &ys, unsigned long long &wkey, float &ex0, float &ey0, uint32_t &steps_sum
 #ifdef SMH_LSD_WDEBUG
                                                    , unsigned long long *sprof, unsigned long long &slast, unsigned long long *uprof, uint32_t &n_units
@@ -496,7 +496,7 @@
 	const uint32_t wy0 = v.wy0, wrows = v.wrows, wwords = v.wwords;
 	const int xorg = v.xorg;
 	const uint32_t WT = wrows * wwords;
-	const bool cull = b.cull_tab != nullptr && max_gap > 0.0f && max_gap <= 49.0f;
+	const uint32_t cull = cull_mode_for(b.cull_tab, max_gap);
 	if (lane == 0) { ws.n_lines = 0u; ws.rounds = 0u; ws.steps = 0ull; }
 	if (TEAM && lane < SEQ_DESK_ENTRIES) ws.rob[lane].state = H_FREE;
 	if (TEAM && lane == 0) { ws.rem_open = 0u; ws.rem_nr = 0u; if (REUSE) ws.frame_no += 1u; }
diff --git a/squad-mortar-helper_amd/csrc/smh_lsd_wave.inc b/squad-mortar-helper_amd/csrc/smh_lsd_wave.inc
--- a/squad-mortar-helper_amd/csrc/smh_lsd_wave.inc
+++ b/squad-mortar-helper_amd/csrc/smh_lsd_wave.inc
@@ -109,7 +109,7 @@
 struct WinTag { int x0w, y0; bool valid; };
 __device__ __forceinline__ uint32_t opaque_lane() { uint32_t l = threadIdx.x & 63u; asm volatile("" : "+v"(l)); return l; }
 template <bool COMPACT = false, uint32_t ROWS = W_WIN_ROWS, bool TAGGED = false>
-__device__ __forceinline__ void cand_setup(const Win &m, uint32_t *wwin, const uint32_t *cull_tab, bool cull, uint32_t px, uint32_t py, float &xs, float &ys, unsigned long long &live,
+__device__ __forceinline__ void cand_setup(const Win &m, uint32_t *wwin, const uint32_t *cull_tab, uint32_t cull, uint32_t px, uint32_t py, float &xs, float &ys, unsigned long long &live,
                                            WinTag *tag = nullptr
 #ifdef SMH_LSD_WDEBUG
                                            , unsigned long long *cprof = nullptr
@@ -207,37 +207,46 @@
 	struct CullTimer { unsigned long long *p, t; __device__ ~CullTimer() { if (p) p[1] += __builtin_amdgcn_s_memtime() - t; } } c_timer{cprof, c_t1};
 #endif
 	if (cull) {
-		unsigned long long acc = 0ull;
 		const int fx = (int)floorf(xs), fy = (int)floorf(ys);
 		constexpr int ROUNDS = (SMH_CULL_CELLS + 63) / 64;
-		uint32_t hits[ROUNDS];
+		const uint32_t sh = (uint32_t)(fx - SMH_SECTOR_R) & 31u;
+		uint32_t cells[ROUNDS], lo[ROUNDS], hi[ROUNDS], m_out[ROUNDS], m_mid[ROUNDS];
 #pragma unroll
 		for (int it = 0; it < ROUNDS; ++it) {
-			const uint32_t cell = lane + 64u * (uint32_t)it;
+			const uint32_t cell = 64 * it + 63 < SMH_CULL_CELLS ? lane + 64u * (uint32_t)it : min(lane + 64u * (uint32_t)it, (uint32_t)SMH_CULL_CELLS - 1u);
 			const int yi = fy + (int)(cell >> 2) - SMH_SECTOR_R;
-			uint32_t hit = 0;
-			if (cell < SMH_CULL_CELLS) {
-				const int b0 = fx - SMH_SECTOR_R + (int)((cell & 3u) << 5);
-				const uint32_t lo = win2_word(mw, b0 >> 5, yi), hi = win2_word(mw, (b0 >> 5) + 1, yi);
-				hit = __builtin_amdgcn_alignbit(hi, lo, (uint32_t)b0 & 31u) & cull_tab[cell];
-			}
-			hits[it] = hit;
-		}
+			const int wq = (fx - SMH_SECTOR_R + (int)((cell & 3u) << 5)) >> 5;
+			lo[it] = win2_word(mw, wq, yi); hi[it] = win2_word(mw, wq + 1, yi);
+			m_out[it] = cull_tab[cell]; m_mid[it] = SMH_CULL_MID_CELL(cull_tab, cell);
+			cells[it] = cell;
+		}
+		const uint8_t *codes = SMH_CULL_CODES(cull_tab);
+		unsigned long long acc_o = 0ull, acc_m = 0ull;
 #pragma unroll
 		for (int it = 0; it < ROUNDS; ++it) {
-			uint32_t hit = hits[it];
-			if (hit) {
-				const uint32_t cell = lane + 64u * (uint32_t)it;
-				const uint8_t *codes = (const uint8_t *)(cull_tab + SMH_CULL_CELLS) + (cell >> 2) * SMH_SECTOR_DIM + ((cell & 3u) << 5);
-				while (hit) {
-					const uint32_t code = codes[__builtin_ctz(hit)];
+			const uint32_t px32 = __builtin_amdgcn_alignbit(hi[it], lo[it], sh);
+			const uint32_t h_out = px32 & m_out[it], h_mid = cull == 2u ? px32 & m_mid[it] : 0u;
+			const uint8_t *c = codes + (cells[it] >> 2) * SMH_SECTOR_DIM + ((cells[it] & 3u) << 5);
+			uint32_t hit = h_out | h_mid;
+			while (hit) {
+				uint32_t b[4], code[4];
+#pragma unroll
+				for (int k = 0; k < 4; ++k) {
+					b[k] = hit || k == 0 ? (uint32_t)__builtin_ctz(hit) : b[k - 1];
 					hit &= hit - 1u;
-					acc |= code == 0xFFu ? ~0ull : ((2ull << (code >> 6)) - 1ull) << (code & 63u);
-				}
-			}
-		}
-		acc = wave_or64(acc);
-		live = (acc | (acc >> LSD_GROUPS)) & ((1ull << LSD_GROUPS) - 1ull);
+				}
+#pragma unroll
+				for (int k = 0; k < 4; ++k) code[k] = c[b[k]];
+#pragma unroll
+				for (int k = 0; k < 4; ++k) {
+					const unsigned long long units = code[k] == 0xFFu ? ~0ull : ((2ull << (code[k] >> 6)) - 1ull) << (code[k] & 63u);
+					if ((h_out >> b[k]) & 1u) acc_o |= units;
+					if ((h_mid >> b[k]) & 1u) acc_m |= units;
+				}
+			}
+		}
+		const unsigned long long seen_outer = cull_fold(wave_or64(acc_o));
+		live = cull == 2u ? smh_cull_live(seen_outer, cull_fold(wave_or64(acc_m)), true) : seen_outer;
 	}
 }
 
@@ -1054,7 +1063,7 @@
 		if (MODE == LSD_MODE_TILE) return tile_word(m, (int)c, (int)(wy0 + r));
 		return m.p[wi];
 	};
-	const bool cull = b.cull_tab != nullptr && max_gap > 0.0f && max_gap <= 49.0f;
+	const uint32_t cull = cull_mode_for(b.cull_tab, max_gap);
 	const uint32_t epoch = b.co.epoch;
 	if (tid == 0) { ws.stuck = 0u; ws.lock = 0u; ws.head = 0u; ws.tail = 0u; ws.spec = 1u; ws.n_lines = 0u; ws.rounds = 0u; ws.frame_done = 0u; ws.steps = 0ull;
 	                ws.win_free = (1u << W_NWIN) - 1u; ws.farm_on = 0u; ws.farm_posted = 0u; ws.farm_retired = 0u;
@@ -1294,7 +1303,7 @@
 	const uint32_t tid = threadIdx.x, lane = tid & 63u;
 	const Win &m = v.m;
 	uint32_t *wwins = smem + win_cap + 2u * list_cap;
-	const bool cull = b.cull_tab != nullptr && max_gap > 0.0f && max_gap <= 49.0f;
+	const uint32_t cull = cull_mode_for(b.cull_tab, max_gap);
 	const uint32_t epoch = b.co.epoch;
 	if (tid == 0) { ws.lock = 0u; ws.head = 0u; ws.tail = 0u; ws.win_free = (1u << W_NWIN) - 1u; ws.farm_posted = 0u; ws.frame_done = 0u; }
 	if (tid < W_ROB) { ws.rob[tid].state = W_FREE; ws.rob[tid].todo = 0ull; }
@@ -1450,7 +1459,7 @@
 #ifdef SMH_LSD_FAT
 	asm volatile("; register footprint experiment" ::: SMH_LSD_FAT);
 #endif
-	const bool cull = b.cull_tab != nullptr && max_gap > 0.0f && max_gap <= 49.0f;
+	const uint32_t cull = cull_mode_for(b.cull_tab, max_gap);
 	const uint32_t f = blockIdx.x;
 	const FrameAux aux = b.aux[f];
 	const TileKernelArgs *ka = (const TileKernelArgs *)__builtin_amdgcn_kernarg_segment_ptr();
diff --git a/squad-mortar-helper_amd/csrc/smh_runtime.cpp b/squad-mortar-helper_amd/csrc/smh_runtime.cpp
--- a/squad-mortar-helper_amd/csrc/smh_runtime.cpp
+++ b/squad-mortar-helper_amd/csrc/smh_runtime.cpp
@@ -329,12 +329,13 @@
 	(void)hipFree(d_dense);
 	if (e != hipSuccess) return fail(SMHV_E_HIP, "sector table: %s", hipGetErrorString(e));
 	std::vector<uint32_t> cells(SMH_CULL_TAB_WORDS, 0u);
-	uint8_t *codes = (uint8_t *)&cells[SMH_CULL_CELLS];
+	uint8_t *codes = (uint8_t *)&cells[SMH_CULL_ANNULI * SMH_CULL_CELLS];
 	for (uint32_t row = 0; row < SMH_SECTOR_DIM; ++row)
 		for (uint32_t col = 0; col < SMH_SECTOR_DIM; ++col) {
-			const unsigned long long m = dense[row * SMH_SECTOR_DIM + col] & ((1ull << 57) - 1ull);
+			const unsigned long long e = dense[row * SMH_SECTOR_DIM + col], m = e & ((1ull << SMH_CULL_UNITS) - 1ull);
 			if (!m) continue;
-			cells[row * 4 + (col >> 5)] |= 1u << (col & 31u);
+			if (e & SMH_CULL_IN_OUTER) cells[row * 4 + (col >> 5)] |= 1u << (col & 31u);
+			if (SMH_CULL_ANNULI == 2 && (e & SMH_CULL_IN_MIDDLE)) cells[(SMH_CULL_ANNULI - 1) * SMH_CULL_CELLS + row * 4 + (col >> 5)] |= 1u << (col & 31u);
 			codes[row * SMH_SECTOR_DIM + col] = unit_code(m);
 		}
 	uint32_t *d = nullptr;
diff --git a/squad-mortar-helper_amd/csrc/smh_service.inc b/squad-mortar-helper_amd/csrc/smh_service.inc
--- a/squad-mortar-helper_amd/csrc/smh_service.inc
+++ b/squad-mortar-helper_amd/csrc/smh_service.inc
@@ -89,7 +89,7 @@
 	if (!uniform_u32(ok)) return;
 	const uint32_t rw = ka->g.rw, rh = ka->g.rh, tile_cap = ka->p.tile_cap, list_cap = ka->p.list_cap;
 	const float max_gap = ka->p.max_gap;
-	const bool cull = ka->p.cull_tab != nullptr && max_gap > 0.0f && max_gap <= 49.0f;
+	const uint32_t cull = cull_mode_for(ka->p.cull_tab, max_gap);
 	const float *ray_off = ka->p.ray_off;
 	Win m;
 	if constexpr (COMPACT) tilec_win(m, rw, rh, opart + SVC_WS_WORDS, tile_cap); else tile_win(m, rw, rh, opart + SVC_WS_WORDS, tile_cap);
@@ -169,7 +169,7 @@
 	}
 	wave_lds_sync();
 	const float max_gap = ka->p.max_gap;
-	const bool cull = ka->p.cull_tab != nullptr && max_gap > 0.0f && max_gap <= 49.0f;
+	const uint32_t cull = cull_mode_for(ka->p.cull_tab, max_gap);
 	const float *ray_off = ka->p.ray_off;
 	Win m;
 	if constexpr (COMPACT) tilec_win(m, rw, rh, store, tile_cap); else tile_win(m, rw, rh, store, tile_cap);
```

Result: faster. 642,700, median of 6 (+1.6%).
